# bplaut/PyTorch-VAE

Hardware: AMD Instinct MI355X
Metric: train images/sec (node) VanillaVAE 64×64 bs=64 at 1/2/4/8 GPU; ELBO match (higher is better)
Workload: dtype bf16; 1 GPU; VanillaVAE latent_dim=128 64x64 train step (fwd+ELBO+bwd+Adam); per_gpu_batch=64, global_batch=64, parallelism=dp1, graph=True, comm=none

## Files before the change

### include/vaehip.h

```cpp
#ifndef VAEHIP_H
#define VAEHIP_H

#include <stddef.h>
#include <stdint.h>

#ifdef __cplusplus
extern "C" {
#endif

#define VAE_ABI_VERSION 26

enum vae_dtype { VAE_F32 = 0, VAE_BF16 = 1 };

enum vae_status {
  VAE_OK = 0,
  VAE_E_BADARG = -1,
  VAE_E_BADSHAPE = -2,
  VAE_E_BADDTYPE = -3,
  VAE_E_UNSUPPORTED = -4
};

enum vae_xform_kind {
  VAE_X_NONE = 0,
  VAE_X_ACT = 1,
  VAE_X_BN_ACT = 2,
  VAE_X_BN_DY = 3
};

typedef struct vae_xform {
  int32_t kind;
  int32_t channels;
  float slope;
  float count;
  float eps;
  float momentum;
  const float* sum;
  const float* sumsq;
  const float* shift;
  const float* gamma;
  const float* beta;
  const float* dgamma;
  const float* dbeta;
  const void* aux;
  float* running_mean;
  float* running_var;
  int32_t reps;
  int32_t rstride;
  float* dgamma_out;
  float* dbeta_out;
  const float* table;
} vae_xform;

typedef struct vae_bn_args {
  int32_t mode;
  vae_xform xf;
  float* table;
  float* db;
} vae_bn_args;

typedef struct vae_conv_args {
  int32_t dtype;
  int32_t n, h, w, c;
  int32_t k, p, q;
  int32_t r, stride, pad;
  int32_t x_nchw_f32;
  const void* x;
  vae_xform x_xf;
  const void* wt;
  const float* bias;
  void* y;
  float* y_sum;
  float* y_sumsq;
  int32_t sum_reps;
  int32_t sum_rstride;
  const void* residual;
  vae_xform residual_xf;
  const void* dy;
  vae_xform dy_xf;
  void* dx;
  vae_xform dx_epi;
  float* dx_dgamma;
  float* dx_dbeta;
  float* dw;
  float* db;
  int32_t split_k;
  void* workspace;
  int64_t workspace_bytes;
  const struct vae_bn_args* bn_finalize;
  uint32_t* bn_counter;
  const void* wt_t;
  int32_t dw_inner;
  int32_t deterministic;
  int32_t defer_reduce;
} vae_conv_args;

typedef struct vae_linear_args {
  int32_t dtype;
  int32_t m, n, k;
  const void* x; vae_xform x_xf;
  const void* wt; const float* bias;
  void* y;
  int32_t y_f32;
  const void* dy;
  int32_t dy_f32;
  void* dx; vae_xform dx_epi; float* dx_dgamma; float* dx_dbeta;
  int32_t sum_reps, sum_rstride;
  float* dw; float* db;
  const float* mulv;
  const float* eps;
  const float* kl_coef;
  float* dmulv;
  int32_t samples;
  void* workspace;
  int64_t workspace_bytes;
  const struct vae_bn_args* bn_finalize;
  uint32_t* bn_counter;
  int32_t deterministic;
} vae_linear_args;

typedef struct vae_head_args {
  int32_t dtype;
  int32_t n, h, w, c;
  const void* x; vae_xform x_xf;
  const float* wt;
  const float* bias;
  const float* target;
  int32_t samples;
  float* recon;
  float* sse;
  const float* coef;
  void* dx; vae_xform dx_epi; float* dx_dgamma; float* dx_dbeta;
  int32_t sum_reps, sum_rstride;
  float* dw; float* db;
  const float* grad_recon;
  void* workspace;
  int64_t workspace_bytes;
  const struct vae_bn_args* bn_finalize;
  uint32_t* bn_counter;
  const struct vae_elbo_args* elbo;
  int32_t deterministic;
  int32_t defer_reduce;
} vae_head_args;



enum vae_loss_kind { VAE_LOSS_VANILLA = 0, VAE_LOSS_BETA_H = 1, VAE_LOSS_BETA_B = 2, VAE_LOSS_IWAE = 3,
                     VAE_LOSS_VQ = 4, VAE_LOSS_INFO = 5, VAE_LOSS_DIP = 6, VAE_LOSS_MIWAE = 7 };

typedef struct vae_elbo_args {
  int32_t kind;
  int32_t batch, samples, latent;
  int32_t img_elems;
  float kld_weight;
  float beta, gamma, c_max, c_stop_iter;
  const float* iter;
  const float* mulv;
  const float* sse;
  float* out;
  float* per_img;
  float* head_coef;
  float* kl_coef;
  const float* vq_sse;
  float vq_beta;
  float vq_elems;
  float recon_weight, kl_factor, mmd_coef;
  int32_t mmd_tiles;
  const double* mmd_partials;
  float* mmd_out;
} vae_elbo_args;

typedef struct vae_dip_args {
  int32_t batch, latent;
  float lambda_diag, lambda_offdiag;
  float grad_scale;
  int32_t reserved;
  const float* mulv;
  float* dmulv_dip;
  float* dmulv;
  void* workspace;
  int64_t workspace_bytes;
} vae_dip_args;

enum vae_mmd_kind { VAE_MMD_IMQ = 0, VAE_MMD_RBF = 1 };
typedef struct vae_mmd_args {
  int32_t kind;
  int32_t batch, latent;
  float latent_var;
  float grad_scale;
  int32_t prior_gen;
  const float* mulv;
  const float* eps;
  float* prior;
  float* dz;
  float* dmulv;
  void* workspace;
  int64_t workspace_bytes;
  const int32_t* prior_step;
  uint64_t prior_seed;
} vae_mmd_args;

typedef struct vae_vq_args {
  int32_t dtype;
  int32_t rows, dim, codes;
  const void* lat;
  vae_xform lat_xf;
  const float* codebook;
  int64_t* indices;
  void* q;
  float* sse;
  float beta;
  const void* dq;
  const float* loss_grad;
  void* dlat;
  float* dcodebook;
} vae_vq_args;

typedef struct vae_recon_args {
  int32_t dtype;
  int32_t n, h, w, c;
  const void* y;
  const float* target;
  float* recon;
  float* sse;
  void* dy;
  float grad_scale;
  const float* grad_recon;
  int32_t ld;
} vae_recon_args;

int vae_abi_version(void);
const char* vae_last_error(void);
const char* vae_build_digest(void);
int vae_launch_log(int32_t on);
int64_t vae_launch_log_names(char* buf, int64_t cap);

int vae_conv2d_fwd(const vae_conv_args* a, void* stream);
int vae_conv2d_bwd_data(const vae_conv_args* a, void* stream);
int vae_conv2d_bwd_filter(const vae_conv_args* a, void* stream);
int vae_convT2d_fwd(const vae_conv_args* a, void* stream);
int vae_convT2d_bwd_data(const vae_conv_args* a, void* stream);
int vae_convT2d_bwd_filter(const vae_conv_args* a, void* stream);
int vae_convT2d_bwd(const vae_conv_args* a, void* stream);
int vae_convT2d_fwd_recon(const vae_conv_args* a, const vae_recon_args* rc, void* stream);
int vae_linear_fwd(const vae_linear_args* a, void* stream);
int vae_linear_bwd_data(const vae_linear_args* a, void* stream);
int vae_linear_bwd_filter(const vae_linear_args* a, void* stream);
int vae_head_fwd(const vae_head_args* a, void* stream);
int vae_head_bwd_data(const vae_head_args* a, void* stream);
int vae_head_bwd_filter(const vae_head_args* a, void* stream);
int vae_head_bwd(const vae_head_args* a, void* stream);
int vae_bn_finalize(const vae_bn_args* a, void* stream);
int vae_reparam_fwd(int32_t dtype, int32_t rows, int32_t samples, int32_t latent,
                    const float* mulv, const float* eps, void* z, void* stream);
int vae_vq_fwd(const vae_vq_args* a, void* stream);
int vae_vq_bwd(const vae_vq_args* a, void* stream);
int vae_recon_fwd(const vae_recon_args* a, void* stream);
int vae_recon_bwd(const vae_recon_args* a, void* stream);
int vae_nchw_to_nhwc_pad(int32_t dtype, int32_t n, int32_t c, int32_t h, int32_t w, int32_t cp, const float* x,
                         void* y, void* stream);
int vae_pad_channels(int32_t dtype, int64_t rows, int32_t c, int32_t cp, const void* src, void* dst, void* stream);
int vae_unpad_accumulate(int64_t rows, int32_t cp, int32_t c, const float* src, float* dst, void* stream);
int vae_elbo_fwd(const vae_elbo_args* a, void* stream);
int vae_mmd_fwd(const vae_mmd_args* a, void* stream);
int vae_mmd_workspace_size(const vae_mmd_args* a, size_t* bytes, int32_t* tiles);
int vae_mmd_reseed(int32_t batch, int32_t latent, const float* dz, const float* scale, const float* mulv,
                   const float* eps, float* dmulv, void* stream);
int vae_dip_fwd(const vae_dip_args* a, void* stream);
int vae_dip_workspace_size(const vae_dip_args* a, size_t* bytes, int32_t* tiles);
int vae_adam_step(int64_t n, float* p, const float* g, float* m, float* v,
                  const int32_t* step, const float* lr, double beta1, double beta2, float eps,
                  float weight_decay, void* p_lowp, void* stream);
#define VAE_SUMSQ_MAX_PARTS 1024
int vae_grad_sumsq(int64_t n, const float* g, double* partials, int32_t* nparts_out, void* stream);
int vae_adam_step_clip(int64_t n, float* p, const float* g, float* m, float* v,
                       const int32_t* step, const float* lr, double beta1, double beta2, float eps,
                       float weight_decay, void* p_lowp, const double* partials, int32_t nparts,
                       const float* max_norm, float* norm_out, void* stream);
#define VAE_SLAB_MAX 32
typedef struct vae_grad_slab {
  float* dst;
  int64_t count;
  const float* slab;
  int32_t rows;
  int64_t ld;
} vae_grad_slab;
int vae_deferred_reset(void);
int32_t vae_deferred_take(vae_grad_slab* out, int32_t max, vae_elbo_args* elbo, int32_t* has_elbo);
typedef struct vae_adam_args {
  int64_t n;
  float* p; float* g; float* m; float* v;
  const int32_t* step; const float* lr;
  double beta1, beta2;
  float eps, weight_decay;
  void* p_lowp;
  int32_t nslab;
  vae_grad_slab slab[VAE_SLAB_MAX];
  int32_t has_elbo;
  vae_elbo_args elbo;
} vae_adam_args;
int vae_adam_step_ex(const vae_adam_args* a, void* stream);
int vae_cast_bf16(int64_t n, const float* src, void* dst, void* stream);
#define VAE_SWAP_MAX 16
typedef struct vae_swap_desc {
  const void* src;
  void* dst;
  int32_t a, rs, b;
  int32_t src_dtype;
} vae_swap_desc;
int vae_swap_axes(int32_t count, const vae_swap_desc* descs, void* stream);
enum vae_op { VAE_OP_FWD = 0, VAE_OP_BWD_DATA = 1, VAE_OP_BWD_FILTER = 2, VAE_OP_BWD = 3  };
int vae_conv2d_workspace_size(const vae_conv_args* a, int32_t op, size_t* bytes);
int vae_convT2d_workspace_size(const vae_conv_args* a, int32_t op, size_t* bytes);
int vae_linear_workspace_size(const vae_linear_args* a, int32_t op, size_t* bytes);
int vae_head_workspace_size(const vae_head_args* a, int32_t op, size_t* bytes);
enum vae_layer_kind { VAE_LAYER_CONV2D = 0, VAE_LAYER_CONVT2D = 1 };
int vae_conv_bwd_filter_batch(int32_t n, const int32_t* kinds, const vae_conv_args* const* items,
                              void* workspace, int64_t workspace_bytes, void* stream);
int vae_conv_bwd_filter_batch_workspace_size(int32_t n, const int32_t* kinds, const vae_conv_args* const* items,
                                             size_t* bytes);
typedef struct vae_record_args {
  int32_t batch, samples, img_elems, nterms, step;
  const float* src_terms; float* terms;
  const float* per_img; float* per;
  const float* img; const float* recon;
  float* best; int32_t* at;
  float* hi_img; float* hi_recon; float* lo_img; float* lo_recon;
} vae_record_args;
int vae_step_record(const vae_record_args* a, void* stream);
int vae_step_begin(void* zero, int64_t bytes, int32_t* step, void* stream);

#define VAE_PAD_MAX 4
typedef struct vae_pad_desc {
  int64_t rows;
  int32_t c, cp;
  const void* src;
  void* dst;
} vae_pad_desc;
typedef struct vae_step_begin_args {
  void* zero;
  int64_t bytes;
  int32_t* step;
  int32_t dtype;
  int32_t n, c, h, w, cp;
  const float* x;
  void* y;
  int32_t npad;
  vae_pad_desc pad[VAE_PAD_MAX];
  int32_t nswap;
  vae_swap_desc swap[VAE_SWAP_MAX];
  int32_t nkeep;
  struct { int64_t off, bytes; } keep[VAE_SLAB_MAX];
} vae_step_begin_args;
int vae_step_begin_ex(const vae_step_begin_args* a, void* stream);

typedef struct vae_latent_args {
  int32_t dtype;
  int32_t batch, samples, latent;
  int32_t in_features, out_features;
  const void* x;
  vae_xform x_xf;
  const void* w1;
  const float* b1;
  float* mulv;
  const float* eps;
  void* z;
  const void* w2;
  const float* b2;
  void* h;
  const void* dh;
  const float* kl_coef;
  float* dmulv;
  float* dw2; float* db2;
  void* dx;
  vae_xform dx_epi;
  float* dx_dgamma; float* dx_dbeta;
  int32_t sum_reps, sum_rstride;
  float* dw1; float* db1;
  const int32_t* eps_step;
  uint64_t eps_seed;
  int32_t eps_gen;
} vae_latent_args;
int vae_latent_fc_fwd(const vae_latent_args* a, void* stream);
int vae_latent_dec_fwd(const vae_latent_args* a, void* stream);
int vae_latent_dec_bwd(const vae_latent_args* a, void* stream);
int vae_latent_fc_bwd(const vae_latent_args* a, void* stream);

typedef struct vae_bn_apply_args {
  int32_t dtype;
  int64_t rows;
  int32_t channels;
  const void* x;
  vae_xform xf;
  float* db;
  void* out;
} vae_bn_apply_args;
int vae_bn_apply(const vae_bn_apply_args* a, void* stream);

enum vae_recon_loss_kind { VAE_RLOSS_CENTER = 0, VAE_RLOSS_MSSIM = 1 };
typedef struct vae_recon_loss_args {
  int32_t kind;
  int32_t n, c, h, w;
  const float* recon;
  const float* target;
  const float* mask;
  float window[16];
  int32_t window_size;
  int32_t levels;
  float level_weights[8];
  int32_t normalize;
  int32_t size_average;
  float* grad;
  float grad_scale;
  float* out;
  const float* sse;
  float* per_img;
  float* workspace;
  int64_t workspace_bytes;
} vae_recon_loss_args;
int vae_recon_loss(const vae_recon_loss_args* a, void* stream);
int vae_recon_loss_workspace_size(const vae_recon_loss_args* a, size_t* bytes);

typedef struct vae_logcosh_args {
  int32_t n;
  int32_t latent;
  int64_t elems;
  float alpha;
  float grad_scale;
  float kl_weight;
  int32_t reserved;
  const float* recon;
  const float* target;
  float* grad;
  const float* mulv;
  float* out;
  float* kl_coef;
  const float* sse;
  float* per_img;
  void* workspace;
  int64_t workspace_bytes;
} vae_logcosh_args;
int vae_logcosh_loss(const vae_logcosh_args* a, void* stream);
int vae_logcosh_loss_workspace_size(const vae_logcosh_args* a, size_t* bytes);

#ifdef __cplusplus
}
#endif
#endif
```

### pytorch-vae_amd/csrc/vae_cgemm.hpp

```cpp
#pragma once
#include "vae_igemm.hpp"

namespace vae {

template <int BM, int BN> struct CgWaves {
  static constexpr int WN = BN >= 2 * BM ? 4 : (BM >= 2 * BN ? 1 : 2);
  static constexpr int WM = 4 / WN;
  static constexpr int TM = BM / WM / 16, TN = BN / WN / 16;
  static_assert(TM >= 1 && TN >= 1, "wave tile below 16x16");
};

template <int XA>
__device__ __forceinline__ uint4 cg_xform(const uint32_t (&w)[4], const uint32_t (&y)[4], const Tab& t, int ch,
                                          float slope) {
  if constexpr (XA == VAE_X_NONE) {
    return uint4{w[0], w[1], w[2], w[3]};
  } else {
    uint4 o;
    uint32_t* op = reinterpret_cast<uint32_t*>(&o);
    f32x2 ab[4], bb[4], cb[4];
    if constexpr (XA != VAE_X_ACT) {
      const f32x4 a0 = tab4(t.a, ch), a1 = tab4(t.a, ch + 4);
      ab[0] = f32x2{a0[0], a0[1]}; ab[1] = f32x2{a0[2], a0[3]}; ab[2] = f32x2{a1[0], a1[1]}; ab[3] = f32x2{a1[2], a1[3]};
      {
        const f32x4 b0 = tab4(t.b, ch), b1 = tab4(t.b, ch + 4);
        bb[0] = f32x2{b0[0], b0[1]}; bb[1] = f32x2{b0[2], b0[3]}; bb[2] = f32x2{b1[0], b1[1]}; bb[3] = f32x2{b1[2], b1[3]};
      }
      if constexpr (XA == VAE_X_BN_DY) {
        const f32x4 c0 = tab4(t.c, ch), c1 = tab4(t.c, ch + 4);
        cb[0] = f32x2{c0[0], c0[1]}; cb[1] = f32x2{c0[2], c0[3]}; cb[2] = f32x2{c1[0], c1[1]}; cb[3] = f32x2{c1[2], c1[3]};
      }
    }
    const f32x2 sl = f32x2{slope, slope};
#pragma unroll
    for (int e = 0; e < 4; ++e) {
      const f32x2 v = f32x2{__uint_as_float(w[e] << 16), __uint_as_float(w[e] & 0xffff0000u)};
      f32x2 r;
      if constexpr (XA == VAE_X_ACT) {
        r = __builtin_elementwise_max(v, v * sl);
      } else if constexpr (XA == VAE_X_BN_ACT) {
        const f32x2 z = __builtin_elementwise_fma(v, ab[e], bb[e]);
        r = __builtin_elementwise_max(z, z * sl);
      } else {
        const f32x2 u = f32x2{__uint_as_float(y[e] << 16), __uint_as_float(y[e] & 0xffff0000u)};
        r = __builtin_elementwise_fma(ab[e], v, __builtin_elementwise_fma(bb[e], u, cb[e]));
      }
      bf16x2 pk;
      pk[0] = (__bf16)r[0];
      pk[1] = (__bf16)r[1];
      op[e] = *reinterpret_cast<uint32_t*>(&pk);
    }
    return o;
  }
}

constexpr int kRingLoads = 20, kRingMax = 8;
constexpr int cg_ring(int loads) {
  return kRingLoads / loads < 2 ? 2 : (kRingLoads / loads > kRingMax ? kRingMax : kRingLoads / loads);
}
template <int LOADS> constexpr int cg_stages() { return cg_ring(LOADS); }
constexpr int kRingLoadsDeep = 40, kRingMaxDeep = 16;
constexpr int cg_ring_deep(int loads) {
  return kRingLoadsDeep / loads < 2 ? 2 : (kRingLoadsDeep / loads > kRingMaxDeep ? kRingMaxDeep : kRingLoadsDeep / loads);
}
template <int LOADS> constexpr int wg_stages() {
  return 20 / LOADS < 2 ? 2 : (20 / LOADS > 8 ? 8 : 20 / LOADS);
}

template <int BM, int BN, int BK, int NBUF = 2> struct CgSmem {
  static constexpr int LDK = BK + 8;
  static constexpr int LOOP = NBUF * (BM + BN) * LDK * 2;
  static constexpr int EPI = BM * (BN + 4) * 4;
  static constexpr int BYTES = LOOP > EPI ? LOOP : EPI;
};

template <int BM, int BN, int XA> constexpr int cg_waves_per_eu() {
  return (BM >= 128 && BN >= 128) ? 2 : ((BM == 64 && BN == 32 && XA == VAE_X_BN_DY) ? 3 : 1);
}

template <int BM, int BN, int BK, int AM, int XA, int EM, int OR>
__device__ __forceinline__ void cgemm_body(const GemmParams& p, const int bid, char* smem) {
  using WG = CgWaves<BM, BN>;
  constexpr int TM = WG::TM, TN = WG::TN, WTM = TM * 16, WTN = TN * 16;
  constexpr int LDK = CgSmem<BM, BN, BK>::LDK;
  constexpr int KC = BK / 8;
  constexpr int RPP = 256 / KC;
  constexpr int APT = (BM + RPP - 1) / RPP, BPT = (BN + RPP - 1) / RPP;
  constexpr bool DY = XA == VAE_X_BN_DY;
  constexpr int NSF = OR == 3 ? cg_ring_deep(APT * (DY ? 2 : 1) + BPT) : cg_stages<APT * (DY ? 2 : 1) + BPT>();
  constexpr int NS = OR == 2 ? (NSF < 2 ? NSF : 2) : NSF;
  constexpr int NBUF = OR == 2 ? 1 : 2;
  constexpr bool ABN = XA == VAE_X_BN_ACT || XA == VAE_X_BN_DY;
  static_assert(BM % RPP == 0 || BM < RPP, "A tile rows");
  static_assert(BN % RPP == 0 || BN < RPP, "B tile rows");

  extern __shared__ float tabs[];
  __bf16* As = reinterpret_cast<__bf16*>(smem);
  __bf16* Bs = As + NBUF * BM * LDK;

#ifdef VAE_PROBE
  unsigned long long clk[4] = {0, 0, 0, 0};
  const unsigned long long wall0 = threadIdx.x == 0 ? wall_clock64() : 0;
#endif
  PROBE_MARK(0);
  const int tid = threadIdx.x, lane = tid & 63;
  const int wave = __builtin_amdgcn_readfirstlane(tid >> 6);
  const int wm = wave / WG::WN, wn = wave % WG::WN;
  const int gm = (p.M + BM - 1) / BM, gn = (p.N + BN - 1) / BN, gz = p.nphase * p.ksplit;
  int tile;
  {
    const int nb = gm * gn * gz, b = bid;
    const int q = nb >> 3, r = nb & 7, x = b & 7, loc = b >> 3;
    tile = x * q + min(x, r) + loc;
  }
  int tn, tz, tmi;
  if (p.m_fast) { tmi = tile % gm; tz = (tile / gm) % gz; tn = tile / (gm * gz); }
  else { tn = tile % gn; tz = (tile / gn) % gz; tmi = tile / (gn * gz); }
  const int m0 = tmi * BM, n0 = tn * BN;
  const int phase = (p.nphase > 1) ? (int)(tz / p.ksplit) : 0;
  const int ks = tz - phase * p.ksplit;
  const bool first_block = tile == 0;

  const PhaseInfo pq = make_phase(p, phase);
  const int Kp = AM == A_CONVT ? pq.nth * pq.ntw * p.gc : p.K;
  const int ktiles = (Kp + BK - 1) / BK;
  const int kper = (ktiles + p.ksplit - 1) / p.ksplit;
  const int kt0 = ks * kper;
  const int kt1 = min(ktiles, kt0 + kper);
  const int kend = min(Kp, kt1 * BK);

  const int kc = tid % KC, r0 = tid / KC;
  const Src<__bf16> sa = make_src<__bf16>(p.a_ptr, p.a_bytes, p.a_xf);
  const rsrc_t rb = make_rsrc(p.b_ptr, p.b_bytes);
  RowOperand<__bf16, AM, true> ar[APT];
  int bbase[BPT];
  bool bok[BPT];
#pragma unroll
  for (int i = 0; i < APT; ++i) ar[i].init(p, m0 + r0 + i * RPP, p.M, phase, p.a_ld);
#pragma unroll
  for (int i = 0; i < BPT; ++i) {
    const int n = n0 + r0 + i * RPP;
    bok[i] = n < p.N && r0 + i * RPP < BN;
    bbase[i] = n * p.b_ld;
  }
  const bool a_row_in_tile = r0 < BM;

  struct Stage {
    uint32_t a[APT][4];
    uint32_t y[DY ? APT : 1][4];
    uint32_t b[BPT][4];
    int ch;
    uint32_t okm;
  };
  auto issue = [&](int kt, Stage& st) {
    const int kk = kt * BK + 8 * kc;
    const KTap t = RowOperand<__bf16, AM, true>::tap(p, pq, p.fd_ach, p.a_xf.channels, ABN, kk, kend);
    st.ch = t.ch;
    uint32_t okm = 0u;
#pragma unroll
    for (int i = 0; i < APT; ++i) {
      bool ok = ar[i].valid && t.kin && a_row_in_tile;
      ok = ok && (uint32_t)(ar[i].hi0 + t.r) < (uint32_t)p.gh && (uint32_t)(ar[i].wi0 + t.s) < (uint32_t)p.gw;
      okm |= (uint32_t)ok << i;
      const uint32_t off = ok ? (uint32_t)(ar[i].base + t.toff) * 2u : kOOB;
      bload<16>(sa.x, off, st.a[i]);
      if constexpr (DY) bload<16>(sa.y, off, st.y[i]);
    }
    st.okm = okm;
    int boff = kk;
    if constexpr (AM == A_CONVT) {
      const int rr = pq.t0h - p.gs * t.r, ss = pq.t0w - p.gs * t.s;
      boff = t.kin ? (rr * p.gr + ss) * p.gc + t.ch : 0;
    }
#pragma unroll
    for (int i = 0; i < BPT; ++i) {
      const uint32_t off = (bok[i] && t.kin) ? (uint32_t)(bbase[i] + boff) * 2u : kOOB;
      bload<16>(rb, off, st.b[i]);
    }
  };

  const int ca = tab_stride(p.a_xf.channels), ce = tab_stride(p.epi_xf.channels);
  const Tab ta{tabs, tabs + ca, tabs + 2 * ca, nullptr, nullptr};
  float* tq = tabs + (ABN ? 3 * ca : 0);
  const Tab te{tq, tq + ce, nullptr, tq + 2 * ce, tq + 3 * ce};

  constexpr int TCH = 2;
  float tva[3][TCH], tve[4][TCH];
  const bool a_tab = ABN && p.a_xf.table != nullptr && p.a_xf.channels <= 256 * TCH;
  const bool e_tab = EM == E_BNBWD && p.epi_xf.kind == VAE_X_BN_ACT && p.epi_xf.table != nullptr &&
                     p.epi_xf.channels <= 256 * TCH;
  if (a_tab) {
    const int C = p.a_xf.channels;
#pragma unroll
    for (int j = 0; j < TCH; ++j) {
      const int ch = min(tid + 256 * j, C - 1);
#pragma unroll
      for (int q = 0; q < (DY ? 3 : 2); ++q) tva[q][j] = p.a_xf.table[q * C + ch];
    }
  }
  if (e_tab) {
    const int C = p.epi_xf.channels;
#pragma unroll
    for (int j = 0; j < TCH; ++j) {
      const int ch = min(tid + 256 * j, C - 1);
#pragma unroll
      for (int q = 0; q < 4; ++q) tve[q][j] = p.epi_xf.table[q * C + ch];
    }
  }
  TabPre<DY ? 4 : 2> pa;
  TabPre<2> pe;
  const bool a_pre = ABN && !a_tab && tab_pre_ok<XA>(p.a_xf);
  const bool e_pre = EM == E_BNBWD && !e_tab && tab_pre_ok<VAE_X_BN_ACT>(p.epi_xf);
  if (a_pre) tab_pre_load(p.a_xf, pa);
  if (e_pre) tab_pre_load(p.epi_xf, pe);
  Stage ring[NS];
#pragma unroll
  for (int u = 0; u < NS; ++u) {
    if (!OR || kt0 + u < kt1) issue(kt0 + u, ring[u]);
  }
  constexpr int EC = BN / 8, ERS = 256 / EC;
  constexpr int EPT = (BM + ERS - 1) / ERS;
  const int ec = tid % EC, er0 = tid / EC;
  const int col = n0 + ec * 8;
  const bool col_ok = col < p.N;
  uint32_t aux[EPT][4], res[EPT][4];
  int obase[EPT];
  bool rok[EPT];
  float bias[8];
  const bool has_res = p.residual != nullptr;
  constexpr bool EARLY = EPT <= 2 && cg_waves_per_eu<BM, BN, XA>() < 3;
  auto epi_loads = [&]() {
    const rsrc_t raux = epi_aux_rsrc<EM>(p);
    const rsrc_t rres = epi_res_rsrc<EM>(p);
    const bool loads = p.slab == nullptr;
#pragma unroll
    for (int i = 0; i < EPT; ++i) {
      const int rl = er0 + i * ERS, row = m0 + rl;
      rok[i] = rl < BM && row < p.M && col_ok;
      obase[i] = out_row_base(p, phase, rok[i] ? row : 0) + col;
      const uint32_t off = (rok[i] && loads) ? (uint32_t)obase[i] * 2u : kOOB;
      bload<16>(raux, off, aux[i]);
      if (EM == E_BNBWD && has_res) bload<16>(rres, off, res[i]);
      else res[i][0] = res[i][1] = res[i][2] = res[i][3] = 0u;
    }
#pragma unroll
    for (int e = 0; e < 8; ++e) bias[e] = 0.f;
    if (EM == E_STORE && p.bias && col_ok && loads) {
#pragma unroll
      for (int e = 0; e < 8; ++e) bias[e] = p.bias[col + e];
    }
  };
  if constexpr (EARLY) epi_loads();
  if (a_tab) {
    const int C = p.a_xf.channels;
#pragma unroll
    for (int j = 0; j < TCH; ++j) {
      const int ch = tid + 256 * j;
      if (ch < C) {
        ta.a[ch] = tva[0][j]; ta.b[ch] = tva[1][j];
        if (DY) ta.c[ch] = tva[2][j];
      }
    }
  } else if constexpr (ABN) {
    tab_fill_pre(p.a_xf, pa, a_pre, ta, false, first_block, reinterpret_cast<float*>(smem));
  }
  if constexpr (ABN) {
    if (tid < 8) { const int z = tab_pad(p.a_xf.channels) + tid; ta.a[z] = 0.f; ta.b[z] = 0.f; ta.c[z] = 0.f; }
  }
  if (e_tab) {
    const int C = p.epi_xf.channels;
#pragma unroll
    for (int j = 0; j < TCH; ++j) {
      const int ch = tid + 256 * j;
      if (ch < C) { te.a[ch] = tve[0][j]; te.b[ch] = tve[1][j]; te.p[ch] = tve[2][j]; te.q[ch] = tve[3][j]; }
    }
  } else if constexpr (EM == E_BNBWD) {
    tab_fill_pre(p.epi_xf, pe, e_pre, te, true, false, reinterpret_cast<float*>(smem));
  }
  __syncthreads();
  PROBE_MARK(1);

  f32x4 acc[TM][TN];
#pragma unroll
  for (int i = 0; i < TM; ++i)
#pragma unroll
    for (int j = 0; j < TN; ++j) acc[i][j] = f32x4{0.f, 0.f, 0.f, 0.f};

  auto store = [&](int buf, const Stage& st) {
    __bf16* ad = As + buf * BM * LDK + r0 * LDK + kc * 8;
#pragma unroll
    for (int i = 0; i < APT; ++i) {
      if (r0 + i * RPP < BM) {
        uint4 v;
        if constexpr (XA == VAE_X_NONE) {
          v = uint4{st.a[i][0], st.a[i][1], st.a[i][2], st.a[i][3]};
        } else {
          const int ch = ((st.okm >> i) & 1u) ? st.ch : sa.zs;
          v = cg_xform<XA>(st.a[i], st.y[DY ? i : 0], ta, ch, sa.slope);
        }
        *reinterpret_cast<uint4*>(ad + i * RPP * LDK) = v;
      }
    }
    __bf16* bd = Bs + buf * BN * LDK + r0 * LDK + kc * 8;
#pragma unroll
    for (int i = 0; i < BPT; ++i)
      if (r0 + i * RPP < BN) *reinterpret_cast<uint4*>(bd + i * RPP * LDK) = uint4{st.b[i][0], st.b[i][1], st.b[i][2], st.b[i][3]};
  };
  auto compute = [&](int buf) {
    const __bf16* a = As + buf * BM * LDK + (wm * WTM + (lane & 15)) * LDK + 8 * (lane >> 4);
    const __bf16* b = Bs + buf * BN * LDK + (wn * WTN + (lane & 15)) * LDK + 8 * (lane >> 4);
#pragma unroll
    for (int kk = 0; kk < BK / 32; ++kk) {
      bf16x8 af[TM], bfr[TN];
#pragma unroll
      for (int i = 0; i < TM; ++i) af[i] = *reinterpret_cast<const bf16x8*>(a + i * 16 * LDK + 32 * kk);
#pragma unroll
      for (int j = 0; j < TN; ++j) bfr[j] = *reinterpret_cast<const bf16x8*>(b + j * 16 * LDK + 32 * kk);
#pragma unroll
      for (int i = 0; i < TM; ++i)
#pragma unroll
        for (int j = 0; j < TN; ++j) acc[i][j] = __builtin_amdgcn_mfma_f32_16x16x32_bf16(af[i], bfr[j], acc[i][j], 0, 0, 0);
    }
  };

  if constexpr (OR != 0) {
#pragma unroll
    for (int u = 0; u < NS; ++u) {
      if (kt0 + u < kt1) {
        if (NBUF == 1 && u > 0) __syncthreads();
        store(u & (NBUF - 1), ring[u]);
        __syncthreads();
        compute(u & (NBUF - 1));
      }
    }
  } else {
    int buf = 0;
    for (int kb = kt0; kb < kt1; kb += NS) {
#pragma unroll
      for (int u = 0; u < NS; ++u) {
        const bool live = kb + u < kt1;
        if (live) store(buf, ring[u]);
        __syncthreads();
        issue(kb + u + NS, ring[u]);
        if (live) compute(buf);
        buf ^= 1;
      }
    }
  }
  PROBE_MARK(2);
#ifdef VAE_PROBE
  struct ProbeEnd {
    unsigned long long* pr; unsigned long long* clk; unsigned long long w0;
    __device__ ~ProbeEnd() { PROBE_MARK(3); probe_write(pr, clk, w0); }
  } probe_end{p.probe, clk, wall0};
#endif

  __shared__ float fpart[CgWaves<BM, BN>::WM][2][BN];
  const bool frag_sums = EM == E_STORE && p.sum != nullptr && p.slab == nullptr;
  if (frag_sums) {
#pragma unroll
    for (int j = 0; j < TN; ++j) {
      float a1 = 0.f, a2 = 0.f;
#pragma unroll
      for (int i = 0; i < TM; ++i)
#pragma unroll
        for (int e = 0; e < 4; ++e) { a1 += acc[i][j][e]; a2 = fmaf(acc[i][j][e], acc[i][j][e], a2); }
      a1 += __shfl_xor(a1, 16); a2 += __shfl_xor(a2, 16);
      a1 += __shfl_xor(a1, 32); a2 += __shfl_xor(a2, 32);
      if (lane < 16) { fpart[wm][0][wn * WTN + j * 16 + lane] = a1; fpart[wm][1][wn * WTN + j * 16 + lane] = a2; }
    }
  }
  __syncthreads();
  float* Cs = reinterpret_cast<float*>(smem);
  constexpr int LDC = BN + 4;
  {
    const int rq = wm * WTM + 4 * (lane >> 4), cq = wn * WTN + (lane & 15);
#pragma unroll
    for (int i = 0; i < TM; ++i)
#pragma unroll
      for (int j = 0; j < TN; ++j)
#pragma unroll
        for (int e = 0; e < 4; ++e) Cs[(rq + i * 16 + e) * LDC + cq + j * 16] = acc[i][j][e];
  }
  __syncthreads();
  if (p.slab) {
    float* sl = p.slab + ((long)(phase * p.ksplit + ks) * p.M) * p.N;
#pragma unroll
    for (int i = 0; i < EPT; ++i) {
      const int rl = er0 + i * ERS, row = m0 + rl;
      if (rl < BM && row < p.M && col_ok) {
        const f32x4 v0 = *reinterpret_cast<const f32x4*>(Cs + rl * LDC + ec * 8);
        const f32x4 v1 = *reinterpret_cast<const f32x4*>(Cs + rl * LDC + ec * 8 + 4);
        *reinterpret_cast<f32x4*>(sl + (long)row * p.N + col) = v0;
        *reinterpret_cast<f32x4*>(sl + (long)row * p.N + col + 4) = v1;
      }
    }
    return;
  }
  if constexpr (!EARLY) epi_loads();
  float s1[8], s2[8];
#pragma unroll
  for (int e = 0; e < 8; ++e) { s1[e] = 0.f; s2[e] = 0.f; }
  int ech = 0;
  if constexpr (EM == E_BNBWD) ech = (int)(col - p.fd_ech.div(col) * p.epi_xf.channels);
  uint4 pk[EPT];
#pragma unroll
  for (int i = 0; i < EPT; ++i) {
    const int rl = min(er0 + i * ERS, BM - 1);
    float v[8], ax[8], rs[8];
    {
      const f32x4 v0 = *reinterpret_cast<const f32x4*>(Cs + rl * LDC + ec * 8);
      const f32x4 v1 = *reinterpret_cast<const f32x4*>(Cs + rl * LDC + ec * 8 + 4);
#pragma unroll
      for (int e = 0; e < 4; ++e) { v[e] = v0[e]; v[e + 4] = v1[e]; }
    }
#pragma unroll
    for (int e = 0; e < 4; ++e) {
      ax[2 * e] = __uint_as_float(aux[i][e] << 16);
      ax[2 * e + 1] = __uint_as_float(aux[i][e] & 0xffff0000u);
      rs[2 * e] = __uint_as_float(res[i][e] << 16);
      rs[2 * e + 1] = __uint_as_float(res[i][e] & 0xffff0000u);
    }
    const float w = rok[i] ? 1.f : 0.f;
    float o[8];
    if constexpr (EM == E_STORE) {
      const bool ract = p.res_xf.kind == VAE_X_ACT;
#pragma unroll
      for (int e = 0; e < 8; ++e) {
        float y = v[e] + bias[e];
        if (has_res) y += ract ? lrelu(ax[e], p.res_xf.slope) : ax[e];
        o[e] = y;
      }
    } else {
      const int ek = p.epi_xf.kind;
#pragma unroll
      for (int e = 0; e < 8; ++e) {
        const float g0 = v[e] + rs[e];
        float g = g0;
        if (ek == VAE_X_BN_ACT) {
          const float z = fmaf(ax[e], te.a[ech + e], te.b[ech + e]);
          g = z > 0.f ? g0 : g0 * p.epi_xf.slope;
          s1[e] = fmaf(w, g, s1[e]);
          s2[e] = fmaf(w * g, fmaf(ax[e], te.p[ech + e], te.q[ech + e]), s2[e]);
        } else if (ek == VAE_X_ACT) {
          g = ax[e] > 0.f ? g0 : g0 * p.epi_xf.slope;
        }
        o[e] = g;
      }
    }
    uint32_t* pp = reinterpret_cast<uint32_t*>(&pk[i]);
#pragma unroll
    for (int e = 0; e < 4; ++e) {
      bf16x2 h;
      h[0] = (__bf16)o[2 * e];
      h[1] = (__bf16)o[2 * e + 1];
      pp[e] = *reinterpret_cast<uint32_t*>(&h);
    }
  }
  if (frag_sums) {
    for (int c = tid; c < BN; c += 256) {
      if (n0 + c < p.N) {
        float t1 = 0.f, t2 = 0.f;
#pragma unroll
        for (int w = 0; w < CgWaves<BM, BN>::WM; ++w) { t1 += fpart[w][0][c]; t2 += fpart[w][1][c]; }
        epi_flush_sums<EM>(p, bid, n0 + c, t1, t2);
      }
    }
  } else if (EM == E_BNBWD && epi_wants_sums<EM>(p)) {
    float* part = Cs;
#pragma unroll
    for (int m = EC; m < 64; m <<= 1) {
#pragma unroll
      for (int e = 0; e < 8; ++e) {
        s1[e] += __shfl_xor(s1[e], m);
        s2[e] += __shfl_xor(s2[e], m);
      }
    }
    __syncthreads();
    if (lane < EC) {
#pragma unroll
      for (int e = 0; e < 8; ++e) {
        part[(wave * 2) * BN + ec * 8 + e] = s1[e];
        part[(wave * 2 + 1) * BN + ec * 8 + e] = s2[e];
      }
    }
    __syncthreads();
    for (int c = tid; c < BN; c += 256) {
      if (n0 + c < p.N) {
        const float t1 = (part[0 * BN + c] + part[2 * BN + c]) + (part[4 * BN + c] + part[6 * BN + c]);
        const float t2 = (part[1 * BN + c] + part[3 * BN + c]) + (part[5 * BN + c] + part[7 * BN + c]);
        epi_flush_sums<EM>(p, bid, n0 + c, t1, t2);
      }
    }
  }
  __bf16* out = static_cast<__bf16*>(p.out);
#pragma unroll
  for (int i = 0; i < EPT; ++i)
    if (rok[i]) *reinterpret_cast<uint4*>(out + obase[i]) = pk[i];
}

template <int BM, int BN, int BK, int OR> constexpr int cg_nbuf() { return OR == 2 ? 1 : 2; }

template <int BM, int BN, int BK, int AM, int XA, int EM, int OR>
__global__ void __launch_bounds__(256) __attribute__((amdgpu_waves_per_eu(cg_waves_per_eu<BM, BN, XA>())))
cgemm_kernel(const GemmParams p) {
  kernarg_prefetch<sizeof(GemmParams)>();
  __shared__ __attribute__((aligned(16))) char smem[CgSmem<BM, BN, BK, cg_nbuf<BM, BN, BK, OR>()>::BYTES];
  cgemm_body<BM, BN, BK, AM, XA, EM, OR>(p, (int)blockIdx.x, smem);
}

}
```

### pytorch-vae_amd/csrc/vae_common.hpp

```cpp
#pragma once
#include <hip/hip_runtime.h>
#include <stdint.h>
#include <string.h>

#include "vaehip.h"

typedef float f32x4 __attribute__((ext_vector_type(4)));
typedef float f32x2 __attribute__((ext_vector_type(2)));
typedef __bf16 bf16x8 __attribute__((ext_vector_type(8)));
typedef __bf16 bf16x4 __attribute__((ext_vector_type(4)));
typedef __bf16 bf16x2 __attribute__((ext_vector_type(2)));

namespace vae {

void set_error(const char* fmt, ...);
int fail(int code, const char* fmt, ...);
int check_launch(const char* what);
int bn_finalize_launch(const vae_bn_args* a, hipStream_t stream);
constexpr int kRouteDeclined = 0x7fff0001;

inline int grid_for(long n, int per_block = 256, int max_blocks = 2048) {
  long b = (n + per_block - 1) / per_block;
  if (b < 1) b = 1;
  return (int)(b > max_blocks ? max_blocks : b);
}

struct OrdSum {
  const float* slab;
  long rstride;
  int groups, rpg, cols, cw;
  long hstride;
  int folds;
  long fstride;
  float* dst[2];
  long gstride;
};
int ordered_sum_launch(const OrdSum& o, hipStream_t st);

struct WsQuery {
  int on;
  long need;
};
inline WsQuery& ws_query() {
  static thread_local WsQuery q = {0, 0};
  return q;
}
inline bool querying() { return ws_query().on != 0; }
struct Deferred {
  int n;
  vae_grad_slab s[VAE_SLAB_MAX];
  int has_elbo;
  vae_elbo_args elbo;
};
inline Deferred& deferred() {
  static thread_local Deferred d = {};
  return d;
}
inline bool defer_slab(float* dst, long count, const float* slab, int rows, long ld) {
  if (querying()) return true;
  Deferred& d = deferred();
  for (int i = 0; i < d.n; ++i)
    if (d.s[i].dst == dst) {
      d.s[i] = vae_grad_slab{dst, count, slab, rows, ld};
      return true;
    }
  if (d.n >= VAE_SLAB_MAX) {
    fail(VAE_E_UNSUPPORTED, "deferred reductions: more than %d outstanding", VAE_SLAB_MAX);
    return false;
  }
  d.s[d.n++] = vae_grad_slab{dst, count, slab, rows, ld};
  return true;
}
inline void defer_elbo(const vae_elbo_args& e) {
  if (querying()) return;
  Deferred& d = deferred();
  d.has_elbo = 1;
  d.elbo = e;
}
inline bool ws_fits(long need, long have, const char* what) {
  WsQuery& q = ws_query();
  if (q.on) {
    if (need > q.need) q.need = need;
    return true;
  }
  if (need <= have) return true;
  fail(VAE_E_BADARG, "%s: workspace of %ld bytes < %ld required (see vae_*_workspace_size)", what, have, need);
  return false;
}
template <class F>
inline int with_ws_tail(long tail, F&& f) {
  WsQuery& q = ws_query();
  if (!q.on) return f();
  const long outer = q.need;
  q.need = 0;
  const int rc = f();
  const long inner = ((q.need + 255) / 256) * 256 + tail;
  q.need = outer > inner ? outer : inner;
  return rc;
}
struct LaunchLog {
  int on;
  int n;
  const void* k[64];
  int count[64];
};
inline LaunchLog& launch_log() {
  static thread_local LaunchLog l = {0, 0, {}, {}};
  return l;
}
inline void log_launch(const void* k) {
  LaunchLog& l = launch_log();
  if (!l.on) return;
  for (int i = 0; i < l.n; ++i)
    if (l.k[i] == k) { ++l.count[i]; return; }
  if (l.n < 64) { l.count[l.n] = 1; l.k[l.n++] = k; }
}
}
#define VAE_LAUNCH(K, ...)                                      \
  do {                                                          \
    if (!::vae::querying()) {                                   \
      ::vae::log_launch((const void*)(K));                      \
      hipLaunchKernelGGL(K, __VA_ARGS__);                       \
    }                                                           \
  } while (0)
namespace vae {

template <int BYTES>
__device__ __forceinline__ void kernarg_prefetch() {
  const void* k = (const void*)__builtin_amdgcn_kernarg_segment_ptr();
  unsigned d1, d2, d3, d4, d5, d6, d7;
  if constexpr (BYTES > 960) {
    unsigned e1, e2, e3, e4, e5, e6, e7, e8;
    asm volatile(
        "s_load_dword %0, %15, 64\n s_load_dword %1, %15, 128\n s_load_dword %2, %15, 192\n"
        " s_load_dword %3, %15, 256\n s_load_dword %4, %15, 320\n s_load_dword %5, %15, 384\n"
        " s_load_dword %6, %15, 448\n s_load_dword %7, %15, 512\n s_load_dword %8, %15, 576\n"
        " s_load_dword %9, %15, 640\n s_load_dword %10, %15, 704\n s_load_dword %11, %15, 768\n"
        " s_load_dword %12, %15, 832\n s_load_dword %13, %15, 896\n s_load_dword %14, %15, 960\n"
        " s_waitcnt lgkmcnt(0)"
        : "=&s"(d1), "=&s"(d2), "=&s"(d3), "=&s"(d4), "=&s"(d5), "=&s"(d6), "=&s"(d7), "=&s"(e1), "=&s"(e2), "=&s"(e3),
          "=&s"(e4), "=&s"(e5), "=&s"(e6), "=&s"(e7), "=&s"(e8)
        : "s"(k));
  } else if constexpr (BYTES > 448) {
    asm volatile(
        "s_load_dword %0, %7, 64\n s_load_dword %1, %7, 128\n s_load_dword %2, %7, 192\n"
        " s_load_dword %3, %7, 256\n s_load_dword %4, %7, 320\n s_load_dword %5, %7, 384\n"
        " s_load_dword %6, %7, 448\n s_waitcnt lgkmcnt(0)"
        : "=&s"(d1), "=&s"(d2), "=&s"(d3), "=&s"(d4), "=&s"(d5), "=&s"(d6), "=&s"(d7)
        : "s"(k));
  } else if constexpr (BYTES > 192) {
    asm volatile("s_load_dword %0, %3, 64\n s_load_dword %1, %3, 128\n s_load_dword %2, %3, 192\n"
                 " s_waitcnt lgkmcnt(0)"
                 : "=&s"(d1), "=&s"(d2), "=&s"(d3)
                 : "s"(k));
  } else if constexpr (BYTES > 64) {
    asm volatile("s_load_dword %0, %1, 64\n s_waitcnt lgkmcnt(0)" : "=&s"(d1) : "s"(k));
  }
}

__device__ __forceinline__ float ld_f(const float* p) { return *p; }
__device__ __forceinline__ float ld_f(const __bf16* p) { return (float)(*p); }
template <class T> __device__ __forceinline__ T cvt(float v);
template <> __device__ __forceinline__ float cvt<float>(float v) { return v; }
template <> __device__ __forceinline__ __bf16 cvt<__bf16>(float v) { return (__bf16)v; }

__device__ __forceinline__ void ld8(const float* p, float (&v)[8]) {
  f32x4 a = *reinterpret_cast<const f32x4*>(p);
  f32x4 b = *reinterpret_cast<const f32x4*>(p + 4);
  v[0] = a[0]; v[1] = a[1]; v[2] = a[2]; v[3] = a[3];
  v[4] = b[0]; v[5] = b[1]; v[6] = b[2]; v[7] = b[3];
}
__device__ __forceinline__ void ld8(const __bf16* p, float (&v)[8]) {
  bf16x8 a = *reinterpret_cast<const bf16x8*>(p);
#pragma unroll
  for (int j = 0; j < 8; ++j) v[j] = (float)a[j];
}
__device__ __forceinline__ void ld4(const float* p, float (&v)[4]) {
  f32x4 a = *reinterpret_cast<const f32x4*>(p);
  v[0] = a[0]; v[1] = a[1]; v[2] = a[2]; v[3] = a[3];
}
__device__ __forceinline__ void ld4(const __bf16* p, float (&v)[4]) {
  bf16x4 a = *reinterpret_cast<const bf16x4*>(p);
#pragma unroll
  for (int j = 0; j < 4; ++j) v[j] = (float)a[j];
}

__device__ __forceinline__ void st8(float* d, const float (&v)[8]) {
  *reinterpret_cast<f32x4*>(d) = f32x4{v[0], v[1], v[2], v[3]};
  *reinterpret_cast<f32x4*>(d + 4) = f32x4{v[4], v[5], v[6], v[7]};
}
__device__ __forceinline__ void st8(__bf16* d, const float (&v)[8]) {
  bf16x8 o;
#pragma unroll
  for (int j = 0; j < 8; ++j) o[j] = (__bf16)v[j];
  *reinterpret_cast<bf16x8*>(d) = o;
}
__device__ __forceinline__ void st2(float* d, float a, float b) { *reinterpret_cast<f32x2*>(d) = f32x2{a, b}; }
// ... 310 lines not shown
```

### pytorch-vae_amd/csrc/vae_convT_bwd_data.hip

```cpp
#include "vae_launch.hpp"
#include "vae_wgrad.hpp"

using namespace vae;

extern "C" int vae_convT2d_bwd_data(const vae_conv_args* a, void* stream) {
  if (int rc = check_geom(a, "convT2d_bwd_data")) return rc;
  if (!a->dy || !a->wt || !a->dx) return fail(VAE_E_BADARG, "convT2d_bwd_data: null tensor");
  if (!xf_ok(a->dy_xf, "convT2d_bwd_data.dy") || !epi_ok(a->dx_epi, "convT2d_bwd_data.epi")) return VAE_E_BADARG;
  hipStream_t st = (hipStream_t)stream;
  GemmParams p = strided_conv_params(a, true, a->wt, a->pad);
  if (int rc = bwd_epilogue(p, a->dx_epi, a->dx_dgamma, a->dx_dbeta, a->sum_reps, a->sum_rstride, nullptr, "convT2d_bwd_data"))
    return rc;
  if (int rc = check_finalize(a->bn_finalize, "convT2d_bwd_data")) return rc;
  if (a->dtype == VAE_BF16 && cg_ok(p, E_BNBWD))
    return then_finalize(cg_launch<A_CONV, E_BNBWD>(p, a->split_k, a->workspace, a->workspace_bytes, st), a->bn_finalize, st);
  return then_finalize(launch<A_CONV, B_NK, E_BNBWD, true, false>(a->dtype, false, false, p, a->split_k, a->workspace,
                                                                  a->workspace_bytes, st),
                       a->bn_finalize, st);
}
```

### pytorch-vae_amd/csrc/vae_convT_fwd.hip

```cpp
#include "vae_launch.hpp"
#include "vae_wgrad.hpp"
#include "vae_hires.hpp"

using namespace vae;

extern "C" int vae_convT2d_fwd(const vae_conv_args* a, void* stream) {
  if (int rc = check_geom(a, "convT2d_fwd")) return rc;
  if (!a->x || !a->wt || !a->y) return fail(VAE_E_BADARG, "convT2d_fwd: null tensor");
  if (!xf_ok(a->x_xf, "convT2d_fwd.x")) return VAE_E_BADARG;
  const int S = a->stride;
  if (a->p % S || a->q % S) return fail(VAE_E_BADSHAPE, "convT2d_fwd: output not a multiple of stride");
  hipStream_t st = (hipStream_t)stream;
  GemmParams p;
  if (!phase_gather_params(p, a, false)) return fail(VAE_E_UNSUPPORTED, "convT2d_fwd: stride/kernel");
  fwd_epilogue(p, a);
  if (int rc = check_finalize(a->bn_finalize, "convT2d_fwd")) return rc;
  if (a->dtype == VAE_BF16) {
    const int rc = hires_convT_fwd_launch(a, st);
    if (rc != kRouteDeclined) return rc;
    const StagedWeights w = staged_weights(a, a->wt_t);
    GemmParams q = p;
    swapped_weights(q, w.ptr);
    if (w.ptr && cg_ok(q, E_STORE)) {
      return with_staged_weights(w, a, a->c, a->k, 0, "convT2d_fwd weight copy", st, [&]() -> int {
        return then_finalize(cg_launch<A_CONVT, E_STORE>(q, a->split_k, a->workspace, w.slab_bytes, st), a->bn_finalize, st);
      });
    }
  }
  return then_finalize(launch<A_CONVT, B_KN, E_STORE, false, false>(a->dtype, false, false, p, a->split_k, a->workspace,
                                                                    a->workspace_bytes, st),
                       a->bn_finalize, st);
}
```

### pytorch-vae_amd/csrc/vae_conv_bwd_data.hip

```cpp
#include "vae_launch.hpp"
#include "vae_wgrad.hpp"
#include "vae_c3.hpp"

using namespace vae;

extern "C" int vae_conv2d_bwd_data(const vae_conv_args* a, void* stream) {
  const char* what = "conv2d_bwd_data";
  if (int rc = check_geom(a, what)) return rc;
  if (!a->dy || !a->wt || !a->dx) return fail(VAE_E_BADARG, "conv2d_bwd_data: null tensor");
  if (!xf_ok(a->dy_xf, "conv2d_bwd_data.dy") || !epi_ok(a->dx_epi, "conv2d_bwd_data.epi")) return VAE_E_BADARG;
  if (a->x_nchw_f32) return fail(VAE_E_UNSUPPORTED, "conv2d_bwd_data: no gradient for the NCHW image input");
  const int S = a->stride;
  if (a->h % S || a->w % S || a->h / S != a->p || a->w / S != a->q)
    return fail(VAE_E_BADSHAPE, "conv2d_bwd_data: needs h == p*stride (got h=%d p=%d S=%d)", a->h, a->p, S);
  hipStream_t st = (hipStream_t)stream;
  const bool tile = a->dtype == VAE_BF16 && a->wt_t && a->dy_xf.kind == VAE_X_NONE &&
                    (a->dx_epi.kind == VAE_X_NONE || a->dx_epi.kind == VAE_X_ACT) && !a->dx_dgamma && !a->bn_finalize &&
                    a->split_k <= 0;
  if (tile && pointwise(a) && p1_shape_ok((long)a->n * a->h * a->w, a->k, a->c)) {
    P1Args c;
    memset(&c, 0, sizeof(c));
    c.a = a->dy; c.b = a->wt_t; c.out = a->dx; c.residual = a->residual;
    if (a->dx_epi.kind == VAE_X_ACT) { c.aux = a->dx_epi.aux; c.aux_slope = a->dx_epi.slope; }
    c.M = (long)a->n * a->h * a->w; c.C = a->k; c.N = a->c;
    return p1_launch(c, st);
  }
  if (tile && c3_shape_ok(a->n, a->p, a->q, a->h, a->w, a->r, a->stride, a->pad, a->k, a->c)) {
    C3Args c;
    memset(&c, 0, sizeof(c));
    c.a = a->dy; c.b = a->wt_t; c.flip = 1; c.out = a->dx; c.residual = a->residual;
    if (a->dx_epi.kind == VAE_X_ACT) { c.aux = a->dx_epi.aux; c.aux_slope = a->dx_epi.slope; }
    c.n = a->n; c.C = a->k; c.N = a->c;
    return c3_launch(c, st);
  }
  auto epilogue = [&](GemmParams& p) {
    return bwd_epilogue(p, a->dx_epi, a->dx_dgamma, a->dx_dbeta, a->sum_reps, a->sum_rstride, a->residual, what);
  };
  GemmParams p;
  const bool phases = phase_gather_params(p, a, true);
  if (phases) {
    if (int rc = epilogue(p)) return rc;
  }
  if (phases && a->dtype == VAE_BF16) {
    const StagedWeights w = staged_weights(a, a->wt_t);
    GemmParams q = p;
    swapped_weights(q, w.ptr);
    if (w.ptr && cg_ok(q, E_BNBWD)) {
      if (int rc = check_finalize(a->bn_finalize, what)) return rc;
      return with_staged_weights(w, a, a->k, a->c, 0, "conv2d_bwd_data weight copy", st, [&]() -> int {
        return then_finalize(cg_launch<A_CONVT, E_BNBWD>(q, a->split_k, a->workspace, w.slab_bytes, st), a->bn_finalize, st);
      });
    }
  }
  if (S == 1 && a->dtype == VAE_BF16 && a->c % 8 == 0 && a->k % 8 == 0 && a->workspace) {
    const StagedWeights w = staged_weights(a, nullptr);
    return with_staged_weights(w, a, a->k, a->c, 1, "conv2d_bwd_data weight copy", st, [&]() -> int {
      GemmParams f = strided_conv_params(a, true, w.ptr, a->r - 1 - a->pad);
      if (int rc = epilogue(f)) return rc;
      if (int rc = check_finalize(a->bn_finalize, what)) return rc;
      return then_finalize(launch<A_CONV, B_NK, E_BNBWD, true, false>(a->dtype, false, false, f, a->split_k, a->workspace,
                                                                      w.slab_bytes, st),
                           a->bn_finalize, st);
    });
  }
  if (!phases) return fail(VAE_E_UNSUPPORTED, "conv2d_bwd_data: stride/kernel");
  if (int rc = check_finalize(a->bn_finalize, what)) return rc;
  return then_finalize(launch<A_CONVT, B_KN, E_BNBWD, true, false>(a->dtype, false, false, p, a->split_k, a->workspace,
                                                                   a->workspace_bytes, st),
                       a->bn_finalize, st);
}
```

### pytorch-vae_amd/csrc/vae_conv_fwd.hip

```cpp
#include "vae_launch.hpp"
#include "vae_wgrad.hpp"
#include "vae_c3.hpp"

using namespace vae;

extern "C" int vae_conv2d_fwd(const vae_conv_args* a, void* stream) {
  if (int rc = check_geom(a, "conv2d_fwd")) return rc;
  if (!a->x || !a->wt || !a->y) return fail(VAE_E_BADARG, "conv2d_fwd: null tensor");
  if (!xf_ok(a->x_xf, "conv2d_fwd.x")) return VAE_E_BADARG;
  hipStream_t st = (hipStream_t)stream;
  const bool tile = a->dtype == VAE_BF16 && !a->x_nchw_f32 && (a->x_xf.kind == VAE_X_NONE || a->x_xf.kind == VAE_X_ACT) &&
                    !a->y_sum && !a->y_sumsq && !a->bn_finalize && a->split_k <= 0;
  if (tile && pointwise(a) && p1_shape_ok((long)a->n * a->p * a->q, a->c, a->k) &&
      (a->residual_xf.kind == VAE_X_NONE || a->residual_xf.kind == VAE_X_ACT)) {
    P1Args c;
    memset(&c, 0, sizeof(c));
    c.a = a->x; c.a_act = a->x_xf.kind == VAE_X_ACT; c.a_slope = a->x_xf.slope;
    c.b = a->wt; c.out = a->y; c.bias = a->bias;
    c.residual = a->residual; c.res_act = a->residual && a->residual_xf.kind == VAE_X_ACT; c.res_slope = a->residual_xf.slope;
    c.M = (long)a->n * a->p * a->q; c.C = a->c; c.N = a->k;
    return p1_launch(c, st);
  }
  if (tile && c3_shape_ok(a->n, a->h, a->w, a->p, a->q, a->r, a->stride, a->pad, a->c, a->k) && !a->residual) {
    C3Args c;
    memset(&c, 0, sizeof(c));
    c.a = a->x; c.a_act = a->x_xf.kind == VAE_X_ACT; c.a_slope = a->x_xf.slope;
    c.b = a->wt; c.flip = 0; c.out = a->y; c.bias = a->bias;
    c.n = a->n; c.C = a->c; c.N = a->k;
    return c3_launch(c, st);
  }
  GemmParams p = strided_conv_params(a, false, a->wt, a->pad);
  fwd_epilogue(p, a);
  if (int rc = check_finalize(a->bn_finalize, "conv2d_fwd")) return rc;
  if (a->dtype == VAE_BF16 && cg_ok(p, E_STORE))
    return then_finalize(cg_launch<A_CONV, E_STORE>(p, a->split_k, a->workspace, a->workspace_bytes, st), a->bn_finalize, st);
  return then_finalize(launch<A_CONV, B_NK, E_STORE, false, false, true>(a->dtype, a->x_nchw_f32 != 0, false, p, a->split_k,
                                                                         a->workspace, a->workspace_bytes, st),
                       a->bn_finalize, st);
}
```

### pytorch-vae_amd/csrc/vae_igemm.hpp

```cpp
#pragma once
#include "vae_common.hpp"

namespace vae {

enum AMode { A_CONV = 0, A_CONVT = 1, A_DENSE = 2, A_KM = 3 };
enum BMode { B_NK = 0, B_KN = 1, B_GATHER = 2 };
enum EMode { E_STORE = 0, E_BNBWD = 1, E_ACC = 2, E_REPARAM = 3 };

constexpr int MAXC = 4096;
constexpr int NTHREADS = 256;

template <class T> constexpr int bk_of() { return sizeof(T) == 2 ? 64 : 32; }

struct FastDiv {
  uint32_t d, mul, shr;
  __device__ __forceinline__ uint32_t div(uint32_t n) const { return (__umulhi(n, mul) + n) >> shr; }
};

inline FastDiv make_fastdiv(uint32_t d) {
  FastDiv f;
  f.d = d < 1 ? 1 : d;
  uint32_t l = 0;
  while ((1ull << l) < f.d) ++l;
  f.shr = l;
  f.mul = (uint32_t)(((1ull << 32) * ((1ull << l) - f.d)) / f.d + 1);
  if (f.d == 1) f.mul = 0;
  return f;
}

struct GemmParams {
  int M, N, K;
  int ksplit, nphase;
  const void* a_ptr; int a_ld; vae_xform a_xf;
  const void* b_ptr; int b_ld; vae_xform b_xf;
  int ones_col;
  int b_taps;
  int g_nchw;
  int gn, gh, gw, gc, gp, gq, gr, gs, gpad, gho, gwo;
  int ntap_h[2], ntap_w[2], tap0[2];
  int tap_d[2];
  FastDiv fd_gq, fd_gp, fd_gc, fd_gr, fd_ntw[2];
  void* out; int out_ld; int out_phase;
  int out_f32;
  const float* bias; float* sum; float* sumsq;
  const void* residual; vae_xform res_xf;
  vae_xform epi_xf; float* dgamma; float* dbeta;
  float* bias_grad;
  float* dbc; int dbc_from_b;
  int sum_reps, sum_rstride;
  const float* mulv; const float* eps; const float* kl_coef; float* dmulv; int samples, latent;
  float* slab;
  uint32_t a_bytes, b_bytes;
  FastDiv fd_ach, fd_bch;
  FastDiv fd_ech;
  uint32_t out_aux_bytes;
  unsigned long long* probe;
  int m_fast;
  int det;
  float* det_slab;
  int det_rows;
};

#ifdef VAE_PROBE
#define PROBE_MARK(i) do { if (threadIdx.x == 0) clk[i] = __builtin_readcyclecounter(); } while (0)
__device__ __forceinline__ void probe_write(unsigned long long* pr, const unsigned long long* clk,
                                           unsigned long long w0) {
  if (!pr || threadIdx.x != 0) return;
  const unsigned long long slot = blockIdx.x + (unsigned long long)gridDim.x * (blockIdx.y + (unsigned long long)gridDim.y * blockIdx.z);
  if (slot >= pr[1]) return;
  unsigned long long* r = pr + 8 + slot * 8;
  r[0] = blockIdx.x | ((unsigned long long)blockIdx.y << 21) | ((unsigned long long)blockIdx.z << 42);
  r[1] = w0;
  r[2] = wall_clock64();
  r[3] = clk[0]; r[4] = clk[1]; r[5] = clk[2]; r[6] = clk[3];
  r[7] = __builtin_amdgcn_s_getreg((23 << 0) | (0 << 6) | (31 << 11));
}
#else
#define PROBE_MARK(i) do { } while (0)
#endif

struct PhaseInfo {
  int ph, pw, t0h, t0w, nth, ntw;
  int dh, dw;
  FastDiv fdw;
};

__device__ __forceinline__ PhaseInfo make_phase(const GemmParams& p, int phase) {
  PhaseInfo q;
  q.ph = phase >= p.gs ? 1 : 0;
  q.pw = phase - q.ph * p.gs;
  q.t0h = q.ph ? p.tap0[1] : p.tap0[0];
  q.t0w = q.pw ? p.tap0[1] : p.tap0[0];
  q.nth = q.ph ? p.ntap_h[1] : p.ntap_h[0];
  q.ntw = q.pw ? p.ntap_w[1] : p.ntap_w[0];
  q.fdw = q.pw ? p.fd_ntw[1] : p.fd_ntw[0];
  q.dh = q.ph ? p.tap_d[1] : p.tap_d[0];
  q.dw = q.pw ? p.tap_d[1] : p.tap_d[0];
  return q;
}

__device__ __forceinline__ void tab_zero_slot(const vae_xform& x, Tab t) {
  if (threadIdx.x < 8) {
    const int z = tab_pad(x.channels) + threadIdx.x;
    t.a[z] = 0.f; t.b[z] = 0.f;
    if (x.kind == VAE_X_BN_DY) t.c[z] = 0.f;
  }
}

__device__ __forceinline__ void tab_fill(const vae_xform& x, Tab t, bool epi, bool update_running, float* scr) {
  if (x.kind != VAE_X_BN_ACT && x.kind != VAE_X_BN_DY) return;
  tab_zero_slot(x, t);
  if (x.table) {
    const int C = x.channels;
    const bool dy = x.kind == VAE_X_BN_DY;
    const int nt = blockDim.x;
    for (int c0 = threadIdx.x; c0 < C; c0 += 4 * nt) {
      float v[4][4];
#pragma unroll
      for (int u = 0; u < 4; ++u) {
        const int ch = c0 + u * nt, cc = ch < C ? ch : C - 1;
        v[u][0] = x.table[cc];
        v[u][1] = x.table[C + cc];
        v[u][2] = (dy || epi) ? x.table[2 * C + cc] : 0.f;
        v[u][3] = (!dy && epi) ? x.table[3 * C + cc] : 0.f;
      }
#pragma unroll
      for (int u = 0; u < 4; ++u) {
        const int ch = c0 + u * nt;
        if (ch >= C) break;
        t.a[ch] = v[u][0]; t.b[ch] = v[u][1];
        if (dy) t.c[ch] = v[u][2];
        else if (epi) { t.p[ch] = v[u][2]; t.q[ch] = v[u][3]; }
      }
    }
    return;
  }
  if (blockDim.x == 256 && bn_fast_ok(x)) {
    tab_build(x, t, epi, update_running, scr);
    return;
  }
  for (int ch = threadIdx.x; ch < x.channels; ch += blockDim.x) {
    BnMom mo;
    bn_moments(x, ch, mo.mean, mo.invstd, mo.var);
    const float g = x.gamma[ch];
    if (x.kind == VAE_X_BN_ACT) {
      const BnFwd f = bn_fwd(mo, g);
      t.a[ch] = f.a;
      t.b[ch] = f.b(x.beta[ch]);
      if (epi) { t.p[ch] = f.p; t.q[ch] = f.q; }
      if (update_running && x.running_mean) {
        const float unb = bn_unbiased(mo, x);
        x.running_mean[ch] = bn_momentum(x, x.running_mean[ch], mo.mean);
        x.running_var[ch] = bn_momentum(x, x.running_var[ch], unb);
      }
    } else {
      const float inv_m = 1.0f / x.count;
      const float A = g * mo.invstd;
      const float mg = rsum(x.dbeta, x, ch) * inv_m;
      const float mgx = rsum(x.dgamma, x, ch) * inv_m;
      t.a[ch] = A;
      t.b[ch] = -A * mo.invstd * mgx;
      t.c[ch] = -A * (mg - mo.mean * mo.invstd * mgx);
    }
  }
}

__device__ __forceinline__ void tab_fill(const vae_xform& x, Tab t, bool epi, bool update_running) {
  __shared__ float scr[4 * 256];
  tab_fill(x, t, epi, update_running, scr);
}

template <int KIND>
__device__ __forceinline__ bool tab_pre_ok(const vae_xform& x) {
  return x.kind == KIND && !x.table && blockDim.x == 256 && bn_fast_ok(x);
}
template <int NS>
__device__ __forceinline__ void tab_fill_pre(const vae_xform& x, const TabPre<NS>& q, bool pre, Tab t, bool epi,
                                             bool update_running, float* scr) {
  if (!pre) { tab_fill(x, t, epi, update_running, scr); return; }
  tab_zero_slot(x, t);
  tab_pre_finish(x, q, t, epi, update_running, scr);
}

__host__ __device__ inline int tab_floats(const vae_xform& x, bool epi) {
  if (x.kind != VAE_X_BN_ACT && x.kind != VAE_X_BN_DY) return 0;
  return (epi ? 4 : 3) * tab_stride(x.channels);
}

constexpr uint32_t kOOB = 0x80000000u;
typedef __amdgpu_buffer_rsrc_t rsrc_t;

__device__ __forceinline__ rsrc_t make_rsrc(const void* ptr, uint32_t bytes) {
  return __builtin_amdgcn_make_buffer_rsrc(const_cast<void*>(ptr), (short)0, (int)bytes, 0x00020000);
}

template <int NB>
__device__ __forceinline__ void bload(rsrc_t r, uint32_t off, uint32_t* d) {
  if constexpr (NB == 16) {
    const auto v = __builtin_amdgcn_raw_buffer_load_b128(r, off, 0, 0);
    d[0] = v[0]; d[1] = v[1]; d[2] = v[2]; d[3] = v[3];
  } else if constexpr (NB == 8) {
    const auto v = __builtin_amdgcn_raw_buffer_load_b64(r, off, 0, 0);
    d[0] = v[0]; d[1] = v[1];
  } else if constexpr (NB == 4) {
    d[0] = __builtin_amdgcn_raw_buffer_load_b32(r, off, 0, 0);
  } else {
    d[0] = __builtin_amdgcn_raw_buffer_load_b16(r, off, 0, 0);
  }
}

template <class TIn>
struct Src {
  rsrc_t x, y;
// ... 997 lines not shown
```

### pytorch-vae_amd/csrc/vae_launch.hpp

```cpp
#pragma once
#include "vae_fgemm.hpp"
#include "vae_cgemm.hpp"
#include "vae_bgemm.hpp"
#include "vae_gemm_desc.hpp"
#include <stdlib.h>

#ifdef VAE_PROBE
extern "C" unsigned long long* vae_probe_buffer(void);
#endif

namespace vae {
namespace {

constexpr int kCUs = 256;
constexpr int kTargetBlocks = 512;
constexpr long kLdsBytes = 160 * 1024;

inline long cg_table_bytes(const GemmParams& p, int em) {
  const int k = p.a_xf.kind;
  return 4l * (((k == VAE_X_BN_ACT || k == VAE_X_BN_DY) ? 3 * tab_stride(p.a_xf.channels) : 0) +
               (em == E_BNBWD ? 4 * tab_stride(p.epi_xf.channels) : 0));
}
inline long cg_static_bytes(int bm, int bn) {
  const int bk = bm >= 128 ? 64 : 128;
  const long loop = 2l * (bm + bn) * (bk + 8) * 2, epi = (long)bm * (bn + 4) * 4;
  const int wn = bn >= 2 * bm ? 4 : (bm >= 2 * bn ? 1 : 2);
  return (loop > epi ? loop : epi) + (4 / wn) * 2l * bn * 4 + 256;
}

inline bool xf_ok(const vae_xform& x, const char* what) {
  if (x.kind < VAE_X_NONE || x.kind > VAE_X_BN_DY) { fail(VAE_E_BADARG, "%s: bad xform kind %d", what, x.kind); return false; }
  if (x.kind == VAE_X_BN_ACT || x.kind == VAE_X_BN_DY) {
    if (x.channels > MAXC) { fail(VAE_E_UNSUPPORTED, "%s: %d channels > %d", what, x.channels, MAXC); return false; }
    if (!x.sum || !x.sumsq || !x.gamma || !x.beta || x.count <= 0.f) {
      fail(VAE_E_BADARG, "%s: BatchNorm transform needs sum/sumsq/gamma/beta/count", what); return false;
    }
    if (x.kind == VAE_X_BN_DY && (!x.dgamma || !x.dbeta || !x.aux)) {
      fail(VAE_E_BADARG, "%s: BN_DY transform needs dgamma/dbeta/aux", what); return false;
    }
  }
  if ((x.kind == VAE_X_ACT || x.kind == VAE_X_BN_ACT) && !(x.slope >= 0.f && x.slope <= 1.f)) {
    fail(VAE_E_BADARG, "%s: LeakyReLU slope %g outside [0, 1]", what, x.slope); return false;
  }
  return true;
}

inline bool epi_ok(const vae_xform& x, const char* what) {
  if (!xf_ok(x, what)) return false;
  if ((x.kind == VAE_X_BN_ACT || x.kind == VAE_X_ACT) && !x.aux) {
    fail(VAE_E_BADARG, "%s: activation-backward epilogue needs aux (the stored pre-activation)", what);
    return false;
  }
  if (x.kind == VAE_X_BN_DY) { fail(VAE_E_BADARG, "%s: BN_DY is not an epilogue transform", what); return false; }
  return true;
}

inline int check_finalize(const vae_bn_args* f, const char* what) {
  if (!f) return VAE_OK;
  if (f->mode != 0 && f->mode != 1) return fail(VAE_E_BADARG, "%s: fused finalisation mode %d", what, f->mode);
  if (!f->table || f->xf.channels <= 0 || !f->xf.sum || !f->xf.sumsq || !f->xf.gamma || !f->xf.beta || f->xf.count <= 0.f ||
      (f->mode == 1 && (!f->xf.dgamma || !f->xf.dbeta)) || f->xf.reps > BNF_LANES * BNF_PER)
    return fail(VAE_E_BADARG, "%s: bn_finalize args", what);
  return VAE_OK;
}

inline int then_finalize(int rc, const vae_bn_args* f, hipStream_t st) {
  if (rc || !f) return rc;
  return bn_finalize_launch(f, st);
}

template <int AM>
inline long a_elems(const GemmParams& p) {
  if (AM == A_CONV || AM == A_CONVT) return (long)p.gn * p.gh * p.gw * p.gc;
  if (AM == A_DENSE) return (long)(p.M - 1) * p.a_ld + p.K;
  return (long)(p.K - 1) * p.a_ld + p.M;
}

template <int BMD>
inline long b_elems(const GemmParams& p) {
  if (BMD == B_GATHER) return (long)p.gn * p.gh * p.gw * p.gc;
  if (BMD == B_NK) return (long)(p.N - 1) * p.b_ld + p.K;
  const long rows = p.b_taps ? (long)p.gc * p.gr * p.gr : p.K;
  return (rows - 1) * p.b_ld + (p.ones_col >= 0 ? p.N - 1 : p.N);
}

inline int phase_kmax(const GemmParams& p, int am) {
  if (am != A_CONVT) return p.K;
  int kmax = 0;
  for (int ph = 0; ph < p.nphase; ++ph) {
    const int k = p.ntap_h[ph / p.gs] * p.ntap_w[ph % p.gs] * p.gc;
    kmax = k > kmax ? k : kmax;
  }
  return kmax;
}

inline long out_elems(const GemmParams& p) {
  if (p.out_phase) return (long)p.gn * p.gho * p.gwo * p.out_ld;
  return (long)p.M * p.out_ld;
}

inline int set_extents(GemmParams& p, const char* kernel, long ab, long bb, long ob, long aux, const char* out_note) {
  constexpr long lim = 1l << 31;
  if (ab <= 0 || bb <= 0 || ab >= lim || bb >= lim)
    return fail(VAE_E_UNSUPPORTED, "%s: operand of %ld / %ld bytes (buffer addressing needs < 2 GiB)", kernel, ab, bb);
  if (ob >= lim) return fail(VAE_E_UNSUPPORTED, "%s: output of %ld bytes%s", kernel, ob, out_note);
  p.a_bytes = (uint32_t)ab;
  p.b_bytes = (uint32_t)bb;
  p.out_aux_bytes = (uint32_t)aux;
#ifdef VAE_PROBE
  p.probe = vae_probe_buffer();
#endif
  return VAE_OK;
}

inline bool aligned(const void* ptr, int bytes) { return ((uintptr_t)ptr & (uintptr_t)(bytes - 1)) == 0; }

inline bool bn_kind(const vae_xform& x) { return x.kind == VAE_X_BN_ACT || x.kind == VAE_X_BN_DY; }

template <int MODE>
inline int operand_vec(const GemmParams& p, const void* ptr, const vae_xform& xf, int esize) {
  const bool vk = MODE == A_CONV || MODE == A_CONVT || MODE == A_DENSE || MODE == 100 + B_NK;
  const int grp = vk ? 8 : 4;
  const int vbytes = (grp * esize) < 16 ? grp * esize : 16;
  if (!aligned(ptr, vbytes) || (xf.kind == VAE_X_BN_DY && !aligned(xf.aux, vbytes))) return 0;
  if (bn_kind(xf) && xf.channels % grp) return 0;
  const int nrows = p.N - (p.ones_col >= 0 ? 1 : 0);
  switch (MODE) {
    case A_CONV: return !p.g_nchw && p.gc % grp == 0;
    case 100 + B_GATHER: return !p.g_nchw && p.gc % grp == 0 && nrows % grp == 0;
    case A_CONVT: return p.gc % grp == 0;
    case A_DENSE: return p.a_ld % grp == 0 && p.K % grp == 0;
    case A_KM: return p.a_ld % grp == 0 && p.M % grp == 0;
    case 100 + B_NK: return p.b_ld % grp == 0 && p.K % grp == 0;
    case 100 + B_KN: return p.b_ld % grp == 0 && nrows % grp == 0;
  }
  return 0;
}

inline void finish_divs(GemmParams& p) {
  p.fd_gq = make_fastdiv(p.gq > 0 ? p.gq : 1);
  p.fd_gp = make_fastdiv(p.gp > 0 ? p.gp : 1);
  p.fd_gc = make_fastdiv(p.gc > 0 ? p.gc : 1);
  p.fd_gr = make_fastdiv(p.gr > 0 ? p.gr : 1);
  p.fd_ntw[0] = make_fastdiv(p.ntap_w[0] > 0 ? p.ntap_w[0] : 1);
  p.fd_ntw[1] = make_fastdiv(p.ntap_w[1] > 0 ? p.ntap_w[1] : 1);
  p.fd_ach = make_fastdiv(p.a_xf.channels > 0 ? p.a_xf.channels : 1);
  p.fd_bch = make_fastdiv(p.b_xf.channels > 0 ? p.b_xf.channels : 1);
  p.fd_ech = make_fastdiv(p.epi_xf.channels > 0 ? p.epi_xf.channels : 1);
}

struct Tile { int bm, bn; };

inline long tile_blocks(long M, long N, int nphase, Tile t) {
  return ((M + t.bm - 1) / t.bm) * ((N + t.bn - 1) / t.bn) * nphase;
}

constexpr int kTileBlocks = 4 * kCUs;
inline Tile pick_tile(long M, long N, int nphase) {
  const Tile wide[] = {{64, 64}, {64, 32}, {32, 64}, {32, 32}};
  const Tile thin_n[] = {{128, 32}, {64, 32}, {32, 32}};
  const Tile thin_m[] = {{32, 128}, {32, 64}, {32, 32}};
  const Tile* c = N <= 32 ? thin_n : (M <= 32 ? thin_m : wide);
  const int nc = N <= 32 ? 3 : (M <= 32 ? 3 : 4);
  for (int i = 0; i < nc; ++i)
    if (tile_blocks(M, N, nphase, c[i]) >= kTileBlocks) return c[i];
  return c[nc - 1];
}

inline int pick_split(long blocks, int ktiles) {
  if (blocks >= kTargetBlocks || ktiles < 8) return 1;
  int s = (int)((kTargetBlocks + blocks - 1) / blocks);
  const int maxs = ktiles / 4;
  if (s > maxs) s = maxs;
  return s < 2 ? 1 : s;
}

inline int split_fits(int* split, int split_req, const GemmParams& p, const void* ws, long ws_bytes, const char* what) {
  if (*split <= 1) return VAE_OK;
  if (!ws && !querying()) {
    if (split_req > 1) return fail(VAE_E_BADARG, "%s: split_k %d needs a workspace", what, split_req);
    *split = 1;
    return VAE_OK;
  }
  return ws_fits((long)*split * p.M * p.N * p.nphase * 4, ws_bytes, what) ? VAE_OK : VAE_E_BADARG;
}

template <class T, int EM>
inline int launch_finalize(const GemmParams& p, hipStream_t st) {
  const long rows = (long)p.M * p.nphase;
  const dim3 grid((unsigned)((rows + FIN_ROWS - 1) / FIN_ROWS), (unsigned)((p.N + 63) / 64));
  const size_t lds = EM == E_BNBWD ? (size_t)tab_floats(p.epi_xf, true) * 4 : 0;
  if (p.N % 4 == 0) VAE_LAUNCH((igemm_finalize<T, EM, true>), grid, dim3(NTHREADS), lds, st, p);
  else VAE_LAUNCH((igemm_finalize<T, EM, false>), grid, dim3(NTHREADS), lds, st, p);
  return check_launch("igemm_finalize");
}

template <int EM>
inline bool det_wants_sums(const GemmParams& p) {
  return (EM == E_STORE && p.sum) || (EM == E_BNBWD && p.epi_xf.kind == VAE_X_BN_ACT);
}
inline long det_sum_rows(const GemmParams& p, int bm) {
  if (p.ksplit > 1) return ((long)p.M * p.nphase + FIN_ROWS - 1) / FIN_ROWS;
  return (long)((p.M + bm - 1) / bm) * p.nphase;
}
template <int EM>
inline long det_slab_bytes(const GemmParams& p, int bm) {
  if (!p.det) return 0;
  if (det_wants_sums<EM>(p)) return det_sum_rows(p, bm) * 2 * p.N * 4;
  if (EM == E_REPARAM) return (long)p.M * 2 * p.latent * 4;
  return 0;
}
template <int EM>
inline int det_reduce(const GemmParams& p, hipStream_t st) {
  if (!p.det_slab) return VAE_OK;
  OrdSum o;
  memset(&o, 0, sizeof(o));
  o.slab = p.det_slab;
  if (EM == E_REPARAM) {
    o.rstride = 2L * p.latent; o.groups = p.M / p.samples; o.rpg = p.samples;
    o.cols = 2 * p.latent; o.cw = p.latent; o.hstride = p.latent; o.folds = 1;
    o.dst[0] = p.dmulv; o.dst[1] = p.dmulv + p.latent; o.gstride = 2L * p.latent;
  } else {
    const int ch = EM == E_STORE ? p.N : p.epi_xf.channels;
    o.rstride = 2L * p.N; o.groups = 1; o.rpg = (int)(p.det_rows);
    o.cols = 2 * ch; o.cw = ch; o.hstride = p.N; o.folds = p.N / ch; o.fstride = ch;
    o.dst[0] = EM == E_STORE ? p.sum : p.dbeta;
    o.dst[1] = EM == E_STORE ? p.sumsq : p.dgamma;
  }
  return ordered_sum_launch(o, st);
}

inline thread_local bool lds_error = false;
template <class K>
inline bool lds_fits(K kernel, size_t dyn) {
  if (dyn <= 64 * 1024 || querying()) return true;
  hipFuncAttributes at;
  if (hipFuncGetAttributes(&at, reinterpret_cast<const void*>(kernel)) != hipSuccess) return true;
  if ((long)(at.sharedSizeBytes + dyn) <= kLdsBytes) return true;
  lds_error = true;
  return false;
}

#define VAE_TILE_CASE(BM_, BN_) \
  if (t.bm == BM_ && t.bn == BN_) { \
    if (lds_fits(igemm_kernel<T, TA, TB, BM_, BN_, AM, BMD, EM, VA, VB, DYA, DYB>, lds)) \
      VAE_LAUNCH((igemm_kernel<T, TA, TB, BM_, BN_, AM, BMD, EM, VA, VB, DYA, DYB>), grid, block, lds, st, p); \
    return; \
  }

template <class T, class TA, class TB, int AM, int BMD, int EM, bool VA, bool VB, bool DYA, bool DYB>
inline void launch_shape(const GemmParams& p, Tile t, hipStream_t st) {
  const dim3 block(NTHREADS);
  const dim3 grid((p.M + t.bm - 1) / t.bm, (p.N + t.bn - 1) / t.bn, p.nphase * p.ksplit);
  const size_t lds = (size_t)table_floats(p, EM == E_BNBWD) * 4;
  VAE_TILE_CASE(64, 64)
  VAE_TILE_CASE(128, 32)
  VAE_TILE_CASE(32, 128)
  VAE_TILE_CASE(64, 32)
  VAE_TILE_CASE(32, 64)
  VAE_TILE_CASE(32, 32)
}
#undef VAE_TILE_CASE

template <class T, class TA, class TB, int AM, int BMD, int EM, bool DYA, bool DYB>
inline int launch_tiled(GemmParams p, Tile t, hipStream_t st) {
  const bool tensor_out = EM != E_ACC && EM != E_REPARAM;
  const long oe = tensor_out ? out_elems(p) : 0;
  if (int rc = set_extents(p, "igemm", a_elems<AM>(p) * (long)sizeof(TA), b_elems<BMD>(p) * (long)sizeof(TB),
                           oe * (long)(p.out_f32 ? 4 : sizeof(T)), oe * (long)sizeof(T), " (needs < 2 GiB)"))
    return rc;
  if ((!DYA && p.a_xf.kind == VAE_X_BN_DY) || (!DYB && p.b_xf.kind == VAE_X_BN_DY))
    return fail(VAE_E_UNSUPPORTED, "igemm: BN_DY transform on an operand this op does not support");
  const bool va = operand_vec<AM>(p, p.a_ptr, p.a_xf, (int)sizeof(TA));
  const bool vb = operand_vec<100 + BMD>(p, p.b_ptr, p.b_xf, (int)sizeof(TB));
  if (va && vb) launch_shape<T, TA, TB, AM, BMD, EM, true, true, DYA, DYB>(p, t, st);
  else if (va) launch_shape<T, TA, TB, AM, BMD, EM, true, false, DYA, DYB>(p, t, st);
  else if (vb) launch_shape<T, TA, TB, AM, BMD, EM, false, true, DYA, DYB>(p, t, st);
  else launch_shape<T, TA, TB, AM, BMD, EM, false, false, DYA, DYB>(p, t, st);
  if (lds_error) {
    lds_error = false;
    return fail(VAE_E_UNSUPPORTED, "igemm: per-channel tables of %d / %d channels exceed the LDS", p.a_xf.channels,
                p.epi_xf.channels);
  }
  int rc = check_launch("igemm");
  if (rc) return rc;
  if (p.slab && (rc = launch_finalize<T, EM>(p, st))) return rc;
  return det_reduce<EM>(p, st);
}

template <int AM, int BMD, int EM>
inline bool fgemm_ok(const GemmParams& p) {
  if constexpr (BMD != B_NK || AM == A_KM || EM == E_ACC) return false;
  if constexpr (AM == A_CONV || AM == A_CONVT) return false;
  if (p.g_nchw || p.ones_col >= 0) return false;
  if (p.K % 32 || p.a_ld % 8 || p.b_ld % 8) return false;
  if (!aligned(p.a_ptr, 16) || !aligned(p.b_ptr, 16)) return false;
  if (p.a_xf.kind == VAE_X_BN_DY && !aligned(p.a_xf.aux, 16)) return false;
  if (bn_kind(p.a_xf) && p.a_xf.channels % 8) return false;
  return true;
}

template <class T, class TA, int AM, int EM, bool DYA>
inline int launch_fgemm(GemmParams p, void* ws, long ws_bytes, hipStream_t st) {
  constexpr int BM = 32, BN = 32;
  if (int rc = set_extents(p, "fgemm", a_elems<AM>(p) * (long)sizeof(TA), b_elems<B_NK>(p) * (long)sizeof(T), 0,
                           EM != E_REPARAM ? out_elems(p) * (long)sizeof(T) : 0, ""))
    return rc;
  const int steps = (phase_kmax(p, AM) + 31) / 32;
  const long tiles = (long)((p.M + BM - 1) / BM) * ((p.N + BN - 1) / BN) * p.nphase;
  int split = 1;
  if (tiles < 2 * kCUs) {
    split = (int)((2 * kCUs + tiles - 1) / tiles);
    if (split > steps / 4) split = steps / 4;
    if (split < 2) split = 1;
  }
  if (int rc = split_fits(&split, 0, p, ws, ws_bytes, "fgemm split-K")) return rc;
  p.ksplit = split;
  p.slab = split > 1 ? static_cast<float*>(ws) : nullptr;
  const dim3 grid((p.M + BM - 1) / BM, (p.N + BN - 1) / BN, p.nphase * p.ksplit);
  const size_t lds = (size_t)(tab_floats(p.a_xf, false) + (EM == E_BNBWD ? tab_floats(p.epi_xf, true) : 0)) * 4;
  VAE_LAUNCH((fgemm_kernel<T, TA, BM, BN, AM, EM, DYA>), grid, dim3(256), lds, st, p);
  int rc = check_launch("fgemm");
  if (rc) return rc;
  if (p.slab) return launch_finalize<T, EM>(p, st);
  return VAE_OK;
}

template <int AM, int BMD, int EM, bool DYA, bool DYB, bool A_F32 = false, bool B_F32 = false>
inline int launch(int dtype, bool a_f32, bool b_f32, GemmParams p, int split_req, void* ws, long ws_bytes,
                  hipStream_t st) {
  if (p.M <= 0 || p.N <= 0) return VAE_OK;
  finish_divs(p);
  if constexpr (BMD == B_NK && AM != A_KM && EM != E_ACC) {
    if (!a_f32 && !b_f32 && split_req <= 0 && !p.det && fgemm_ok<AM, BMD, EM>(p)) {
      if (dtype == VAE_F32) return launch_fgemm<float, float, AM, EM, DYA>(p, ws, ws_bytes, st);
      if (dtype == VAE_BF16) return launch_fgemm<__bf16, __bf16, AM, EM, DYA>(p, ws, ws_bytes, st);
    }
// ... 28 lines not shown
  }
  if (dtype == VAE_F32) return launch_tiled<float, float, float, AM, BMD, EM, DYA, DYB>(p, t, st);
  if (dtype != VAE_BF16) return fail(VAE_E_BADDTYPE, "dtype %d", dtype);
  if constexpr (A_F32) {
    if (a_f32) return launch_tiled<__bf16, float, __bf16, AM, BMD, EM, DYA, DYB>(p, t, st);
  }
  if constexpr (B_F32) {
    if (b_f32) return launch_tiled<__bf16, __bf16, float, AM, BMD, EM, DYA, DYB>(p, t, st);
  }
  if (a_f32 || b_f32) return fail(VAE_E_UNSUPPORTED, "fp32 operand not instantiated for this op");
  return launch_tiled<__bf16, __bf16, __bf16, AM, BMD, EM, DYA, DYB>(p, t, st);
}

template <class T, int V>
__global__ void __launch_bounds__(256) column_sum_flat(const T* x, long nvec, int C, float* out) {
  extern __shared__ float red[];
  const int groups = C / V;
  for (int c = threadIdx.x; c < C; c += blockDim.x) red[c] = 0.f;
  __syncthreads();
  const int c0 = (int)(threadIdx.x % groups) * V;
  float acc[V];
#pragma unroll
  for (int j = 0; j < V; ++j) acc[j] = 0.f;
  const long stride = (long)gridDim.x * blockDim.x;
  long i = (long)blockIdx.x * blockDim.x + threadIdx.x;
  for (; i + 7 * stride < nvec; i += 8 * stride) {
    if constexpr (V == 8) {
      float v[8][8];
#pragma unroll
      for (int u = 0; u < 8; ++u) ld8(x + (i + u * stride) * 8, v[u]);
#pragma unroll
      for (int u = 0; u < 8; ++u)
#pragma unroll
        for (int j = 0; j < 8; ++j) acc[j] += v[u][j];
    } else {
      float v[8];
#pragma unroll
      for (int u = 0; u < 8; ++u) v[u] = ld_f(x + i + u * stride);
      acc[0] += ((v[0] + v[1]) + (v[2] + v[3])) + ((v[4] + v[5]) + (v[6] + v[7]));
    }
  }
  for (; i < nvec; i += stride) {
    if constexpr (V == 8) {
      float v[8];
      ld8(x + i * 8, v);
#pragma unroll
      for (int j = 0; j < 8; ++j) acc[j] += v[j];
    } else {
      acc[0] += ld_f(x + i);
    }
  }
#pragma unroll
  for (int j = 0; j < V; ++j) atomicAdd(red + c0 + j, acc[j]);
  __syncthreads();
  for (int c = threadIdx.x; c < C; c += blockDim.x) atomicAdd(out + c, red[c]);
}

template <class T>
__global__ void column_sum(const T* x, long rows, int C, float* out) {
  const int c = blockIdx.y * 64 + (threadIdx.x & 63);
  if (c >= C) return;
  float s = 0.f;
  for (long r = blockIdx.x * 4 + (threadIdx.x >> 6); r < rows; r += (long)gridDim.x * 4) s += ld_f(x + r * C + c);
  atomicAdd(out + c, s);
}

__global__ void __launch_bounds__(256) flip_weights_kernel(const __bf16* w, __bf16* wf, int K, int RR, int C, int flip) {
  __shared__ float t[32][33];
  const int tap = blockIdx.z, k0 = blockIdx.y * 32, c0 = blockIdx.x * 32;
  const int tx = threadIdx.x & 31, ty = threadIdx.x >> 5;
  for (int j = ty; j < 32; j += 8) {
    const int k = k0 + j, c = c0 + tx;
    t[j][tx] = (k < K && c < C) ? (float)w[((long)k * RR + tap) * C + c] : 0.f;
  }
  __syncthreads();
  const int tap2 = flip ? RR - 1 - tap : tap;
  for (int j = ty; j < 32; j += 8) {
    const int c = c0 + j, k = k0 + tx;
    if (c < C && k < K) wf[((long)c * RR + tap2) * K + k] = (__bf16)t[tx][j];
  }
}

inline int flip_weights_launch(const __bf16* w, __bf16* wf, int K, int R, int C, hipStream_t st, int flip) {
  const dim3 grid((C + 31) / 32, (K + 31) / 32, R * R);
  VAE_LAUNCH(flip_weights_kernel, grid, dim3(256), 0, st, w, wf, K, R * R, C, flip);
  return check_launch("flip_weights");
}

struct StagedWeights {
  const void* ptr;
  long slab_bytes;
  long tail;
};
inline StagedWeights staged_weights(const vae_conv_args* a, const void* given) {
  StagedWeights s = {given, a->workspace_bytes, 0};
  if (!given && a->workspace) {
    s.tail = (long)a->k * a->r * a->r * a->c * 2;
    s.slab_bytes = ((a->workspace_bytes - s.tail) / 256) * 256;
    if (s.slab_bytes < 0) s.slab_bytes = 0;
    s.ptr = static_cast<char*>(a->workspace) + s.slab_bytes;
  }
  return s;
}
template <class F>
inline int with_staged_weights(const StagedWeights& s, const vae_conv_args* a, int K, int C, int flip, const char* what,
                               hipStream_t st, F&& go) {
  return with_ws_tail(s.tail, [&]() -> int {
    if (s.tail) {
      if (!ws_fits(s.tail, a->workspace_bytes, what)) return VAE_E_BADARG;
      if (int rc = flip_weights_launch(static_cast<const __bf16*>(a->wt), static_cast<__bf16*>(const_cast<void*>(s.ptr)),
                                       K, a->r, C, st, flip)) return rc;
    }
    return go();
  });
}

inline bool cg_ok(const GemmParams& p, int em) {
  if (p.g_nchw || p.ones_col >= 0 || p.gc % 8 || p.N % 8 || p.out_ld % 8 || p.b_ld % 8) return false;
  if (!aligned(p.a_ptr, 16) || !aligned(p.b_ptr, 16) || !aligned(p.out, 16)) return false;
  const int k = p.a_xf.kind;
  if (em == E_STORE && k == VAE_X_BN_DY) return false;
  if (em == E_BNBWD && k == VAE_X_BN_ACT) return false;
  if ((k == VAE_X_BN_ACT || k == VAE_X_BN_DY) && (p.a_xf.channels != p.gc || p.a_xf.channels > MAXC)) return false;
  if (k == VAE_X_BN_DY && !aligned(p.a_xf.aux, 16)) return false;
  if (p.residual && !aligned(p.residual, 16)) return false;
  if (cg_table_bytes(p, em) + cg_static_bytes(32, 32) > kLdsBytes) return false;
  if (em == E_BNBWD && p.epi_xf.kind != VAE_X_NONE) {
    if (!aligned(p.epi_xf.aux, 16) || (p.epi_xf.kind == VAE_X_BN_ACT && p.epi_xf.channels % 8)) return false;
  }
  return true;
}

struct CgTile { int bm, bn; };

constexpr int kCgMinWg = 2, kCgSplitWg = 1;

inline CgTile cg_pick(long M, long N, int nphase, long table_bytes = 0, bool xform = false) {
  const CgTile c[] = {{128, 128}, {128, 32}, {64, 64}, {64, 32}, {32, 64}, {32, 32}};
  for (const CgTile& t : c) {
    if (table_bytes + cg_static_bytes(t.bm, t.bn) > kLdsBytes) continue;
    if (t.bm > 32 && M < t.bm) continue;
    if (t.bn > 32 && N < t.bn) continue;
    if (t.bm == 128 && t.bn == 32 && tile_blocks(M, N, nphase, Tile{64, 32}) < (xform ? 4 : 8) * kCUs) continue;
    if (tile_blocks(M, N, nphase, Tile{t.bm, t.bn}) >= (long)kCgMinWg * kCUs) return t;
  }
  return CgTile{32, 32};
}

template <int BM, int BN> constexpr int cg_bk() { return BM >= 128 ? 64 : 128; }

template <int AM, int XA, int EM, int OR>
inline void cg_launch_tile(const GemmParams& p, CgTile t, hipStream_t st) {
  const size_t lds = (size_t)cg_table_bytes(p, EM);
#define VAE_CG_CASE(BM_, BN_) \
  if (t.bm == BM_ && t.bn == BN_) { \
    const unsigned nb = (unsigned)(((p.M + BM_ - 1) / BM_) * ((p.N + BN_ - 1) / BN_) * p.nphase * p.ksplit); \
    VAE_LAUNCH((cgemm_kernel<BM_, BN_, cg_bk<BM_, BN_>(), AM, XA, EM, OR>), dim3(nb), dim3(256), lds, st, p); \
    return; \
  }
  VAE_CG_CASE(128, 128)
  VAE_CG_CASE(128, 32)
  VAE_CG_CASE(64, 64)
  VAE_CG_CASE(64, 32)
  VAE_CG_CASE(32, 64)
  VAE_CG_CASE(32, 32)
#undef VAE_CG_CASE
}

template <int AM, int EM>
inline int cg_launch(GemmParams p, int split_req, void* ws, long ws_bytes, hipStream_t st) {
  if (p.M <= 0 || p.N <= 0) return VAE_OK;
  finish_divs(p);
  const long ob = out_elems(p) * 2;
  if (int rc = set_extents(p, "cgemm", a_elems<AM>(p) * 2, (long)p.N * p.b_ld * 2, ob, ob, "")) return rc;
  if (split_req <= 0 && bgemm_ok(p, AM, EM)) {
    const int rc = bgemm_launch(p, AM, EM, ws, ws_bytes, st);
    if (rc != kRouteDeclined) return rc;
  }
  const CgTile t = cg_pick(p.M, p.N, p.nphase, cg_table_bytes(p, EM),
                           p.a_xf.kind == VAE_X_BN_ACT || p.a_xf.kind == VAE_X_BN_DY);
  const int bk = t.bm >= 128 ? 64 : 128;
  p.m_fast = (long)p.b_bytes > (long)p.a_bytes ? 1 : 0;
  const int ktiles = (phase_kmax(p, AM) + bk - 1) / bk;
  const long blocks = tile_blocks(p.M, p.N, p.nphase, Tile{t.bm, t.bn});
  int split = split_req > 0 ? split_req : 1;
  if (split_req <= 0 && blocks < (long)kCgSplitWg * kCUs && ktiles >= 4) {
    split = (int)((2 * (long)kCgSplitWg * kCUs + blocks - 1) / blocks);
    if (split > ktiles / 2) split = ktiles / 2;
  }
  if (int rc = split_fits(&split, split_req, p, ws, ws_bytes, "cgemm split-K")) return rc;
  p.ksplit = split < 1 ? 1 : split;
  p.slab = p.ksplit > 1 ? static_cast<float*>(ws) : nullptr;
  const int kps = (ktiles + p.ksplit - 1) / p.ksplit;
  const bool dy = p.a_xf.kind == VAE_X_BN_DY;
  const int KCt = bk / 8, RPPt = 256 / KCt;
  const int loads = ((t.bm + RPPt - 1) / RPPt) * (dy ? 2 : 1) + (t.bn + RPPt - 1) / RPPt;
  const int ns = cg_ring(loads);
  const bool one = kps <= ns;
  const bool deep = EM == E_STORE && !one && kps <= cg_ring_deep(loads) && blocks * p.ksplit <= 2l * kCUs;
#define VAE_CG_XA(XA_) (deep ? cg_launch_tile<AM, XA_, EM, (EM == E_STORE ? 3 : 0)>(p, t, st) \
                        : !one ? cg_launch_tile<AM, XA_, EM, 0>(p, t, st) \
                              : kps <= 2 ? cg_launch_tile<AM, XA_, EM, 2>(p, t, st) : cg_launch_tile<AM, XA_, EM, 1>(p, t, st))
  switch (p.a_xf.kind) {
    case VAE_X_NONE: VAE_CG_XA(VAE_X_NONE); break;
    case VAE_X_ACT: VAE_CG_XA(VAE_X_ACT); break;
    case VAE_X_BN_ACT:
      if constexpr (EM == E_STORE) VAE_CG_XA(VAE_X_BN_ACT);
      break;
    case VAE_X_BN_DY:
      if constexpr (EM == E_BNBWD) VAE_CG_XA(VAE_X_BN_DY);
      break;
  }
#undef VAE_CG_XA
  int rc = check_launch("cgemm");
  if (rc) return rc;
  if (p.slab) return launch_finalize<__bf16, EM>(p, st);
  return VAE_OK;
}

inline int column_sum_launch(int dtype, const void* dy, long rows, int C, float* db, hipStream_t st) {
  const int V = (C % 8 == 0 && ((uintptr_t)dy % 16) == 0) ? 8 : 1;
  const int groups = C / V;
  if (groups <= 256 && rows > 0) {
    const int bd = (256 / groups) * groups;
    const long nvec = rows * (long)(C / V);
    long blocks = (nvec + (long)bd * 8 - 1) / ((long)bd * 8);
    if (blocks > 256) blocks = 256;
    if (blocks < 1) blocks = 1;
    const size_t lds = (size_t)C * sizeof(float);
    if (dtype == VAE_F32) {
      if (V == 8) VAE_LAUNCH((column_sum_flat<float, 8>), dim3((unsigned)blocks), dim3(bd), lds, st, (const float*)dy, nvec, C, db);
      else VAE_LAUNCH((column_sum_flat<float, 1>), dim3((unsigned)blocks), dim3(bd), lds, st, (const float*)dy, nvec, C, db);
    } else {
      if (V == 8) VAE_LAUNCH((column_sum_flat<__bf16, 8>), dim3((unsigned)blocks), dim3(bd), lds, st, (const __bf16*)dy, nvec, C, db);
      else VAE_LAUNCH((column_sum_flat<__bf16, 1>), dim3((unsigned)blocks), dim3(bd), lds, st, (const __bf16*)dy, nvec, C, db);
    }
    return check_launch("column_sum");
  }
  const dim3 grid(64, (C + 63) / 64);
  if (dtype == VAE_F32) VAE_LAUNCH(column_sum<float>, grid, dim3(256), 0, st, (const float*)dy, rows, C, db);
  else VAE_LAUNCH(column_sum<__bf16>, grid, dim3(256), 0, st, (const __bf16*)dy, rows, C, db);
  return check_launch("column_sum");
}

inline int then_bias_grad(int rc, const vae_conv_args* a, bool done, hipStream_t st) {
  if (rc || !a->db || done) return rc;
  return column_sum_launch(a->dtype, a->dy, (long)a->n * a->p * a->q, a->k, a->db, st);
}

}
}
```

### pytorch-vae_amd/csrc/vae_runtime.hip

```cpp
#include <cxxabi.h>
#include <stdarg.h>
#include <stdio.h>
#include <stdlib.h>

#include "vae_common.hpp"

namespace vae {

static thread_local char g_err[512] = "";

void set_error(const char* fmt, ...) {
  va_list ap;
  va_start(ap, fmt);
  vsnprintf(g_err, sizeof(g_err), fmt, ap);
  va_end(ap);
}

int fail(int code, const char* fmt, ...) {
  va_list ap;
  va_start(ap, fmt);
  vsnprintf(g_err, sizeof(g_err), fmt, ap);
  va_end(ap);
  return code;
}

int check_launch(const char* what) {
  if (querying()) return VAE_OK;
  const hipError_t e = hipGetLastError();
  if (e != hipSuccess) return fail((int)e, "%s: %s", what, hipGetErrorString(e));
  return VAE_OK;
}

namespace {

__global__ void __launch_bounds__(256) ordered_sum_kernel(const OrdSum o) {
  __shared__ float part[8][33];
  const int cl = threadIdx.x & 31, rl = threadIdx.x >> 5;
  const long e = (long)blockIdx.x * 32 + cl;
  const bool ok = e < (long)o.groups * o.cols;
  const int g = ok ? (int)(e / o.cols) : 0;
  const int c = ok ? (int)(e - (long)g * o.cols) : 0;
  const int half = c / o.cw, cc = c - half * o.cw;
  const float* base = o.slab + (long)g * o.rpg * o.rstride + (long)half * o.hstride + cc;
  float s = 0.f;
  if (ok) {
    int r = rl;
    for (; r + 24 < o.rpg; r += 32) {
      float v[4];
#pragma unroll
      for (int u = 0; u < 4; ++u) {
        float t = 0.f;
        for (int f = 0; f < o.folds; ++f) t += base[(long)(r + 8 * u) * o.rstride + (long)f * o.fstride];
        v[u] = t;
      }
#pragma unroll
      for (int u = 0; u < 4; ++u) s += v[u];
    }
    for (; r < o.rpg; r += 8) {
      float t = 0.f;
      for (int f = 0; f < o.folds; ++f) t += base[(long)r * o.rstride + (long)f * o.fstride];
      s += t;
    }
  }
  part[rl][cl] = s;
  __syncthreads();
  if (rl == 0 && ok) {
    float t = 0.f;
#pragma unroll
    for (int l = 0; l < 8; ++l) t += part[l][cl];
    float* d = o.dst[half] + (long)g * o.gstride + cc;
    *d += t;
  }
}

}

int ordered_sum_launch(const OrdSum& o, hipStream_t st) {
  const long outs = (long)o.groups * o.cols;
  if (outs <= 0 || o.rpg <= 0) return VAE_OK;
  if (!o.slab || !o.dst[0] || (o.cols > o.cw && !o.dst[1]))
    return fail(VAE_E_BADARG, "ordered_sum: null slab or destination");
  VAE_LAUNCH(ordered_sum_kernel, dim3((unsigned)((outs + 31) / 32)), dim3(256), 0, st, o);
  return check_launch("ordered_sum");
}
}

using namespace vae;

extern "C" int vae_abi_version(void) { return VAE_ABI_VERSION; }

extern "C" int vae_launch_log(int32_t on) {
  LaunchLog& l = launch_log();
  if (on) l.n = 0;
  l.on = on ? 1 : 0;
  return VAE_OK;
}

extern "C" int64_t vae_launch_log_names(char* buf, int64_t cap) {
  const LaunchLog& l = launch_log();
  int64_t need = 0;
  for (int i = 0; i < l.n; ++i) {
    const char* m = hipKernelNameRefByPtr(l.k[i], nullptr);
    if (!m) m = "?";
    int st = 0;
    char* d = abi::__cxa_demangle(m, nullptr, nullptr, &st);
    const int w = snprintf(buf && need < cap ? buf + need : nullptr, buf && need < cap ? (size_t)(cap - need) : 0,
                           "%s\t%s\t%d\n", m, (st == 0 && d) ? d : m, l.count[i]);
    free(d);
    need += w > 0 ? w : 0;
  }
  if (buf && cap > 0 && need >= cap) buf[cap - 1] = '\0';
  return need + 1;
}
extern "C" const char* vae_last_error(void) { return g_err; }

#ifdef VAE_PROBE
static unsigned long long* g_probe = nullptr;
extern "C" void vae_probe_set(void* buf) { g_probe = static_cast<unsigned long long*>(buf); }
extern "C" unsigned long long* vae_probe_buffer(void) { return g_probe; }
#endif

extern "C" int vae_deferred_reset(void) {
  deferred().n = 0;
  deferred().has_elbo = 0;
  return VAE_OK;
}

extern "C" int32_t vae_deferred_take(vae_grad_slab* out, int32_t max, vae_elbo_args* elbo, int32_t* has_elbo) {
  Deferred& d = deferred();
  const int n = d.n;
  for (int i = 0; i < n && i < max && out; ++i) out[i] = d.s[i];
  if (has_elbo) *has_elbo = d.has_elbo;
  if (elbo && d.has_elbo) *elbo = d.elbo;
  d.n = 0;
  d.has_elbo = 0;
  return n;
}

namespace {
template <class A, class F>
int ws_size(const A* a, size_t* bytes, F&& call) {
  if (!a || !bytes) return fail(VAE_E_BADARG, "workspace_size: null argument");
  A c = *a;
  c.workspace = reinterpret_cast<void*>(uintptr_t(1) << 40);
  c.workspace_bytes = int64_t(1) << 50;
  WsQuery& q = ws_query();
  q.on = 1;
  q.need = 0;
  const int rc = call(&c);
  *bytes = rc ? 0 : (size_t)q.need;
  q.on = 0;
  q.need = 0;
  return rc;
}
}

extern "C" int vae_conv2d_workspace_size(const vae_conv_args* a, int32_t op, size_t* bytes) {
  switch (op) {
    case VAE_OP_FWD: return ws_size(a, bytes, [](const vae_conv_args* c) { return vae_conv2d_fwd(c, nullptr); });
    case VAE_OP_BWD_DATA: return ws_size(a, bytes, [](const vae_conv_args* c) { return vae_conv2d_bwd_data(c, nullptr); });
    case VAE_OP_BWD_FILTER: return ws_size(a, bytes, [](const vae_conv_args* c) { return vae_conv2d_bwd_filter(c, nullptr); });
  }
  return fail(VAE_E_BADARG, "conv2d_workspace_size: op %d", op);
}

extern "C" int vae_convT2d_workspace_size(const vae_conv_args* a, int32_t op, size_t* bytes) {
  switch (op) {
    case VAE_OP_FWD: return ws_size(a, bytes, [](const vae_conv_args* c) { return vae_convT2d_fwd(c, nullptr); });
    case VAE_OP_BWD_DATA: return ws_size(a, bytes, [](const vae_conv_args* c) { return vae_convT2d_bwd_data(c, nullptr); });
    case VAE_OP_BWD_FILTER: return ws_size(a, bytes, [](const vae_conv_args* c) { return vae_convT2d_bwd_filter(c, nullptr); });
    case VAE_OP_BWD: return ws_size(a, bytes, [](const vae_conv_args* c) { return vae_convT2d_bwd(c, nullptr); });
  }
  return fail(VAE_E_BADARG, "convT2d_workspace_size: op %d", op);
}

extern "C" int vae_linear_workspace_size(const vae_linear_args* a, int32_t op, size_t* bytes) {
  switch (op) {
    case VAE_OP_FWD: return ws_size(a, bytes, [](const vae_linear_args* c) { return vae_linear_fwd(c, nullptr); });
    case VAE_OP_BWD_DATA: return ws_size(a, bytes, [](const vae_linear_args* c) { return vae_linear_bwd_data(c, nullptr); });
    case VAE_OP_BWD_FILTER: return ws_size(a, bytes, [](const vae_linear_args* c) { return vae_linear_bwd_filter(c, nullptr); });
  }
  return fail(VAE_E_BADARG, "linear_workspace_size: op %d", op);
}

extern "C" int vae_head_workspace_size(const vae_head_args* a, int32_t op, size_t* bytes) {
  switch (op) {
    case VAE_OP_FWD: return ws_size(a, bytes, [](const vae_head_args* c) { return vae_head_fwd(c, nullptr); });
    case VAE_OP_BWD_DATA: return ws_size(a, bytes, [](const vae_head_args* c) { return vae_head_bwd_data(c, nullptr); });
    case VAE_OP_BWD_FILTER: return ws_size(a, bytes, [](const vae_head_args* c) { return vae_head_bwd_filter(c, nullptr); });
    case VAE_OP_BWD: return ws_size(a, bytes, [](const vae_head_args* c) { return vae_head_bwd(c, nullptr); });
  }
  return fail(VAE_E_BADARG, "head_workspace_size: op %d", op);
}
```

### pytorch-vae_amd/vae_amd/_lib.py

```python
from __future__ import annotations

import ctypes
import os
from ctypes import POINTER, c_float, c_int32, c_int64, c_void_p

import torch

LIB_NAME = "libvaehip.so"
LIB_PATH = os.path.join(os.path.dirname(os.path.abspath(__file__)), LIB_NAME)
if os.environ.get("VAE_HIP_LIB"):
    LIB_PATH = LIB_PATH.replace("libvaehip.so", "libvaehip_%s.so" % os.environ["VAE_HIP_LIB"])
ABI_VERSION = 26

F32, BF16 = 0, 1
X_NONE, X_ACT, X_BN_ACT, X_BN_DY = 0, 1, 2, 3
LOSS_VANILLA, LOSS_BETA_H, LOSS_BETA_B, LOSS_IWAE, LOSS_VQ, LOSS_INFO, LOSS_DIP = 0, 1, 2, 3, 4, 5, 6
LOSS_MIWAE = 7
MMD_IMQ, MMD_RBF = 0, 1


class VaeHipError(RuntimeError):
    pass


class Xform(ctypes.Structure):
    _fields_ = [("kind", c_int32), ("channels", c_int32), ("slope", c_float), ("count", c_float),
                ("eps", c_float), ("momentum", c_float),
                ("sum", c_void_p), ("sumsq", c_void_p), ("shift", c_void_p), ("gamma", c_void_p),
                ("beta", c_void_p), ("dgamma", c_void_p), ("dbeta", c_void_p), ("aux", c_void_p),
                ("running_mean", c_void_p), ("running_var", c_void_p),
                ("reps", c_int32), ("rstride", c_int32), ("dgamma_out", c_void_p), ("dbeta_out", c_void_p),
                ("table", c_void_p)]


class BnArgs(ctypes.Structure):
    _fields_ = [("mode", c_int32), ("xf", Xform), ("table", c_void_p), ("db", c_void_p)]


class ConvArgs(ctypes.Structure):
    _fields_ = [("dtype", c_int32), ("n", c_int32), ("h", c_int32), ("w", c_int32), ("c", c_int32),
                ("k", c_int32), ("p", c_int32), ("q", c_int32), ("r", c_int32), ("stride", c_int32),
                ("pad", c_int32), ("x_nchw_f32", c_int32),
                ("x", c_void_p), ("x_xf", Xform), ("wt", c_void_p), ("bias", c_void_p), ("y", c_void_p),
                ("y_sum", c_void_p), ("y_sumsq", c_void_p), ("sum_reps", c_int32), ("sum_rstride", c_int32),
                ("residual", c_void_p), ("residual_xf", Xform),
                ("dy", c_void_p), ("dy_xf", Xform), ("dx", c_void_p), ("dx_epi", Xform),
                ("dx_dgamma", c_void_p), ("dx_dbeta", c_void_p), ("dw", c_void_p), ("db", c_void_p),
                ("split_k", c_int32), ("workspace", c_void_p), ("workspace_bytes", c_int64),
                ("bn_finalize", POINTER(BnArgs)), ("bn_counter", c_void_p), ("wt_t", c_void_p),
                ("dw_inner", c_int32), ("deterministic", c_int32), ("defer_reduce", c_int32)]


class LinearArgs(ctypes.Structure):
    _fields_ = [("dtype", c_int32), ("m", c_int32), ("n", c_int32), ("k", c_int32),
                ("x", c_void_p), ("x_xf", Xform), ("wt", c_void_p), ("bias", c_void_p), ("y", c_void_p),
                ("y_f32", c_int32), ("dy", c_void_p), ("dy_f32", c_int32), ("dx", c_void_p), ("dx_epi", Xform),
                ("dx_dgamma", c_void_p),
                ("dx_dbeta", c_void_p), ("sum_reps", c_int32), ("sum_rstride", c_int32),
                ("dw", c_void_p), ("db", c_void_p),
                ("mulv", c_void_p), ("eps", c_void_p), ("kl_coef", c_void_p), ("dmulv", c_void_p),
                ("samples", c_int32), ("workspace", c_void_p), ("workspace_bytes", c_int64),
                ("bn_finalize", POINTER(BnArgs)), ("bn_counter", c_void_p), ("deterministic", c_int32)]


class HeadArgs(ctypes.Structure):
    _fields_ = [("dtype", c_int32), ("n", c_int32), ("h", c_int32), ("w", c_int32), ("c", c_int32),
                ("x", c_void_p), ("x_xf", Xform), ("wt", c_void_p), ("bias", c_void_p),
                ("target", c_void_p), ("samples", c_int32), ("recon", c_void_p), ("sse", c_void_p),
                ("coef", c_void_p), ("dx", c_void_p), ("dx_epi", Xform), ("dx_dgamma", c_void_p),
                ("dx_dbeta", c_void_p), ("sum_reps", c_int32), ("sum_rstride", c_int32),
                ("dw", c_void_p), ("db", c_void_p), ("grad_recon", c_void_p),
                ("workspace", c_void_p), ("workspace_bytes", c_int64),
                ("bn_finalize", POINTER(BnArgs)), ("bn_counter", c_void_p), ("elbo", c_void_p),
                ("deterministic", c_int32), ("defer_reduce", c_int32)]


class ElboArgs(ctypes.Structure):
    _fields_ = [("kind", c_int32), ("batch", c_int32), ("samples", c_int32), ("latent", c_int32),
                ("img_elems", c_int32), ("kld_weight", c_float), ("beta", c_float), ("gamma", c_float),
                ("c_max", c_float), ("c_stop_iter", c_float), ("iter", c_void_p), ("mulv", c_void_p),
                ("sse", c_void_p), ("out", c_void_p), ("per_img", c_void_p), ("head_coef", c_void_p),
                ("kl_coef", c_void_p), ("vq_sse", c_void_p), ("vq_beta", c_float), ("vq_elems", c_float),
                ("recon_weight", c_float), ("kl_factor", c_float), ("mmd_coef", c_float), ("mmd_tiles", c_int32),
                ("mmd_partials", c_void_p), ("mmd_out", c_void_p)]


class MmdArgs(ctypes.Structure):
    _fields_ = [("kind", c_int32), ("batch", c_int32), ("latent", c_int32), ("latent_var", c_float),
                ("grad_scale", c_float), ("prior_gen", c_int32), ("mulv", c_void_p), ("eps", c_void_p),
                ("prior", c_void_p), ("dz", c_void_p), ("dmulv", c_void_p), ("workspace", c_void_p),
                ("workspace_bytes", c_int64), ("prior_step", c_void_p), ("prior_seed", ctypes.c_uint64)]


class DipArgs(ctypes.Structure):
    _fields_ = [("batch", c_int32), ("latent", c_int32), ("lambda_diag", c_float), ("lambda_offdiag", c_float),
                ("grad_scale", c_float), ("reserved", c_int32), ("mulv", c_void_p), ("dmulv_dip", c_void_p),
                ("dmulv", c_void_p), ("workspace", c_void_p), ("workspace_bytes", c_int64)]


SLAB_MAX = 32
SUMSQ_MAX_PARTS = 1024


class GradSlab(ctypes.Structure):
    _fields_ = [("dst", c_void_p), ("count", c_int64), ("slab", c_void_p), ("rows", c_int32), ("ld", c_int64)]


class AdamArgs(ctypes.Structure):
    _fields_ = [("n", c_int64), ("p", c_void_p), ("g", c_void_p), ("m", c_void_p), ("v", c_void_p),
                ("step", c_void_p), ("lr", c_void_p), ("beta1", ctypes.c_double), ("beta2", ctypes.c_double),
                ("eps", c_float), ("weight_decay", c_float), ("p_lowp", c_void_p), ("nslab", c_int32),
                ("slab", GradSlab * SLAB_MAX), ("has_elbo", c_int32), ("elbo", ElboArgs)]


class VqArgs(ctypes.Structure):
    _fields_ = [("dtype", c_int32), ("rows", c_int32), ("dim", c_int32), ("codes", c_int32),
                ("lat", c_void_p), ("lat_xf", Xform), ("codebook", c_void_p), ("indices", c_void_p),
                ("q", c_void_p), ("sse", c_void_p), ("beta", c_float), ("dq", c_void_p), ("loss_grad", c_void_p),
                ("dlat", c_void_p), ("dcodebook", c_void_p)]


class ReconArgs(ctypes.Structure):
    _fields_ = [("dtype", c_int32), ("n", c_int32), ("h", c_int32), ("w", c_int32), ("c", c_int32),
                ("y", c_void_p), ("target", c_void_p), ("recon", c_void_p), ("sse", c_void_p), ("dy", c_void_p),
                ("grad_scale", c_float), ("grad_recon", c_void_p), ("ld", c_int32)]


class BnApplyArgs(ctypes.Structure):
    _fields_ = [("dtype", c_int32), ("rows", c_int64), ("channels", c_int32), ("x", c_void_p), ("xf", Xform),
                ("db", c_void_p), ("out", c_void_p)]


class ReconLossArgs(ctypes.Structure):
    _fields_ = [("kind", c_int32), ("n", c_int32), ("c", c_int32), ("h", c_int32), ("w", c_int32),
                ("recon", c_void_p), ("target", c_void_p), ("mask", c_void_p), ("window", c_float * 16),
                ("window_size", c_int32), ("levels", c_int32), ("level_weights", c_float * 8),
                ("normalize", c_int32), ("size_average", c_int32), ("grad", c_void_p), ("grad_scale", c_float),
                ("out", c_void_p), ("sse", c_void_p), ("per_img", c_void_p), ("workspace", c_void_p),
                ("workspace_bytes", c_int64)]


RLOSS_CENTER, RLOSS_MSSIM = 0, 1


class LogCoshArgs(ctypes.Structure):
    _fields_ = [("n", c_int32), ("latent", c_int32), ("elems", c_int64), ("alpha", c_float),
                ("grad_scale", c_float), ("kl_weight", c_float), ("reserved", c_int32),
                ("recon", c_void_p), ("target", c_void_p), ("grad", c_void_p), ("mulv", c_void_p),
                ("out", c_void_p), ("kl_coef", c_void_p), ("sse", c_void_p), ("per_img", c_void_p),
                ("workspace", c_void_p), ("workspace_bytes", c_int64)]


class RecordArgs(ctypes.Structure):
    _fields_ = [("batch", c_int32), ("samples", c_int32), ("img_elems", c_int32), ("nterms", c_int32),
                ("step", c_int32), ("src_terms", c_void_p), ("terms", c_void_p), ("per_img", c_void_p),
                ("per", c_void_p), ("img", c_void_p), ("recon", c_void_p), ("best", c_void_p), ("at", c_void_p),
                ("hi_img", c_void_p), ("hi_recon", c_void_p), ("lo_img", c_void_p), ("lo_recon", c_void_p)]


class SwapDesc(ctypes.Structure):
    _fields_ = [("src", c_void_p), ("dst", c_void_p), ("a", c_int32), ("rs", c_int32), ("b", c_int32),
                ("src_dtype", c_int32)]


SWAP_MAX = 16
PAD_MAX = 4


class PadDesc(ctypes.Structure):
    _fields_ = [("rows", c_int64), ("c", c_int32), ("cp", c_int32), ("src", c_void_p), ("dst", c_void_p)]


class KeepRange(ctypes.Structure):
    _fields_ = [("off", c_int64), ("bytes", c_int64)]


class StepBeginArgs(ctypes.Structure):
    _fields_ = [("zero", c_void_p), ("bytes", c_int64), ("step", c_void_p), ("dtype", c_int32),
                ("n", c_int32), ("c", c_int32), ("h", c_int32), ("w", c_int32), ("cp", c_int32),
                ("x", c_void_p), ("y", c_void_p), ("npad", c_int32), ("pad", PadDesc * PAD_MAX),
                ("nswap", c_int32), ("swap", SwapDesc * SWAP_MAX), ("nkeep", c_int32),
                ("keep", KeepRange * 32)]


class LatentArgs(ctypes.Structure):
    _fields_ = [("dtype", c_int32), ("batch", c_int32), ("samples", c_int32), ("latent", c_int32),
                ("in_features", c_int32), ("out_features", c_int32),
                ("x", c_void_p), ("x_xf", Xform), ("w1", c_void_p), ("b1", c_void_p), ("mulv", c_void_p),
                ("eps", c_void_p), ("z", c_void_p), ("w2", c_void_p), ("b2", c_void_p), ("h", c_void_p),
                ("dh", c_void_p), ("kl_coef", c_void_p), ("dmulv", c_void_p), ("dw2", c_void_p), ("db2", c_void_p),
                ("dx", c_void_p), ("dx_epi", Xform), ("dx_dgamma", c_void_p), ("dx_dbeta", c_void_p),
                ("sum_reps", c_int32), ("sum_rstride", c_int32), ("dw1", c_void_p), ("db1", c_void_p),
                ("eps_step", c_void_p), ("eps_seed", ctypes.c_uint64), ("eps_gen", c_int32)]

_SIGS = {
    "vae_abi_version": [],
    "vae_last_error": [],
    "vae_build_digest": [],
    "vae_launch_log": [c_int32],
    "vae_launch_log_names": [ctypes.c_char_p, c_int64],
    "vae_conv2d_fwd": [POINTER(ConvArgs), c_void_p],
    "vae_conv2d_bwd_data": [POINTER(ConvArgs), c_void_p],
    "vae_conv2d_bwd_filter": [POINTER(ConvArgs), c_void_p],
    "vae_convT2d_fwd": [POINTER(ConvArgs), c_void_p],
    "vae_convT2d_bwd_data": [POINTER(ConvArgs), c_void_p],
    "vae_convT2d_bwd_filter": [POINTER(ConvArgs), c_void_p],
    "vae_convT2d_bwd": [POINTER(ConvArgs), c_void_p],
    "vae_convT2d_fwd_recon": [POINTER(ConvArgs), POINTER(ReconArgs), c_void_p],
    "vae_linear_fwd": [POINTER(LinearArgs), c_void_p],
    "vae_linear_bwd_data": [POINTER(LinearArgs), c_void_p],
    "vae_linear_bwd_filter": [POINTER(LinearArgs), c_void_p],
    "vae_head_fwd": [POINTER(HeadArgs), c_void_p],
    "vae_head_bwd_data": [POINTER(HeadArgs), c_void_p],
    "vae_head_bwd_filter": [POINTER(HeadArgs), c_void_p],
    "vae_head_bwd": [POINTER(HeadArgs), c_void_p],
    "vae_bn_finalize": [POINTER(BnArgs), c_void_p],
    "vae_reparam_fwd": [c_int32, c_int32, c_int32, c_int32, c_void_p, c_void_p, c_void_p, c_void_p],
    "vae_elbo_fwd": [POINTER(ElboArgs), c_void_p],
    "vae_mmd_fwd": [POINTER(MmdArgs), c_void_p],
    "vae_mmd_workspace_size": [POINTER(MmdArgs), POINTER(ctypes.c_size_t), POINTER(c_int32)],
    "vae_mmd_reseed": [c_int32, c_int32, c_void_p, c_void_p, c_void_p, c_void_p, c_void_p, c_void_p],
    "vae_dip_fwd": [POINTER(DipArgs), c_void_p],
    "vae_dip_workspace_size": [POINTER(DipArgs), POINTER(ctypes.c_size_t), POINTER(c_int32)],
    "vae_vq_fwd": [POINTER(VqArgs), c_void_p],
    "vae_vq_bwd": [POINTER(VqArgs), c_void_p],
    "vae_recon_fwd": [POINTER(ReconArgs), c_void_p],
    "vae_recon_bwd": [POINTER(ReconArgs), c_void_p],
    "vae_adam_step": [c_int64, c_void_p, c_void_p, c_void_p, c_void_p, c_void_p, c_void_p, ctypes.c_double,
                      ctypes.c_double, c_float, c_float, c_void_p, c_void_p],
    "vae_grad_sumsq": [c_int64, c_void_p, c_void_p, POINTER(c_int32), c_void_p],
    "vae_adam_step_clip": [c_int64, c_void_p, c_void_p, c_void_p, c_void_p, c_void_p, c_void_p, ctypes.c_double,
                           ctypes.c_double, c_float, c_float, c_void_p, c_void_p, c_int32, c_void_p, c_void_p,
                           c_void_p],
    "vae_cast_bf16": [c_int64, c_void_p, c_void_p, c_void_p],
    "vae_deferred_reset": [],
    "vae_deferred_take": [POINTER(GradSlab), c_int32, POINTER(ElboArgs), POINTER(c_int32)],
    "vae_adam_step_ex": [POINTER(AdamArgs), c_void_p],
    "vae_step_begin": [c_void_p, c_int64, c_void_p, c_void_p],
    "vae_step_record": [POINTER(RecordArgs), c_void_p],
    "vae_swap_axes": [c_int32, c_void_p, c_void_p],
    "vae_nchw_to_nhwc_pad": [c_int32, c_int32, c_int32, c_int32, c_int32, c_int32, c_void_p, c_void_p, c_void_p],
    "vae_pad_channels": [c_int32, c_int64, c_int32, c_int32, c_void_p, c_void_p, c_void_p],
    "vae_unpad_accumulate": [c_int64, c_int32, c_int32, c_void_p, c_void_p, c_void_p],
    "vae_conv2d_workspace_size": [POINTER(ConvArgs), c_int32, POINTER(ctypes.c_size_t)],
    "vae_convT2d_workspace_size": [POINTER(ConvArgs), c_int32, POINTER(ctypes.c_size_t)],
    "vae_linear_workspace_size": [POINTER(LinearArgs), c_int32, POINTER(ctypes.c_size_t)],
    "vae_head_workspace_size": [POINTER(HeadArgs), c_int32, POINTER(ctypes.c_size_t)],
    "vae_conv_bwd_filter_batch": [c_int32, c_void_p, c_void_p, c_void_p, c_int64, c_void_p],
    "vae_conv_bwd_filter_batch_workspace_size": [c_int32, c_void_p, c_void_p, POINTER(ctypes.c_size_t)],
    "vae_step_begin_ex": [POINTER(StepBeginArgs), c_void_p],
    "vae_latent_fc_fwd": [POINTER(LatentArgs), c_void_p],
    "vae_latent_dec_fwd": [POINTER(LatentArgs), c_void_p],
    "vae_latent_dec_bwd": [POINTER(LatentArgs), c_void_p],
    "vae_latent_fc_bwd": [POINTER(LatentArgs), c_void_p],
    "vae_recon_loss": [POINTER(ReconLossArgs), c_void_p],
    "vae_bn_apply": [POINTER(BnApplyArgs), c_void_p],
    "vae_recon_loss_workspace_size": [POINTER(ReconLossArgs), POINTER(ctypes.c_size_t)],
    "vae_logcosh_loss": [POINTER(LogCoshArgs), c_void_p],
    "vae_logcosh_loss_workspace_size": [POINTER(LogCoshArgs), POINTER(ctypes.c_size_t)],
}
EXPORTED = tuple(_SIGS)

_lib = None


def load(path: str = LIB_PATH):
    global _lib
    if _lib is not None:
        return _lib
    if not os.path.exists(path):
        raise VaeHipError(f"{path} not found — build it with `make -C pytorch-vae_amd/csrc` "
                          f"(or __graft_entry__.build()); there is no fallback path")
    lib = ctypes.CDLL(path)
    for name, argtypes in _SIGS.items():
        fn = getattr(lib, name)
        fn.argtypes = argtypes
        fn.restype = (ctypes.c_char_p if name in ("vae_last_error", "vae_build_digest") else
                      c_int64 if name == "vae_launch_log_names" else c_int32)
    if lib.vae_abi_version() != ABI_VERSION:
        raise VaeHipError(f"libvaehip ABI {lib.vae_abi_version()} != expected {ABI_VERSION}")
    _lib = lib
    return lib


def call(name: str, *args):
    lib = load()
    rc = getattr(lib, name)(*args)
    if rc != 0:
        msg = lib.vae_last_error().decode(errors="replace")
        raise VaeHipError(f"{name} failed (rc={rc}): {msg}")


OP_FWD, OP_BWD_DATA, OP_BWD_FILTER, OP_BWD = 0, 1, 2, 3
LAYER_CONV2D, LAYER_CONVT2D = 0, 1

WS_QUERY = {
    "vae_conv2d_fwd": ("vae_conv2d_workspace_size", OP_FWD),
    "vae_conv2d_bwd_data": ("vae_conv2d_workspace_size", OP_BWD_DATA),
    "vae_conv2d_bwd_filter": ("vae_conv2d_workspace_size", OP_BWD_FILTER),
    "vae_convT2d_fwd": ("vae_convT2d_workspace_size", OP_FWD),
    "vae_convT2d_bwd_data": ("vae_convT2d_workspace_size", OP_BWD_DATA),
    "vae_convT2d_bwd_filter": ("vae_convT2d_workspace_size", OP_BWD_FILTER),
    "vae_convT2d_bwd": ("vae_convT2d_workspace_size", OP_BWD),
    "vae_linear_fwd": ("vae_linear_workspace_size", OP_FWD),
    "vae_linear_bwd_data": ("vae_linear_workspace_size", OP_BWD_DATA),
    "vae_linear_bwd_filter": ("vae_linear_workspace_size", OP_BWD_FILTER),
    "vae_head_fwd": ("vae_head_workspace_size", OP_FWD),
    "vae_head_bwd_data": ("vae_head_workspace_size", OP_BWD_DATA),
    "vae_head_bwd_filter": ("vae_head_workspace_size", OP_BWD_FILTER),
    "vae_head_bwd": ("vae_head_workspace_size", OP_BWD),
}


def deferred_take():
    lib = load()
    out = (GradSlab * SLAB_MAX)()
    el = ElboArgs()
    has = c_int32(0)
    n = lib.vae_deferred_take(out, SLAB_MAX, ctypes.byref(el), ctypes.byref(has))
    if n > SLAB_MAX:
        raise VaeHipError(f"{n} deferred reductions > {SLAB_MAX}")
    return [GradSlab.from_buffer_copy(out[i]) for i in range(n)], (el if has.value else None)


def workspace_size(fn: str, arg) -> int:
    q, op = WS_QUERY[fn]
    out = ctypes.c_size_t(0)
    call(q, ctypes.byref(arg), op, ctypes.byref(out))
    return int(out.value)


def ptr(t) -> int | None:
    if t is None:
        return None
    return t.data_ptr()


def stream_ptr() -> int:
    return torch.cuda.current_stream().cuda_stream


def dtype_code(dt: torch.dtype) -> int:
    if dt == torch.float32:
        return F32
    if dt == torch.bfloat16:
        return BF16
    raise VaeHipError(f"unsupported dtype {dt}")


class FilterBatch:

    FNS = {"vae_conv2d_bwd_filter": LAYER_CONV2D, "vae_convT2d_bwd_filter": LAYER_CONVT2D}

    def __init__(self, calls):
        self.calls = list(calls)
        n = len(self.calls)
        self.kinds = (c_int32 * n)(*[self.FNS[fn] for fn, _ in self.calls])
        self.items = (c_void_p * n)(*[ctypes.addressof(ref._obj) for _, ref in self.calls])
        self.workspace, self.workspace_bytes = None, 0
        self.side = False
        self.after = []

    @property
    def args(self):
        return [ref._obj for _, ref in self.calls]

    def workspace_size(self) -> int:
        out = ctypes.c_size_t(0)
        call("vae_conv_bwd_filter_batch_workspace_size", len(self.calls), self.kinds, self.items, ctypes.byref(out))
        return int(out.value)

    def __call__(self, stream):
        call("vae_conv_bwd_filter_batch", len(self.calls), self.kinds, self.items, self.workspace,
             self.workspace_bytes, stream)
        for fn, args in self.after:
            call(fn, *args, stream)


def recon_loss_args(kind: int, n: int, c: int, h: int, w: int, *, mask=None, window=None, levels: int = 5,
                    level_weights=(0.0448, 0.2856, 0.3001, 0.2363, 0.1333), normalize: bool = True) -> "ReconLossArgs":
    a = ReconLossArgs(kind=kind, n=n, c=c, h=h, w=w, size_average=1, grad_scale=1.0)
    if kind == RLOSS_CENTER:
        a.mask = mask.data_ptr()
    else:
        win = [float(v) for v in window]
        a.window_size = len(win)
        for i, v in enumerate(win):
            a.window[i] = v
        a.levels = levels
        for i, v in enumerate(level_weights):
            a.level_weights[i] = float(v)
        a.normalize = int(normalize)
    return a


def logcosh_args(n: int, elems: int, alpha: float, *, kl_weight: float = 0.0, latent: int = 0,
                 grad_scale: float = 1.0) -> "LogCoshArgs":
    return LogCoshArgs(n=n, elems=elems, alpha=alpha, grad_scale=grad_scale, kl_weight=kl_weight, latent=latent)


def mmd_workspace(a: "MmdArgs"):
    out, tiles = ctypes.c_size_t(0), c_int32(0)
    call("vae_mmd_workspace_size", ctypes.byref(a), ctypes.byref(out), ctypes.byref(tiles))
    return int(out.value), int(tiles.value)


def dip_workspace(a: "DipArgs"):
    out, tiles = ctypes.c_size_t(0), c_int32(0)
    call("vae_dip_workspace_size", ctypes.byref(a), ctypes.byref(out), ctypes.byref(tiles))
    return int(out.value), int(tiles.value)


def recon_loss_workspace(a: "ReconLossArgs") -> int:
    out = ctypes.c_size_t(0)
    call("vae_recon_loss_workspace_size", ctypes.byref(a), ctypes.byref(out))
    return int(out.value)


def logcosh_workspace(a: "LogCoshArgs") -> int:
    out = ctypes.c_size_t(0)
    call("vae_logcosh_loss_workspace_size", ctypes.byref(a), ctypes.byref(out))
    return int(out.value)
```

### pytorch-vae_amd/vae_amd/calls.py

```python
from __future__ import annotations

import ctypes
from typing import List

import torch

from . import _lib as L

BATCH_FN = "vae_conv_bwd_filter_batch"
DEFERRED_FNS = frozenset(("vae_conv2d_bwd_filter", "vae_convT2d_bwd_filter", "vae_unpad_accumulate"))
SIDE_FNS = frozenset(("vae_conv2d_bwd_filter", "vae_convT2d_bwd_filter", "vae_linear_bwd_filter",
                      "vae_unpad_accumulate"))
_BYREF = type(ctypes.byref(ctypes.c_int32()))


def structs(ref) -> List[ctypes.Structure]:
    if isinstance(ref, L.FilterBatch):
        return ref.args
    if isinstance(ref, _BYREF):
        return [ref._obj]
    if isinstance(ref, tuple):
        return [r._obj for r in ref if isinstance(r, _BYREF)]
    return []


def on_side(plan, fn, ref) -> bool:
    if fn == BATCH_FN:
        return ref.side
    return plan.side_all and fn in SIDE_FNS


def batch_filter_calls(calls, ends, splits=(), enabled: bool = True):
    if not enabled:
        return list(calls), list(ends)
    out, new_ends, lo = [], [], 0

    def emit(deferred, side):
        wg = [(fn, ref) for fn, ref in deferred if fn != "vae_unpad_accumulate"]
        if len(wg) > 1 or (side and wg):
            b = L.FilterBatch(wg)
            b.side = side
            out.append((BATCH_FN, b))
            unpads = [(fn, ref) for fn, ref in deferred if fn == "vae_unpad_accumulate"]
            if side:
                b.after = unpads
            else:
                out.extend(unpads)
        else:
            out.extend(deferred)

    for end in ends:
        deferred = []
        for i in range(lo, end):
            if i in splits and deferred:
                emit(deferred, True)
                deferred = []
            fn, ref = calls[i]
            if fn in DEFERRED_FNS:
                deferred.append((fn, ref))
            else:
                out.append((fn, ref))
        emit(deferred, False)
        new_ends.append(len(out))
        lo = end
    return out, new_ends


def size_workspaces(plan, call_lists):
    dev = plan.net.device
    need = {"main": 0, "side": 0}
    sized = []
    for calls in call_lists:
        for fn, ref in calls:
            if fn == BATCH_FN:
                arg = ref
                b = ref.workspace_size()
            elif fn not in L.WS_QUERY:
                continue
            else:
                arg = ref._obj
                b = L.workspace_size(fn, arg)
            deferred = any(getattr(a, "defer_reduce", 0) for a in structs(ref))
            chain = "side" if plan.side is not None and on_side(plan, fn, ref) else "main"
            if deferred and b > 0:
                chain = f"deferred{len(need)}"
                need[chain] = 0
            need[chain] = max(need[chain], b)
            sized.append((arg, b, chain))
    bufs = {c: torch.empty(max(1, (n + 3) // 4), dtype=torch.float32, device=dev) for c, n in need.items()}
    for arg, b, chain in sized:
        if b > 0:
            arg.workspace = bufs[chain].data_ptr()
            arg.workspace_bytes = bufs[chain].numel() * 4
        else:
            arg.workspace, arg.workspace_bytes = None, 0
    plan.workspace, plan.workspace_side, plan.workspace_need = bufs["main"], bufs["side"], need
    plan.workspace_deferred = [v for k, v in bufs.items() if k.startswith("deferred")]


def run_calls(plan, calls, stream):
    if plan.net.swaps_stale:
        plan.net.refresh_swaps(stream)
    side = plan.side
    main = torch.cuda.current_stream() if side is not None else None
    if main is not None and main.cuda_stream != stream:
        side = None
    forked = False
    for fn, arg in calls:
        if side is not None and on_side(plan, fn, arg):
            side.wait_stream(main)
            call_one(fn, arg, side.cuda_stream)
            forked = True
        else:
            call_one(fn, arg, stream)
    if forked:
        main.wait_stream(side)


def call_one(fn, arg, stream):
    if fn == BATCH_FN:
        arg(stream)
    elif isinstance(arg, tuple):
        L.call(fn, *arg, stream)
    else:
        L.call(fn, arg, stream)
```

### pytorch-vae_amd/vae_amd/net.py

```python
from __future__ import annotations

import ctypes
from typing import Dict, List, Optional

import torch

from . import _lib as L
from .calls import BATCH_FN, batch_filter_calls, call_one, run_calls, size_workspaces, structs
from .layout import reference_key_order, vanilla_layout
from .plan import NetBase, PlanBase, ZeroRegion, _pad4, make_swaps
from .closers import CLOSERS, ReconLoss
from .terms import MMD_KINDS, TERMS

SLOPE = 0.01
MAT_MIN_FLOPS = 4e9
BN_EPS = 1e-5
BN_MOMENTUM = 0.1


class VAENet(NetBase):

    swaps_in_step_begin = True

    def __init__(self, in_channels: int = 3, latent_dim: int = 128, hidden_dims: Optional[List[int]] = None,
                 img_size: int = 64, dtype: torch.dtype = torch.float32, device=None,
                 generator: Optional[torch.Generator] = None):
        self.in_channels = in_channels
        self.latent_dim = latent_dim
        self.hidden_dims = list(hidden_dims or [32, 64, 128, 256, 512])
        self.img_size = img_size
        if img_size % (2 ** len(self.hidden_dims)) or img_size // (2 ** len(self.hidden_dims)) != 2:
            raise ValueError("the reference's bottleneck is a [C,2,2] map (fc_mu = hidden_dims[-1]*4, "
                             "models/vanilla_vae.py:36): need img_size == 2 * 2**len(hidden_dims)")
        if in_channels != 3:
            raise ValueError("the head reconstructs 3 channels (vanilla_vae.py:73); in_channels must be 3")
        super().__init__(vanilla_layout(in_channels, latent_dim, self.hidden_dims),
                         reference_key_order(in_channels, latent_dim, self.hidden_dims), dtype, device, generator)
        if self.lowp is not None:
            names = ([f"encoder.{i}.0.weight" for i in range(1, len(self.hidden_dims))] +
                     [f"decoder.{i}.0.weight" for i in range(len(self.hidden_dims) - 1)] + ["final_layer.0.weight"])
            descs, self.lowp_t = make_swaps(self.layout, self.params, names, self.device, self.wt_t, self.lowp)
            self.swap_descs = [descs]
        self.sync_lowp()

    def run_stats(self, prefix: str):
        b = self.layout.bn_by_prefix[prefix]
        return self.running.data_ptr() + 4 * b.offset, self.running.data_ptr() + 4 * (b.offset + b.channels)


class StepPlan(PlanBase):

    def __init__(self, net: VAENet, batch: int, *, loss: str = "vanilla", kld_weight: float = 1e-8,
                 samples: int = 1, beta: float = 4.0, gamma: float = 1000.0, max_capacity: float = 25.0,
                 capacity_max_iter: float = 1e5, fused_loss: bool = True, training: bool = True,
                 concurrent: bool = False, fuse_bn: bool = False, bn_in_consumer: bool = True,
                 wg_overlap: bool = False, recon_loss: Optional[dict] = None,
                 deterministic: Optional[bool] = None, latent_kernels: bool = True, head_kernels: bool = True,
                 pad_rgb: bool = True, materialise: bool = True, mat_min_flops: float = MAT_MIN_FLOPS,
                 batch_wgrads: bool = True, alpha: float = -0.5, reg_weight: float = 100.0,
                 kernel_type: str = "imq", latent_var: float = 2.0, lambda_diag: float = 10.0,
                 lambda_offdiag: float = 5.0, estimates: Optional[int] = None):
        if loss in CLOSERS:
            CLOSERS[loss].check(alpha=alpha, samples=samples, recon_loss=recon_loss)
        super().__init__(net)
        self.materialise, self.mat_min_flops = bool(materialise), float(mat_min_flops)
        self.batch_wgrads_on = bool(batch_wgrads)
        self.deterministic = (net.dtype == torch.float32) if deterministic is None else bool(deterministic)
        closing = (ReconLoss if recon_loss is not None else CLOSERS.get(loss)) if training and fused_loss else None
        self.seed_recon = (not fused_loss) or closing is not None
        self.B = batch
        self.training = training
        self.fused_loss = fused_loss
        self.bn_in_consumer = bn_in_consumer and training
        if estimates is not None and loss != "miwae":
            raise ValueError(f"estimates is MIWAE's argument, not loss {loss!r}'s")
        self.M = 1
        if loss == "miwae":
            self.M = 1 if estimates is None else int(estimates)
            if self.M < 1 or int(samples) < 1:
                raise ValueError(f"StepPlan(loss='miwae') needs samples >= 1 and estimates >= 1, "
                                 f"got {samples} and {estimates}")
            if not 1 <= batch <= 1024:
                raise ValueError(f"StepPlan(loss='miwae') takes 1..1024 images a batch (vae_elbo_fwd), got {batch}")
        self.S = samples if loss == "iwae" else (self.M * int(samples) if loss == "miwae" else 1)
        self.loss, self.loss_kind = loss, self.LOSS_KINDS[loss]
        self.kld_weight, self.beta, self.gamma = kld_weight, beta, gamma
        if kernel_type not in MMD_KINDS:
            raise ValueError('Undefined kernel type.')
        if loss in TERMS and fused_loss and not training:
            raise ValueError(f"StepPlan(loss='{loss}', training=False) has no fused loss: pass fused_loss=False")
        self.max_capacity, self.capacity_max_iter = max_capacity, capacity_max_iter
        dev, T = net.device, net.dtype
        D, h, img = net.latent_dim, net.hidden_dims, net.img_size
        B, BS = self.B, self.B * self.S
        C5, r0 = net.hidden_dims[-1], net.hidden_dims[::-1][0]
        self.latent_fused = (T == torch.bfloat16 and training and fused_loss and net.latent_dim in (64, 128)
                             and C5 % 128 == 0 and (4 * r0) % 128 == 0 and net.img_size == 64
                             and latent_kernels)
        head_mfma = T == torch.bfloat16 and img == 64 and h[0] in (64, 128) and head_kernels
        self.wide_head = h[0] > 32 and self.S == 1 and not head_mfma

        f32 = dict(dtype=torch.float32, device=dev)
        self.x = torch.zeros(B, 3, img, img, **f32)
        self.pad_rgb = T == torch.bfloat16 and pad_rgb
        if self.pad_rgb:
            self.x8 = torch.zeros(B, img, img, 8, dtype=T, device=dev)
            self.w8 = torch.zeros(h[0] * 9 * 8, dtype=T, device=dev)
        self.eps = torch.zeros(BS, D, **f32)
        self.enc = [torch.empty(B, img >> (i + 1), img >> (i + 1), c, dtype=T, device=dev) for i, c in enumerate(h)]
        self.mulv = torch.empty(B, 2 * D, **f32)
        self.z = torch.empty(BS, D, dtype=T, device=dev)
        r = h[::-1]
        self.h0 = torch.empty(BS, 2, 2, r[0], dtype=T, device=dev)
        self.dec = [torch.empty(BS, 4 << i, 4 << i, c, dtype=T, device=dev) for i, c in enumerate(r[1:])]
        self.fin = torch.empty(BS, img, img, r[-1], dtype=T, device=dev)
        if self.wide_head:
            self.y8 = torch.zeros(BS, img, img, 8, dtype=T, device=dev)
            self.g8 = torch.zeros(BS, img, img, 8, dtype=T, device=dev)
            self.w8h = torch.zeros(8 * 9 * r[-1], dtype=T, device=dev)
            self.b8h = torch.zeros(8, dtype=torch.float32, device=dev)
        self.recon = torch.empty(BS, 3, img, img, **f32)
        self.grad_recon = torch.zeros(BS, 3, img, img, **f32) if self.seed_recon else None
        self.out = torch.zeros(4, **f32)
        self.per_img, self.head_coef, self.kl_coef = (torch.zeros(BS, **f32) for _ in range(3))
        self.num_iter = torch.zeros(1, **f32)
        self.g_enc = [torch.empty_like(t) for t in self.enc]
        self.g_h0 = torch.empty_like(self.h0)
        self.g_dec = [torch.empty_like(t) for t in self.dec]
        self.g_fin = torch.empty_like(self.fin)
        bn_shape = {b.prefix: (2, bn_reps(b.channels), b.channels) for b in net.layout.bns}
        zr = ZeroRegion()
        zr.add("grads", net.layout.total)
        zr.add("metrics", 4)
        for p, (_, reps, c) in bn_shape.items():
            zr.add("bnfwd." + p, 2 * reps * c, pad=False)
            zr.add("bnbwd." + p, 2 * reps * c, pad=False)
        zr.add("sse", BS)
        zr.add("dmulv", B * 2 * D)
        zr.add("counters", 2 * len(bn_shape))
        if self.latent_fused:
            zr.add("mulv", B * 2 * D)
        if self.wide_head:
            zr.add("dw8h", 8 * 9 * r[-1])
            zr.add("db8h", 8)
        z = zr.alloc(dev)
        self.zero, self.grads, self.metrics, self.sse, self.dmulv = (z[k] for k in ("zero", "grads", "metrics", "sse", "dmulv"))
        self.bnfwd = {p: z["bnfwd." + p].view(s) for p, s in bn_shape.items()}
        self.bnbwd = {p: z["bnbwd." + p].view(s) for p, s in bn_shape.items()}
        self.counters = z["counters"].view(torch.int32)
        if self.latent_fused:
            self.mulv = z["mulv"].view(B, 2 * D)
        self.dw8h, self.db8h = z.get("dw8h"), z.get("db8h")
        self.bntab: Dict[str, torch.Tensor] = {
            b.prefix: torch.zeros(7 * b.channels, **f32) for b in net.layout.bns}
        self.step = torch.zeros(1, dtype=torch.int32, device=dev)
        self.side = torch.cuda.Stream(device=dev) if (concurrent and training) else None
        self.wg_overlap = wg_overlap and training and not concurrent
        self._mat_a: Dict[str, torch.Tensor] = {}
        self._mat_dz: Dict[str, torch.Tensor] = {}
        self.side_all = self.side is not None
        if self.wg_overlap:
            self.side = torch.cuda.Stream(device=dev)
        self.term = None
        if loss in TERMS and training:
            self.term = TERMS[loss](self, alpha=alpha, reg_weight=reg_weight, kernel_type=kernel_type,
                                    latent_var=latent_var, lambda_diag=lambda_diag, lambda_offdiag=lambda_offdiag)
        self.closer = None
        if closing is not None:
            self.closer = closing.for_plan(self, recon_loss=recon_loss, alpha=alpha, beta=beta)
        self._build()
        if fuse_bn and training:
            self._fuse_finalize(self.fwd_calls)
            self._fuse_finalize(self.bwd_calls)
        self._bwd_raw = list(self.bwd_calls)
        self.batch_wgrads([len(self._bwd_raw)])

    def defer_reductions(self) -> bool:
        if self.deferred or self.net.dtype != torch.bfloat16 or not self.training:
            return self.deferred
        args = [a for fn, ref in self.bwd_calls if fn in (BATCH_FN, "vae_convT2d_bwd", "vae_head_bwd")
                for a in structs(ref)]
        for a in args:
            a.defer_reduce = 1
        if args:
            self.deferred = True
            self.size_workspaces()
        return self.deferred

    def batch_wgrads(self, ends):
        splits = []
        if self.wg_overlap and len(ends) == 1:
            raw = self.bwd_calls_raw
            first_lin = next((i for i, (fn, _) in enumerate(raw)
                              if fn in ("vae_latent_dec_bwd", "vae_linear_bwd_data")), None)
            if first_lin is not None:
                splits = [first_lin]
        if self.deterministic:
            for fn, ref in self.fwd_calls + self.bwd_calls_raw:
                for a in structs(ref):
                    if hasattr(a, "deterministic"):
                        a.deterministic = 1
        self.bwd_calls, new_ends = batch_filter_calls(self.bwd_calls_raw, ends, splits,
                                                      enabled=self.batch_wgrads_on)
        self.size_workspaces()
        return new_ends

    def _bn_prod_bias(self, prefix: str) -> str:
        return prefix[:-2] + ".0.bias"

    def bn_xf(self, prefix: str, kind: int, count: int, aux=None, running: bool = False,
              table: Optional[bool] = None) -> L.Xform:
        if table is None:
            table = not self.bn_in_consumer or self.wide_bn(prefix)
        net = self.net
        C = net.layout.bn_by_prefix[prefix].channels
        s = self.bnfwd[prefix]
        xf = L.Xform(kind=kind, channels=C, slope=SLOPE, count=float(count), eps=BN_EPS, momentum=BN_MOMENTUM)
        xf.sum, xf.sumsq, xf.reps, xf.rstride = s[0].data_ptr(), s[1].data_ptr(), s.shape[1], C
        xf.shift, xf.gamma, xf.beta = net.p(self._bn_prod_bias(prefix)), net.p(prefix + ".weight"), net.p(prefix + ".bias")
        if kind == L.X_BN_DY:
            xf.dgamma, xf.dbeta = self.bnbwd[prefix][0].data_ptr(), self.bnbwd[prefix][1].data_ptr()
        if table:
            xf.table = self.bntab[prefix].data_ptr() + (4 * 4 * C if kind == L.X_BN_DY else 0)
        if aux is not None:
            xf.aux = aux.data_ptr()
        if running:
            xf.running_mean, xf.running_var = net.run_stats(prefix)
        return xf

    def _publish(self, arg, xf, prefix: str):
        xf.dgamma_out, xf.dbeta_out = self.g(prefix + ".weight"), self.g(prefix + ".bias")
        arg.db = self.g(self._bn_prod_bias(prefix))

    def wide_bn(self, prefix: str) -> bool:
        return self.bn_in_consumer and self.net.layout.bn_by_prefix[prefix].channels > 512

    def fwd_sums(self, arg, prefix: str):
        s = self.bnfwd[prefix]
        arg.y_sum, arg.y_sumsq = s[0].data_ptr(), s[1].data_ptr()
        arg.sum_reps, arg.sum_rstride = s.shape[1], s.shape[2]

    def bwd_sums(self, arg, prefix: str):
        s = self.bnbwd[prefix]
        arg.dx_dgamma, arg.dx_dbeta = s[0].data_ptr(), s[1].data_ptr()
        arg.sum_reps, arg.sum_rstride = s.shape[1], s.shape[2]

    def bwd_extras(self, arg, prefix: str):
        if self.bn_in_consumer and not self.wide_bn(prefix):
            self._publish(arg, arg.dy_xf, prefix)

    def bn_finalize(self, lst, prefix: str, mode: int, count: int):
        if self.bn_in_consumer and mode in (0, 1) and not self.wide_bn(prefix):
            return
        C = self.net.layout.bn_by_prefix[prefix].channels
        a = L.BnArgs(mode=mode)
        a.xf = self.bn_xf(prefix, L.X_BN_DY if mode == 1 else L.X_BN_ACT, count, running=(mode != 1), table=False)
        a.table = self.bntab[prefix].data_ptr() + (4 * 4 * C if mode == 1 else 0)
        if mode == 1:
            self._publish(a, a.xf, prefix)
        self._add(lst, "vae_bn_finalize", a)

    def big_layer(self, flops: float, cin: int, cout: int) -> bool:
        return (self.net.dtype == torch.bfloat16 and self.training and self.materialise
                and flops >= self.mat_min_flops and min(cin, cout) >= 128)

    def mat_act(self, F, prefix: str, t: torch.Tensor):
        out = self._mat_a[prefix] = torch.empty_like(t)
        a = L.BnApplyArgs(dtype=self.net.dcode, rows=t.numel() // t.shape[-1], channels=t.shape[-1])
        a.x, a.out = t.data_ptr(), out.data_ptr()
        a.xf = self.bn_xf(prefix, L.X_BN_ACT, _cnt(t), running=True)
        self._add(F, "vae_bn_apply", a)

    def mat_dz(self, Bw, prefix: str, g: torch.Tensor, y: torch.Tensor):
        out = self._mat_dz[prefix] = torch.empty_like(g)
        a = L.BnApplyArgs(dtype=self.net.dcode, rows=g.numel() // g.shape[-1], channels=g.shape[-1])
        a.x, a.out = g.data_ptr(), out.data_ptr()
        a.xf = self.bn_xf(prefix, L.X_BN_DY, _cnt(y), aux=y)
        if self.bn_in_consumer and not self.wide_bn(prefix):
            self._publish(a, a.xf, prefix)
        self._add(Bw, "vae_bn_apply", a)
        return out

    def _read(self, a, prefix: str, t: torch.Tensor, running: bool = False):
        if prefix in self._mat_a:
            a.x = self._mat_a[prefix].data_ptr()
        else:
            a.x, a.x_xf = t.data_ptr(), self.bn_xf(prefix, L.X_BN_ACT, _cnt(t), running=running)

    def _bwd_dy(self, Bw, prefix: str, g: torch.Tensor, y: torch.Tensor, big: bool):
        self.bn_finalize(Bw, prefix, 1, _cnt(y))
        if big:
            return self.mat_dz(Bw, prefix, g, y).data_ptr(), L.Xform(kind=L.X_NONE, channels=y.shape[-1]), True
        return g.data_ptr(), self.bn_xf(prefix, L.X_BN_DY, _cnt(y), aux=y), False

    def _fuse_finalize(self, calls):
        out = []
        nctr = 0
        for fn, ref in calls:
            bn = structs(ref)[0] if fn == "vae_bn_finalize" else None
            if bn is not None and bn.mode in (0, 1):
                field, key = ("y_sum", bn.xf.sum) if bn.mode == 0 else ("dx_dgamma", bn.xf.dgamma)
                prod = next((a for _, pref in reversed(out) for a in structs(pref)
# ... 399 lines not shown
```

### pytorch-vae_amd/vae_amd/plan.py

```python
from __future__ import annotations

import ctypes
from typing import Dict, List

import torch

from . import _lib as L
from .calls import run_calls, size_workspaces
from .layout import Layout, default_init


def _pad4(n: int) -> int:
    return (n + 3) // 4 * 4


class NetBase:

    swaps_in_step_begin = False

    def __init__(self, layout: Layout, ref_order, dtype: torch.dtype, device, generator):
        self.layout, self.ref_order, self.dtype = layout, ref_order, dtype
        self.device = torch.device(device) if device is not None else torch.device("cuda", torch.cuda.current_device())
        cpu_p = torch.zeros(layout.total)
        cpu_r = torch.zeros(max(1, layout.bn_total))
        default_init(layout, cpu_p, cpu_r[:layout.bn_total], generator)
        self.params = cpu_p.to(self.device)
        self.running = cpu_r.to(self.device)
        self.lowp = (torch.zeros(layout.total, dtype=torch.bfloat16, device=self.device)
                     if dtype == torch.bfloat16 else None)
        self.num_batches_tracked = 0
        self.wt_t: Dict[str, int] = {}
        self.swap_descs: List = []
        self.swaps_stale = False

    @property
    def dcode(self) -> int:
        return L.dtype_code(self.dtype)

    def refresh_swaps(self, stream=None):
        self.swaps_stale = False
        for d in self.swap_descs:
            L.call("vae_swap_axes", len(d), ctypes.byref(d), stream if stream is not None else L.stream_ptr())

    def sync_lowp(self):
        if self.lowp is not None:
            L.call("vae_cast_bf16", self.params.numel(), self.params.data_ptr(), self.lowp.data_ptr(), L.stream_ptr())
            self.refresh_swaps()

    def load_reference_state_dict(self, sd: Dict[str, torch.Tensor]):
        self.layout.load_reference(self.params, self.running, {k: v.to(self.device) for k, v in sd.items()})
        bns = self.layout.bns
        nbt = sd.get(bns[0].prefix + ".num_batches_tracked") if bns else None
        self.num_batches_tracked = int(nbt) if nbt is not None else 0
        self.sync_lowp()

    def reference_state_dict(self) -> Dict[str, torch.Tensor]:
        return self.layout.export_reference(self.params, self.running, self.num_batches_tracked, self.ref_order)

    def p(self, name: str) -> int:
        s = self.layout.by_name[name]
        return self.params.data_ptr() + 4 * s.offset

    def w(self, name: str) -> int:
        s = self.layout.by_name[name]
        if self.lowp is not None:
            return self.lowp.data_ptr() + 2 * s.offset
        return self.params.data_ptr() + 4 * s.offset


def make_swaps(layout: Layout, params: torch.Tensor, names, device, out: Dict[str, int], lowp=None):
    specs = [layout.by_name[n] for n in names if n in layout.by_name]
    if len(specs) > L.SWAP_MAX:
        raise ValueError(f"{len(specs)} swapped weights > {L.SWAP_MAX} per vae_swap_axes launch")
    sizes = [(s.numel + 63) // 64 * 64 for s in specs]
    buf = torch.zeros(max(1, sum(sizes)), dtype=torch.bfloat16, device=device)
    descs = (L.SwapDesc * len(specs))()
    o = 0
    for i, (spec, n) in enumerate(zip(specs, sizes)):
        a, r, r2, b = spec.native_shape
        d = descs[i]
        if lowp is not None:
            d.src, d.src_dtype = lowp.data_ptr() + 2 * spec.offset, L.BF16
        else:
            d.src, d.src_dtype = params.data_ptr() + 4 * spec.offset, L.F32
        d.dst = buf.data_ptr() + 2 * o
        d.a, d.rs, d.b = a, r * r2, b
        out[spec.name] = d.dst
        o += n
    return descs, buf


class ZeroRegion:

    def __init__(self):
        self.pieces = []
        self.numel = 0

    def add(self, name: str, numel: int, pad: bool = True):
        self.pieces.append((name, self.numel, numel))
        self.numel += _pad4(numel) if pad else numel

    def alloc(self, device) -> Dict[str, torch.Tensor]:
        zero = torch.zeros(self.numel, dtype=torch.float32, device=device)
        return {"zero": zero, **{name: zero[o:o + n] for name, o, n in self.pieces}}


class PlanBase:

    side = None
    side_all = True
    wg_overlap = False
    elbo_in_head = False
    closer = None
    term = None
    prior = None
    extra_term = None
    backward_done = False
    deferred = False
    loss_names = ("loss", "Reconstruction_Loss", "KLD")
    _loss_pending = False
    _bwd_raw = None

    def __init__(self, net):
        self.net = net
        self._keep = []
        self.fwd_calls: List = []
        self.bwd_calls: List = []

    @property
    def bwd_calls_raw(self):
        return self.bwd_calls if self._bwd_raw is None else self._bwd_raw

    def batch_wgrads(self, ends):
        return ends

    def defer_reductions(self) -> bool:
        return False

    def use_device_eps(self, step: torch.Tensor, seed: int = 1265) -> bool:
        return False

    def use_device_prior(self, step: torch.Tensor, seed: int = 1265) -> bool:
        return False

    def draw_noise(self, eps: bool = True, prior: bool = True):
        """Fill the step's random inputs on the host side (a plan without any has nothing to do)."""

    def g(self, name: str) -> int:
        s = self.net.layout.by_name[name]
        return self.grads.data_ptr() + 4 * s.offset

    def _add(self, lst, fn, arg):
        self._keep.append(arg)
        lst.append((fn, ctypes.byref(arg)))

    def size_workspaces(self):
        size_workspaces(self, [self.fwd_calls, self.bwd_calls])

    def _run(self, calls, stream):
        run_calls(self, calls, stream)

    def begin(self, stream=None):
        stream = stream if stream is not None else L.stream_ptr()
        L.call("vae_step_begin", self.zero.data_ptr(), self.zero.numel() * 4, self.step.data_ptr(), stream)

    def forward(self, stream=None):
        self._run(self.fwd_calls, stream if stream is not None else L.stream_ptr())
        self._loss_pending = self.elbo_in_head

    def backward(self, stream=None):
        if self.deferred:
            raise RuntimeError(DEFERRED_MSG)
        self._run(self.bwd_calls, stream if stream is not None else L.stream_ptr())
        self._loss_pending = False

    def loss_dict(self) -> Dict[str, float]:
        return dict(zip(self.loss_names, self.out.tolist()))


DEFERRED_MSG = ("this plan's backward is deferred to the optimizer launch of a TrainStep (defer_reductions): "
                "run on its own it leaves unreduced partial gradients.  Build a new plan for plan.backward(), "
                "for a step with a gradient exchange or for TrainStep(defer_reductions=False)")
```

### pytorch-vae_amd/vae_amd/vq.py

```python
from __future__ import annotations

import ctypes
from typing import Dict, List, Optional

import torch

from . import _lib as L
from .calls import structs
from .layout import vq_layout, vq_param_spec
from .net import MAT_MIN_FLOPS, SLOPE
from .plan import NetBase, PlanBase, ZeroRegion, make_swaps

NRES = 6


class VQNet(NetBase):

    def __init__(self, in_channels: int = 3, embedding_dim: int = 64, num_embeddings: int = 512,
                 hidden_dims: Optional[List[int]] = None, img_size: int = 64, dtype: torch.dtype = torch.float32,
                 device=None, generator: Optional[torch.Generator] = None):
        if in_channels != 3:
            raise ValueError("the output layer reconstructs 3 channels (vq_vae.py:156); in_channels must be 3")
        self.in_channels = in_channels
        self.embedding_dim = embedding_dim
        self.num_embeddings = num_embeddings
        self.hidden_dims = list(hidden_dims or [128, 256])
        self.img_size = img_size
        if img_size % (2 ** len(self.hidden_dims)):
            raise ValueError("img_size must be divisible by 2**len(hidden_dims)")
        spec = vq_param_spec(in_channels, embedding_dim, num_embeddings, self.hidden_dims)
        super().__init__(vq_layout(in_channels, embedding_dim, num_embeddings, self.hidden_dims),
                         [n for n, _, _ in spec], dtype, device, generator)
        self.lowp_t: List[torch.Tensor] = []
        self.sync_lowp()

    def ensure_swaps(self, names):
        if self.lowp is None:
            return
        new = sorted(set(names) - set(self.wt_t))
        if not new:
            return
        for i in range(0, len(new), L.SWAP_MAX):
            d, b = make_swaps(self.layout, self.params, new[i:i + L.SWAP_MAX], self.device, self.wt_t)
            self.swap_descs.append(d)
            self.lowp_t.append(b)
        self.refresh_swaps()

    def name_of_lowp(self, ptr: int) -> Optional[str]:
        if self.lowp is None:
            return None
        off = (ptr - self.lowp.data_ptr()) // 2
        for s in self.layout.params:
            if s.offset == off:
                return s.name
        return None


def _act(slope: float = SLOPE, aux: Optional[torch.Tensor] = None) -> L.Xform:
    xf = L.Xform(kind=L.X_ACT, channels=1, slope=slope)
    if aux is not None:
        xf.aux = aux.data_ptr()
    return xf


class VQStepPlan(PlanBase):

    loss_kind = L.LOSS_VQ
    loss_names = ("loss", "Reconstruction_Loss", "VQ_Loss")

    def __init__(self, net: VQNet, batch: int, *, beta: float = 0.25, fused_loss: bool = True, concurrent: bool = False,
                 materialise: bool = True, mat_min_flops: float = MAT_MIN_FLOPS):
        super().__init__(net)
        self.B, self.beta, self.fused_loss = batch, beta, fused_loss
        self.materialise, self.mat_min_flops = bool(materialise), float(mat_min_flops)
        dev, T = net.device, net.dtype
        h, E, img = net.hidden_dims, net.embedding_dim, net.img_size
        B = batch
        f32 = dict(dtype=torch.float32, device=dev)
        act = dict(dtype=T, device=dev)
        self.x = torch.zeros(B, 3, img, img, **f32)
        sp = img
        self.enc = []
        for c in h:
            sp //= 2
            self.enc.append(torch.empty(B, sp, sp, c, **act))
        self.s, C = sp, h[-1]
        m = (B, sp, sp, C)
        self.e_in = torch.empty(*m, **act)
        self.e_t = [torch.empty(*m, **act) for _ in range(NRES)]
        self.e_h = [torch.empty(*m, **act) for _ in range(NRES)]
        self.latpre = torch.empty(B, sp, sp, E, **act)
        self.q = torch.empty(B, sp, sp, E, **act)
        self.indices = torch.zeros(B * sp * sp, dtype=torch.int64, device=dev)
        self.d_in = torch.empty(*m, **act)
        self.d_t = [torch.empty(*m, **act) for _ in range(NRES)]
        self.d_h = [torch.empty(*m, **act) for _ in range(NRES)]
        r = h[::-1]
        self.up = []
        s2 = sp
        for i in range(len(r) - 1):
            s2 *= 2
            self.up.append(torch.empty(B, s2, s2, r[i + 1], **act))
        self.pad_rgb = T == torch.bfloat16
        self.cy = 8 if self.pad_rgb else 3
        if self.pad_rgb:
            self.x8 = torch.zeros(B, img, img, 8, **act)
            self.w8e = torch.zeros(h[0] * 16 * 8, **act)
            self.w8d = torch.zeros(r[-1] * 16 * 8, **act)
            self.b8d = torch.zeros(8, **f32)
        self.y = torch.empty(B, img, img, self.cy, **act)
        self.recon = torch.empty(B, 3, img, img, **f32)
        self.grad_recon = None if fused_loss else torch.zeros(B, 3, img, img, **f32)
        self.vq_grad = torch.ones(1, **f32)
        self.out = torch.zeros(4, **f32)
        self.per_img = torch.zeros(B, **f32)
        self.num_iter = torch.zeros(1, **f32)
        self.g_y = torch.empty_like(self.y)
        self.g_up = [torch.empty_like(t) for t in self.up]
        self.g_h = {st: [torch.empty(*m, **act) for _ in range(NRES + 1)] for st in ("encoder", "decoder")}
        self.g_t = {st: [torch.empty(*m, **act) for _ in range(NRES)] for st in ("encoder", "decoder")}
        self.g_q = torch.empty_like(self.q)
        self.g_lat = torch.empty_like(self.latpre)
        self.g_enc = [torch.empty_like(t) for t in self.enc]
        zr = ZeroRegion()
        zr.add("grads", net.layout.total)
        zr.add("metrics", 4)
        zr.add("sse", B)
        zr.add("vq_sse", 1)
        z = zr.alloc(dev)
        self.zero, self.grads, self.metrics, self.sse, self.vq_sse = (z[k] for k in ("zero", "grads", "metrics", "sse", "vq_sse"))
        self.step = torch.zeros(1, dtype=torch.int32, device=dev)
        self._mat: Dict[int, torch.Tensor] = {}
        self.side = torch.cuda.Stream(device=dev) if concurrent else None
        self._build()
        self._attach_swaps()
        self.size_workspaces()

    def _attach_swaps(self):
        net = self.net
        if net.lowp is None:
            return
        use = []
        for fn, ref in self.fwd_calls + self.bwd_calls:
            if fn in ("vae_conv2d_bwd_data", "vae_convT2d_fwd"):
                for a in structs(ref):
                    name = net.name_of_lowp(a.wt or 0)
                    if name is not None:
                        use.append((a, name))
        net.ensure_swaps([n for _, n in use])
        for arg, name in use:
            arg.wt_t = net.wt_t[name]

    def _conv(self, t_in, cin, cout, r, stride, pad, transposed=False):
        n, hh, ww = t_in.shape[0], t_in.shape[1], t_in.shape[2]
        if transposed:
            p = q = hh * stride
        else:
            p = q = (hh + 2 * pad - r) // stride + 1
        return L.ConvArgs(dtype=self.net.dcode, n=n, h=hh, w=ww, c=cin, k=cout, p=p, q=q, r=r, stride=stride, pad=pad)

    def _res_stack(self, pre: str, first_idx: int, x0: torch.Tensor, ts, hs):
        F, net = self.fwd_calls, self.net
        C = x0.shape[3]
        for j in range(NRES):
            idx = first_idx + j
            hin, hin_xf = (x0, _act()) if j == 0 else (hs[j - 1], L.Xform())
            a = self._conv(hin, C, C, 3, 1, 1)
            a.x, a.x_xf = hin.data_ptr(), hin_xf
            a.wt = net.w(f"{pre}.{idx}.resblock.0.weight")
            a.y = ts[j].data_ptr()
            self._add(F, "vae_conv2d_fwd", a)
            b = self._conv(ts[j], C, C, 1, 1, 0)
            b.x, b.x_xf = ts[j].data_ptr(), _act(0.0)
            b.wt = net.w(f"{pre}.{idx}.resblock.2.weight")
            b.residual, b.residual_xf = hin.data_ptr(), (_act() if j == 0 else L.Xform())
            b.y = hs[j].data_ptr()
            self._add(F, "vae_conv2d_fwd", b)

    def _res_stack_bwd(self, pre: str, first_idx: int, x0: torch.Tensor, ts, hs) -> torch.Tensor:
        Bw, net = self.bwd_calls, self.net
        C = x0.shape[3]
        gh, gt_ = self.g_h[pre], self.g_t[pre]
        for j in reversed(range(NRES)):
            idx = first_idx + j
            dh, dnext, gt = gh[j + 1], gh[j], gt_[j]
            hin, hin_xf = (x0, _act()) if j == 0 else (hs[j - 1], L.Xform())
            a = self._conv(ts[j], C, C, 1, 1, 0)
            a.dy, a.wt = dh.data_ptr(), net.w(f"{pre}.{idx}.resblock.2.weight")
            a.dx, a.dx_epi = gt.data_ptr(), _act(0.0, ts[j])
            self._add(Bw, "vae_conv2d_bwd_data", a)
            f = self._conv(ts[j], C, C, 1, 1, 0)
            f.x, f.x_xf = ts[j].data_ptr(), _act(0.0)
            f.dy, f.dw = dh.data_ptr(), self.g(f"{pre}.{idx}.resblock.2.weight")
            self._add(Bw, "vae_conv2d_bwd_filter", f)
            a = self._conv(hin, C, C, 3, 1, 1)
            a.dy, a.wt = gt.data_ptr(), net.w(f"{pre}.{idx}.resblock.0.weight")
            a.dx, a.residual = dnext.data_ptr(), dh.data_ptr()
            if j == 0:
                a.dx_epi = _act(SLOPE, x0)
            self._add(Bw, "vae_conv2d_bwd_data", a)
            f = self._conv(hin, C, C, 3, 1, 1)
            f.x, f.x_xf = hin.data_ptr(), hin_xf
            f.dy, f.dw = gt.data_ptr(), self.g(f"{pre}.{idx}.resblock.0.weight")
            self._add(Bw, "vae_conv2d_bwd_filter", f)
        return gh[0]

    def _mat_lrelu(self, F, t: torch.Tensor) -> torch.Tensor:
        key = t.data_ptr()
        out = self._mat.get(key)
        if out is None:
            out = self._mat[key] = torch.empty_like(t)
            a = L.BnApplyArgs(dtype=self.net.dcode, rows=t.numel() // t.shape[-1], channels=t.shape[-1])
            a.x, a.out, a.xf = t.data_ptr(), out.data_ptr(), _act()
            self._add(F, "vae_bn_apply", a)
        return out

    def _mat_ok(self, flops: float) -> bool:
        return self.net.dtype == torch.bfloat16 and self.materialise and flops >= self.mat_min_flops

    def _build(self):
        net = self.net
        h, E, K = net.hidden_dims, net.embedding_dim, net.num_embeddings
        nh = len(h)
        B, img = self.B, net.img_size
        C = h[-1]
        F = self.fwd_calls
        T = net.dcode
        r = h[::-1]
        iup = 1 + NRES + 1
        wout = f"decoder.{iup + len(r) - 1}.0"

        def strided(i, cin):
            return L.ConvArgs(dtype=T, n=B, h=img >> i, w=img >> i, c=cin, k=h[i], p=img >> (i + 1), q=img >> (i + 1),
                              r=4, stride=2, pad=1)
        if self.pad_rgb:
            F.append(("vae_nchw_to_nhwc_pad", (T, B, 3, img, img, 8, self.x.data_ptr(), self.x8.data_ptr())))
            F.append(("vae_pad_channels", (T, h[0] * 16, 3, 8, net.w("encoder.0.0.weight"), self.w8e.data_ptr())))
            F.append(("vae_pad_channels", (T, r[-1] * 16, 3, 8, net.w(wout + ".weight"), self.w8d.data_ptr())))
            F.append(("vae_pad_channels", (L.F32, 1, 3, 8, net.p(wout + ".bias"), self.b8d.data_ptr())))
        for i in range(nh):
            src = self.x if i == 0 else self.enc[i - 1]
            cin = 3 if i == 0 else h[i - 1]
            a = strided(i, cin)
            if i == 0:
                if self.pad_rgb:
                    a.c, a.x = 8, self.x8.data_ptr()
                else:
                    a.x_nchw_f32, a.x = 1, self.x.data_ptr()
            elif self._mat_ok(2.0 * B * a.p * a.q * h[i] * 16 * cin):
                a.x = self._mat_lrelu(F, src).data_ptr()
            else:
                a.x, a.x_xf = src.data_ptr(), _act()
            a.wt, a.bias = net.w(f"encoder.{i}.0.weight"), net.p(f"encoder.{i}.0.bias")
            if i == 0 and self.pad_rgb:
                a.wt = self.w8e.data_ptr()
            a.y = self.enc[i].data_ptr()
            self._add(F, "vae_conv2d_fwd", a)
        a = self._conv(self.enc[-1], C, C, 3, 1, 1)
        a.x, a.x_xf = self.enc[-1].data_ptr(), _act()
        a.wt, a.bias = net.w(f"encoder.{nh}.0.weight"), net.p(f"encoder.{nh}.0.bias")
        a.y = self.e_in.data_ptr()
        self._add(F, "vae_conv2d_fwd", a)
        self._res_stack("encoder", nh + 1, self.e_in, self.e_t, self.e_h)
        ilat = nh + 1 + NRES + 1
        a = self._conv(self.e_h[-1], C, E, 1, 1, 0)
        a.x, a.x_xf = self.e_h[-1].data_ptr(), _act()
        a.wt, a.bias = net.w(f"encoder.{ilat}.0.weight"), net.p(f"encoder.{ilat}.0.bias")
        a.y = self.latpre.data_ptr()
        self._add(F, "vae_conv2d_fwd", a)
        self.n_encode = len(F)
        v = L.VqArgs(dtype=net.dcode, rows=B * self.s * self.s, dim=E, codes=K, beta=self.beta)
        v.lat, v.lat_xf = self.latpre.data_ptr(), _act()
        v.codebook = net.p("vq_layer.embedding.weight")
        v.indices, v.q, v.sse = self.indices.data_ptr(), self.q.data_ptr(), self.vq_sse.data_ptr()
        v.dq, v.dlat = self.g_q.data_ptr(), self.g_lat.data_ptr()
        v.loss_grad = None if self.fused_loss else self.vq_grad.data_ptr()
        v.dcodebook = self.g("vq_layer.embedding.weight")
        self._add(F, "vae_vq_fwd", v)
        self.n_decode0 = len(F)
        a = self._conv(self.q, E, C, 3, 1, 1)
        a.x = self.q.data_ptr()
        a.wt, a.bias = net.w("decoder.0.0.weight"), net.p("decoder.0.0.bias")
# ... 112 lines not shown
```

Before: 142,600 images/s.

## Fuse split-K reduction into the GEMM launch via per-tile tickets

For 32x32 cgemm tiles with split-K, each split writes its partial slab, then takes an atomic ticket per output tile. The last arriving workgroup sums all partial slabs and runs the epilogue, including BN sums, inside the same launch. This removes the separate finalize kernel launch for conv forward and backward-data layers. Ticket counters live in the zeroed region or workspace and reset themselves after use. The cost is atomics plus a serialized reduction by one workgroup per tile, and reliance on correct memory ordering.

```diff
diff --git a/include/vaehip.h b/include/vaehip.h
--- a/include/vaehip.h
+++ b/include/vaehip.h
@@ -57,6 +57,8 @@
   float* table;
   float* db;
 } vae_bn_args;
+
+enum vae_split_reduce { VAE_SPLIT_DEFAULT = 0, VAE_SPLIT_IN_LAUNCH = 1, VAE_SPLIT_TWO_LAUNCH = 2 };
 
 typedef struct vae_conv_args {
   int32_t dtype;
@@ -92,6 +94,9 @@
   int32_t dw_inner;
   int32_t deterministic;
   int32_t defer_reduce;
+  int32_t split_reduce;
+  uint32_t* split_tickets;
+  int64_t split_tickets_bytes;
 } vae_conv_args;
 
 typedef struct vae_linear_args {
@@ -313,6 +318,8 @@
 int vae_convT2d_workspace_size(const vae_conv_args* a, int32_t op, size_t* bytes);
 int vae_linear_workspace_size(const vae_linear_args* a, int32_t op, size_t* bytes);
 int vae_head_workspace_size(const vae_head_args* a, int32_t op, size_t* bytes);
+int vae_conv2d_split_tickets_size(const vae_conv_args* a, int32_t op, size_t* bytes);
+int vae_convT2d_split_tickets_size(const vae_conv_args* a, int32_t op, size_t* bytes);
 enum vae_layer_kind { VAE_LAYER_CONV2D = 0, VAE_LAYER_CONVT2D = 1 };
 int vae_conv_bwd_filter_batch(int32_t n, const int32_t* kinds, const vae_conv_args* const* items,
                               void* workspace, int64_t workspace_bytes, void* stream);
diff --git a/pytorch-vae_amd/csrc/vae_cgemm.hpp b/pytorch-vae_amd/csrc/vae_cgemm.hpp
--- a/pytorch-vae_amd/csrc/vae_cgemm.hpp
+++ b/pytorch-vae_amd/csrc/vae_cgemm.hpp
@@ -78,8 +78,9 @@
   return (BM >= 128 && BN >= 128) ? 2 : ((BM == 64 && BN == 32 && XA == VAE_X_BN_DY) ? 3 : 1);
 }
 
-template <int BM, int BN, int BK, int AM, int XA, int EM, int OR>
+template <int BM, int BN, int BK, int AM, int XA, int EM, int OR, bool FUSE = false>
 __device__ __forceinline__ void cgemm_body(const GemmParams& p, const int bid, char* smem) {
+  static_assert(!FUSE || (BM == 32 && BN == 32), "the in-launch reducer is written for the 32 x 32 tile");
   using WG = CgWaves<BM, BN>;
   constexpr int TM = WG::TM, TN = WG::TN, WTM = TM * 16, WTN = TN * 16;
   constexpr int LDK = CgSmem<BM, BN, BK>::LDK;
@@ -229,15 +230,16 @@
   float bias[8];
   const bool has_res = p.residual != nullptr;
   constexpr bool EARLY = EPT <= 2 && cg_waves_per_eu<BM, BN, XA>() < 3;
-  auto epi_loads = [&]() {
+  auto epi_loads = [&](const bool loads, const bool addr = true) {
     const rsrc_t raux = epi_aux_rsrc<EM>(p);
     const rsrc_t rres = epi_res_rsrc<EM>(p);
-    const bool loads = p.slab == nullptr;
 #pragma unroll
     for (int i = 0; i < EPT; ++i) {
-      const int rl = er0 + i * ERS, row = m0 + rl;
-      rok[i] = rl < BM && row < p.M && col_ok;
-      obase[i] = out_row_base(p, phase, rok[i] ? row : 0) + col;
+      if (addr) {
+        const int rl = er0 + i * ERS, row = m0 + rl;
+        rok[i] = rl < BM && row < p.M && col_ok;
+        obase[i] = out_row_base(p, phase, rok[i] ? row : 0) + col;
+      }
       const uint32_t off = (rok[i] && loads) ? (uint32_t)obase[i] * 2u : kOOB;
       bload<16>(raux, off, aux[i]);
       if (EM == E_BNBWD && has_res) bload<16>(rres, off, res[i]);
@@ -250,7 +252,7 @@
       for (int e = 0; e < 8; ++e) bias[e] = p.bias[col + e];
     }
   };
-  if constexpr (EARLY) epi_loads();
+  if constexpr (EARLY) epi_loads(p.slab == nullptr);
   if (a_tab) {
     const int C = p.a_xf.channels;
 #pragma unroll
@@ -383,24 +385,81 @@
         for (int e = 0; e < 4; ++e) Cs[(rq + i * 16 + e) * LDC + cq + j * 16] = acc[i][j][e];
   }
   __syncthreads();
+  bool reduced = false;
   if (p.slab) {
     float* sl = p.slab + ((long)(phase * p.ksplit + ks) * p.M) * p.N;
+    const rsrc_t rsl = make_rsrc(p.slab, (uint32_t)((long)p.M * p.nphase * p.ksplit * p.N * 4));
+    typedef decltype(__builtin_amdgcn_raw_buffer_load_b128(rsl, 0, 0, 0)) u32x4;
 #pragma unroll
     for (int i = 0; i < EPT; ++i) {
       const int rl = er0 + i * ERS, row = m0 + rl;
       if (rl < BM && row < p.M && col_ok) {
         const f32x4 v0 = *reinterpret_cast<const f32x4*>(Cs + rl * LDC + ec * 8);
         const f32x4 v1 = *reinterpret_cast<const f32x4*>(Cs + rl * LDC + ec * 8 + 4);
-        *reinterpret_cast<f32x4*>(sl + (long)row * p.N + col) = v0;
-        *reinterpret_cast<f32x4*>(sl + (long)row * p.N + col + 4) = v1;
-      }
-    }
-    return;
-  }
-  if constexpr (!EARLY) epi_loads();
+        if constexpr (FUSE) {
+          const uint32_t off = (uint32_t)((((long)phase * p.ksplit + ks) * p.M + row) * p.N + col) * 4u;
+          __builtin_amdgcn_raw_buffer_store_b128(__builtin_bit_cast(u32x4, v0), rsl, off, 0, 16);
+          __builtin_amdgcn_raw_buffer_store_b128(__builtin_bit_cast(u32x4, v1), rsl, off + 16u, 0, 16);
+        } else {
+          *reinterpret_cast<f32x4*>(sl + (long)row * p.N + col) = v0;
+          *reinterpret_cast<f32x4*>(sl + (long)row * p.N + col + 4) = v1;
+        }
+      }
+    }
+    if constexpr (!FUSE) {
+      return;
+    } else {
+      asm volatile("s_waitcnt vmcnt(0)" ::: "memory");
+      __syncthreads();
+      uint32_t* const draw_s = reinterpret_cast<uint32_t*>(smem);
+      const uint32_t last = (uint32_t)p.ksplit - 1u;
+      if (tid == 0) {
+        const long tix = ((long)phase * ((p.M + BM - 1) / BM) + m0 / BM) * ((p.N + BN - 1) / BN) + n0 / BN;
+        typedef __attribute__((address_space(1))) uint32_t gu32;
+        gu32* const ticket = (gu32*)(p.tickets + tix);
+        const uint32_t d = __hip_atomic_fetch_add(ticket, 1u, __ATOMIC_RELAXED, __HIP_MEMORY_SCOPE_AGENT);
+        if (d == last) __hip_atomic_store(ticket, 0u, __ATOMIC_RELAXED, __HIP_MEMORY_SCOPE_AGENT);
+        *draw_s = d;
+      }
+      __syncthreads();
+      const uint32_t draw = (uint32_t)__builtin_amdgcn_readfirstlane((int)*draw_s);
+      if (draw != last) return;
+      __syncthreads();
+      __builtin_amdgcn_fence(__ATOMIC_ACQUIRE, "wavefront");
+      static_assert(EARLY, "the fused tile issues its epilogue loads early");
+      epi_loads(true, false);
+      {
+        static_assert(BM * BN == 256 * 4, "one 16-byte group per thread");
+        const int rr = tid / (BN / 4), rc = (tid % (BN / 4)) * 4;
+        const bool ok = m0 + rr < p.M && n0 + rc < p.N;
+        const uint32_t soff = (uint32_t)((((long)phase * p.ksplit) * p.M + m0 + rr) * p.N + n0 + rc) * 4u;
+        const uint32_t sstride = (uint32_t)((long)p.M * p.N * 4);
+        f32x4 v = f32x4{0.f, 0.f, 0.f, 0.f};
+        for (int s0 = 0; s0 < p.ksplit; s0 += 4) {
+          uint32_t t[4][4];
+#pragma unroll
+          for (int u = 0; u < 4; ++u)
+          {
+            const u32x4 q = __builtin_amdgcn_raw_buffer_load_b128(
+                rsl, (ok && s0 + u < p.ksplit) ? soff + (uint32_t)(s0 + u) * sstride : kOOB, 0, 16);
+            t[u][0] = q[0]; t[u][1] = q[1]; t[u][2] = q[2]; t[u][3] = q[3];
+          }
+#pragma unroll
+          for (int u = 0; u < 4; ++u)
+#pragma unroll
+            for (int e = 0; e < 4; ++e) v[e] += __uint_as_float(t[u][e]);
+        }
+        *reinterpret_cast<f32x4*>(Cs + rr * LDC + rc) = v;
+      }
+      __syncthreads();
+      reduced = true;
+    }
+  }
+  if constexpr (!EARLY) epi_loads(true);
   float s1[8], s2[8];
 #pragma unroll
   for (int e = 0; e < 8; ++e) { s1[e] = 0.f; s2[e] = 0.f; }
+  const bool tile_sums = FUSE && EM == E_STORE && reduced && p.sum != nullptr;
   int ech = 0;
   if constexpr (EM == E_BNBWD) ech = (int)(col - p.fd_ech.div(col) * p.epi_xf.channels);
   uint4 pk[EPT];
@@ -466,6 +525,14 @@
         epi_flush_sums<EM>(p, bid, n0 + c, t1, t2);
       }
     }
+  } else if (tile_sums) {
+    for (int c = tid; c < BN; c += 256) {
+      if (n0 + c < p.N) {
+        float t1 = 0.f, t2 = 0.f;
+        for (int r = 0; r < BM; ++r) { const float x = Cs[r * LDC + c]; t1 += x; t2 = fmaf(x, x, t2); }
+        epi_flush_sums<EM>(p, bid, n0 + c, t1, t2);
+      }
+    }
   } else if (EM == E_BNBWD && epi_wants_sums<EM>(p)) {
     float* part = Cs;
 #pragma unroll
@@ -509,4 +576,12 @@
   cgemm_body<BM, BN, BK, AM, XA, EM, OR>(p, (int)blockIdx.x, smem);
 }
 
-}
+template <int AM, int XA, int EM, int OR>
+__global__ void __launch_bounds__(256) __attribute__((amdgpu_waves_per_eu(cg_waves_per_eu<32, 32, XA>())))
+cgemm_kernel_fused(const GemmParams p) {
+  kernarg_prefetch<sizeof(GemmParams)>();
+  __shared__ __attribute__((aligned(16))) char smem[CgSmem<32, 32, 128, cg_nbuf<32, 32, 128, OR>()>::BYTES];
+  cgemm_body<32, 32, 128, AM, XA, EM, OR, true>(p, (int)blockIdx.x, smem);
+}
+
+}
diff --git a/pytorch-vae_amd/csrc/vae_common.hpp b/pytorch-vae_amd/csrc/vae_common.hpp
--- a/pytorch-vae_amd/csrc/vae_common.hpp
+++ b/pytorch-vae_amd/csrc/vae_common.hpp
@@ -40,9 +40,10 @@
 struct WsQuery {
   int on;
   long need;
+  long tickets;
 };
 inline WsQuery& ws_query() {
-  static thread_local WsQuery q = {0, 0};
+  static thread_local WsQuery q = {0, 0, 0};
   return q;
 }
 inline bool querying() { return ws_query().on != 0; }
diff --git a/pytorch-vae_amd/csrc/vae_convT_bwd_data.hip b/pytorch-vae_amd/csrc/vae_convT_bwd_data.hip
--- a/pytorch-vae_amd/csrc/vae_convT_bwd_data.hip
+++ b/pytorch-vae_amd/csrc/vae_convT_bwd_data.hip
@@ -13,7 +13,7 @@
     return rc;
   if (int rc = check_finalize(a->bn_finalize, "convT2d_bwd_data")) return rc;
   if (a->dtype == VAE_BF16 && cg_ok(p, E_BNBWD))
-    return then_finalize(cg_launch<A_CONV, E_BNBWD>(p, a->split_k, a->workspace, a->workspace_bytes, st), a->bn_finalize, st);
+    return then_finalize(cg_launch<A_CONV, E_BNBWD>(p, a->split_k, a->workspace, a->workspace_bytes, split_mode(a), st), a->bn_finalize, st);
   return then_finalize(launch<A_CONV, B_NK, E_BNBWD, true, false>(a->dtype, false, false, p, a->split_k, a->workspace,
                                                                   a->workspace_bytes, st),
                        a->bn_finalize, st);
diff --git a/pytorch-vae_amd/csrc/vae_convT_fwd.hip b/pytorch-vae_amd/csrc/vae_convT_fwd.hip
--- a/pytorch-vae_amd/csrc/vae_convT_fwd.hip
+++ b/pytorch-vae_amd/csrc/vae_convT_fwd.hip
@@ -23,7 +23,7 @@
     swapped_weights(q, w.ptr);
     if (w.ptr && cg_ok(q, E_STORE)) {
       return with_staged_weights(w, a, a->c, a->k, 0, "convT2d_fwd weight copy", st, [&]() -> int {
-        return then_finalize(cg_launch<A_CONVT, E_STORE>(q, a->split_k, a->workspace, w.slab_bytes, st), a->bn_finalize, st);
+        return then_finalize(cg_launch<A_CONVT, E_STORE>(q, a->split_k, a->workspace, w.slab_bytes, split_mode(a), st), a->bn_finalize, st);
       });
     }
   }
diff --git a/pytorch-vae_amd/csrc/vae_conv_bwd_data.hip b/pytorch-vae_amd/csrc/vae_conv_bwd_data.hip
--- a/pytorch-vae_amd/csrc/vae_conv_bwd_data.hip
+++ b/pytorch-vae_amd/csrc/vae_conv_bwd_data.hip
@@ -48,7 +48,7 @@
     if (w.ptr && cg_ok(q, E_BNBWD)) {
       if (int rc = check_finalize(a->bn_finalize, what)) return rc;
       return with_staged_weights(w, a, a->k, a->c, 0, "conv2d_bwd_data weight copy", st, [&]() -> int {
-        return then_finalize(cg_launch<A_CONVT, E_BNBWD>(q, a->split_k, a->workspace, w.slab_bytes, st), a->bn_finalize, st);
+        return then_finalize(cg_launch<A_CONVT, E_BNBWD>(q, a->split_k, a->workspace, w.slab_bytes, split_mode(a), st), a->bn_finalize, st);
       });
     }
   }
diff --git a/pytorch-vae_amd/csrc/vae_conv_fwd.hip b/pytorch-vae_amd/csrc/vae_conv_fwd.hip
--- a/pytorch-vae_amd/csrc/vae_conv_fwd.hip
+++ b/pytorch-vae_amd/csrc/vae_conv_fwd.hip
@@ -33,7 +33,7 @@
   fwd_epilogue(p, a);
   if (int rc = check_finalize(a->bn_finalize, "conv2d_fwd")) return rc;
   if (a->dtype == VAE_BF16 && cg_ok(p, E_STORE))
-    return then_finalize(cg_launch<A_CONV, E_STORE>(p, a->split_k, a->workspace, a->workspace_bytes, st), a->bn_finalize, st);
+    return then_finalize(cg_launch<A_CONV, E_STORE>(p, a->split_k, a->workspace, a->workspace_bytes, split_mode(a), st), a->bn_finalize, st);
   return then_finalize(launch<A_CONV, B_NK, E_STORE, false, false, true>(a->dtype, a->x_nchw_f32 != 0, false, p, a->split_k,
                                                                          a->workspace, a->workspace_bytes, st),
                        a->bn_finalize, st);
diff --git a/pytorch-vae_amd/csrc/vae_igemm.hpp b/pytorch-vae_amd/csrc/vae_igemm.hpp
--- a/pytorch-vae_amd/csrc/vae_igemm.hpp
+++ b/pytorch-vae_amd/csrc/vae_igemm.hpp
@@ -59,6 +59,7 @@
   int det;
   float* det_slab;
   int det_rows;
+  uint32_t* tickets;
 };
 
 #ifdef VAE_PROBE
diff --git a/pytorch-vae_amd/csrc/vae_launch.hpp b/pytorch-vae_amd/csrc/vae_launch.hpp
--- a/pytorch-vae_amd/csrc/vae_launch.hpp
+++ b/pytorch-vae_amd/csrc/vae_launch.hpp
@@ -175,14 +175,32 @@
   return s < 2 ? 1 : s;
 }
 
-inline int split_fits(int* split, int split_req, const GemmParams& p, const void* ws, long ws_bytes, const char* what) {
+inline long split_ticket_offset(int split, const GemmParams& p) {
+  return (((long)split * p.M * p.N * p.nphase * 4 + 255) / 256) * 256;
+}
+inline long split_ticket_bytes(long words) { return ((words * 4 + 15) / 16) * 16; }
+inline int split_fits(int* split, int split_req, const GemmParams& p, const void* ws, long ws_bytes, const char* what,
+                      long ticket_words = 0) {
   if (*split <= 1) return VAE_OK;
   if (!ws && !querying()) {
     if (split_req > 1) return fail(VAE_E_BADARG, "%s: split_k %d needs a workspace", what, split_req);
     *split = 1;
     return VAE_OK;
   }
-  return ws_fits((long)*split * p.M * p.N * p.nphase * 4, ws_bytes, what) ? VAE_OK : VAE_E_BADARG;
+  const long need = ticket_words > 0 ? split_ticket_offset(*split, p) + split_ticket_bytes(ticket_words)
+                                     : (long)*split * p.M * p.N * p.nphase * 4;
+  return ws_fits(need, ws_bytes, what) ? VAE_OK : VAE_E_BADARG;
+}
+
+constexpr bool kCgSplitInLaunch = true;
+struct SplitMode {
+  uint32_t* words;
+  long bytes;
+  bool two_launch;
+};
+inline SplitMode split_mode(const vae_conv_args* a) {
+  const bool in_launch = a->split_reduce == VAE_SPLIT_IN_LAUNCH || (a->split_reduce == VAE_SPLIT_DEFAULT && kCgSplitInLaunch);
+  return SplitMode{a->split_tickets, (long)a->split_tickets_bytes, !in_launch};
 }
 
 template <class T, int EM>
@@ -517,6 +535,12 @@
 template <int AM, int XA, int EM, int OR>
 inline void cg_launch_tile(const GemmParams& p, CgTile t, hipStream_t st) {
   const size_t lds = (size_t)cg_table_bytes(p, EM);
+  if (p.tickets) {
+    static_assert(cg_bk<32, 32>() == 128, "cgemm_kernel_fused's K-step");
+    const unsigned nb = (unsigned)(((p.M + 31) / 32) * ((p.N + 31) / 32) * p.nphase * p.ksplit);
+    VAE_LAUNCH((cgemm_kernel_fused<AM, XA, EM, OR>), dim3(nb), dim3(256), lds, st, p);
+    return;
+  }
 #define VAE_CG_CASE(BM_, BN_) \
   if (t.bm == BM_ && t.bn == BN_) { \
     const unsigned nb = (unsigned)(((p.M + BM_ - 1) / BM_) * ((p.N + BN_ - 1) / BN_) * p.nphase * p.ksplit); \
@@ -533,7 +557,7 @@
 }
 
 template <int AM, int EM>
-inline int cg_launch(GemmParams p, int split_req, void* ws, long ws_bytes, hipStream_t st) {
+inline int cg_launch(GemmParams p, int split_req, void* ws, long ws_bytes, const SplitMode& sm, hipStream_t st) {
   if (p.M <= 0 || p.N <= 0) return VAE_OK;
   finish_divs(p);
   const long ob = out_elems(p) * 2;
@@ -553,9 +577,27 @@
     split = (int)((2 * (long)kCgSplitWg * kCUs + blocks - 1) / blocks);
     if (split > ktiles / 2) split = ktiles / 2;
   }
-  if (int rc = split_fits(&split, split_req, p, ws, ws_bytes, "cgemm split-K")) return rc;
+  const bool fuse = !sm.two_launch && t.bm == 32 && t.bn == 32 &&
+                    (long)split * p.M * p.N * p.nphase * 4 < (1l << 31);
+  const bool own_words = fuse && sm.words == nullptr;
+  if (int rc = split_fits(&split, split_req, p, ws, ws_bytes, "cgemm split-K", own_words ? blocks : 0)) return rc;
   p.ksplit = split < 1 ? 1 : split;
   p.slab = p.ksplit > 1 ? static_cast<float*>(ws) : nullptr;
+  if (p.slab && fuse) {
+    const long tbytes = split_ticket_bytes(blocks);
+    if (querying()) {
+      if (tbytes > ws_query().tickets) ws_query().tickets = tbytes;
+    } else if (own_words) {
+      p.tickets = reinterpret_cast<uint32_t*>(static_cast<char*>(ws) + split_ticket_offset(p.ksplit, p));
+      const hipError_t e = hipMemsetAsync(p.tickets, 0, (size_t)tbytes, st);
+      if (e != hipSuccess) return fail((int)e, "cgemm split-K tickets: %s", hipGetErrorString(e));
+    } else {
+      if (sm.bytes < tbytes)
+        return fail(VAE_E_BADARG, "cgemm split-K: split_tickets of %ld bytes < %ld required (see vae_*_split_tickets_size)",
+                    sm.bytes, tbytes);
+      p.tickets = sm.words;
+    }
+  }
   const int kps = (ktiles + p.ksplit - 1) / p.ksplit;
   const bool dy = p.a_xf.kind == VAE_X_BN_DY;
   const int KCt = bk / 8, RPPt = 256 / KCt;
@@ -579,7 +621,7 @@
 #undef VAE_CG_XA
   int rc = check_launch("cgemm");
   if (rc) return rc;
-  if (p.slab) return launch_finalize<__bf16, EM>(p, st);
+  if (p.slab && !p.tickets) return launch_finalize<__bf16, EM>(p, st);
   return VAE_OK;
 }
 
diff --git a/pytorch-vae_amd/csrc/vae_runtime.hip b/pytorch-vae_amd/csrc/vae_runtime.hip
--- a/pytorch-vae_amd/csrc/vae_runtime.hip
+++ b/pytorch-vae_amd/csrc/vae_runtime.hip
@@ -139,7 +139,7 @@
 
 namespace {
 template <class A, class F>
-int ws_size(const A* a, size_t* bytes, F&& call) {
+int ws_size(const A* a, size_t* bytes, F&& call, bool tickets = false) {
   if (!a || !bytes) return fail(VAE_E_BADARG, "workspace_size: null argument");
   A c = *a;
   c.workspace = reinterpret_cast<void*>(uintptr_t(1) << 40);
@@ -147,12 +147,30 @@
   WsQuery& q = ws_query();
   q.on = 1;
   q.need = 0;
+  q.tickets = 0;
   const int rc = call(&c);
-  *bytes = rc ? 0 : (size_t)q.need;
+  *bytes = rc ? 0 : (size_t)(tickets ? q.tickets : q.need);
   q.on = 0;
   q.need = 0;
+  q.tickets = 0;
   return rc;
 }
+}
+
+extern "C" int vae_conv2d_split_tickets_size(const vae_conv_args* a, int32_t op, size_t* bytes) {
+  switch (op) {
+    case VAE_OP_FWD: return ws_size(a, bytes, [](const vae_conv_args* c) { return vae_conv2d_fwd(c, nullptr); }, true);
+    case VAE_OP_BWD_DATA: return ws_size(a, bytes, [](const vae_conv_args* c) { return vae_conv2d_bwd_data(c, nullptr); }, true);
+  }
+  return fail(VAE_E_BADARG, "conv2d_split_tickets_size: op %d", op);
+}
+
+extern "C" int vae_convT2d_split_tickets_size(const vae_conv_args* a, int32_t op, size_t* bytes) {
+  switch (op) {
+    case VAE_OP_FWD: return ws_size(a, bytes, [](const vae_conv_args* c) { return vae_convT2d_fwd(c, nullptr); }, true);
+    case VAE_OP_BWD_DATA: return ws_size(a, bytes, [](const vae_conv_args* c) { return vae_convT2d_bwd_data(c, nullptr); }, true);
+  }
+  return fail(VAE_E_BADARG, "convT2d_split_tickets_size: op %d", op);
 }
 
 extern "C" int vae_conv2d_workspace_size(const vae_conv_args* a, int32_t op, size_t* bytes) {
diff --git a/pytorch-vae_amd/vae_amd/_lib.py b/pytorch-vae_amd/vae_amd/_lib.py
--- a/pytorch-vae_amd/vae_amd/_lib.py
+++ b/pytorch-vae_amd/vae_amd/_lib.py
@@ -13,6 +13,7 @@
 ABI_VERSION = 26
 
 F32, BF16 = 0, 1
+SPLIT_DEFAULT, SPLIT_IN_LAUNCH, SPLIT_TWO_LAUNCH = 0, 1, 2
 X_NONE, X_ACT, X_BN_ACT, X_BN_DY = 0, 1, 2, 3
 LOSS_VANILLA, LOSS_BETA_H, LOSS_BETA_B, LOSS_IWAE, LOSS_VQ, LOSS_INFO, LOSS_DIP = 0, 1, 2, 3, 4, 5, 6
 LOSS_MIWAE = 7
@@ -48,7 +49,8 @@
                 ("dx_dgamma", c_void_p), ("dx_dbeta", c_void_p), ("dw", c_void_p), ("db", c_void_p),
                 ("split_k", c_int32), ("workspace", c_void_p), ("workspace_bytes", c_int64),
                 ("bn_finalize", POINTER(BnArgs)), ("bn_counter", c_void_p), ("wt_t", c_void_p),
-                ("dw_inner", c_int32), ("deterministic", c_int32), ("defer_reduce", c_int32)]
+                ("dw_inner", c_int32), ("deterministic", c_int32), ("defer_reduce", c_int32),
+                ("split_reduce", c_int32), ("split_tickets", c_void_p), ("split_tickets_bytes", c_int64)]
 
 
 class LinearArgs(ctypes.Structure):
@@ -246,7 +248,9 @@
     "vae_convT2d_workspace_size": [POINTER(ConvArgs), c_int32, POINTER(ctypes.c_size_t)],
     "vae_linear_workspace_size": [POINTER(LinearArgs), c_int32, POINTER(ctypes.c_size_t)],
     "vae_head_workspace_size": [POINTER(HeadArgs), c_int32, POINTER(ctypes.c_size_t)],
-    "vae_conv_bwd_filter_batch": [c_int32, c_void_p, c_void_p, c_void_p, c_int64, c_void_p],
+    "vae_conv2d_split_tickets_size": [POINTER(ConvArgs), c_int32, POINTER(ctypes.c_size_t)],
+    "vae_convT2d_split_tickets_size": [POINTER(ConvArgs), c_int32, POINTER(ctypes.c_size_t)],
+    "vae_conv_bwd_filter_batch":[c_int32, c_void_p, c_void_p, c_void_p, c_int64, c_void_p],
     "vae_conv_bwd_filter_batch_workspace_size": [c_int32, c_void_p, c_void_p, POINTER(ctypes.c_size_t)],
     "vae_step_begin_ex": [POINTER(StepBeginArgs), c_void_p],
     "vae_latent_fc_fwd": [POINTER(LatentArgs), c_void_p],
@@ -330,6 +334,21 @@
     return int(out.value)
 
 
+TICKET_QUERY = {
+    "vae_conv2d_fwd": ("vae_conv2d_split_tickets_size", OP_FWD),
+    "vae_conv2d_bwd_data": ("vae_conv2d_split_tickets_size", OP_BWD_DATA),
+    "vae_convT2d_fwd": ("vae_convT2d_split_tickets_size", OP_FWD),
+    "vae_convT2d_bwd_data": ("vae_convT2d_split_tickets_size", OP_BWD_DATA),
+}
+
+
+def split_tickets_size(fn: str, arg) -> int:
+    q, op = TICKET_QUERY[fn]
+    out = ctypes.c_size_t(0)
+    call(q, ctypes.byref(arg), op, ctypes.byref(out))
+    return int(out.value)
+
+
 def ptr(t) -> int | None:
     if t is None:
         return None
diff --git a/pytorch-vae_amd/vae_amd/calls.py b/pytorch-vae_amd/vae_amd/calls.py
--- a/pytorch-vae_amd/vae_amd/calls.py
+++ b/pytorch-vae_amd/vae_amd/calls.py
@@ -66,8 +66,26 @@
     return out, new_ends
 
 
+def assign_split_tickets(plan, call_lists):
+    pool = plan.tickets
+    used = 0
+    for calls in call_lists:
+        for fn, ref in calls:
+            if fn not in L.TICKET_QUERY:
+                continue
+            arg = ref._obj
+            arg.split_reduce = L.SPLIT_IN_LAUNCH if plan.split_in_launch else L.SPLIT_TWO_LAUNCH
+            arg.split_tickets, arg.split_tickets_bytes = None, 0
+            b = L.split_tickets_size(fn, arg)
+            if pool is not None and 0 < b <= pool.numel() * 4 - used:
+                arg.split_tickets, arg.split_tickets_bytes = pool.data_ptr() + used, b
+                used += b
+    plan.tickets_used = used
+
+
 def size_workspaces(plan, call_lists):
     dev = plan.net.device
+    assign_split_tickets(plan, call_lists)
     need = {"main": 0, "side": 0}
     sized = []
     for calls in call_lists:
diff --git a/pytorch-vae_amd/vae_amd/net.py b/pytorch-vae_amd/vae_amd/net.py
--- a/pytorch-vae_amd/vae_amd/net.py
+++ b/pytorch-vae_amd/vae_amd/net.py
@@ -8,7 +8,7 @@
 from . import _lib as L
 from .calls import BATCH_FN, batch_filter_calls, call_one, run_calls, size_workspaces, structs
 from .layout import reference_key_order, vanilla_layout
-from .plan import NetBase, PlanBase, ZeroRegion, _pad4, make_swaps
+from .plan import TICKET_POOL_WORDS, NetBase, PlanBase, ZeroRegion, _pad4, make_swaps
 from .closers import CLOSERS, ReconLoss
 from .terms import MMD_KINDS, TERMS
 
@@ -59,11 +59,13 @@
                  pad_rgb: bool = True, materialise: bool = True, mat_min_flops: float = MAT_MIN_FLOPS,
                  batch_wgrads: bool = True, alpha: float = -0.5, reg_weight: float = 100.0,
                  kernel_type: str = "imq", latent_var: float = 2.0, lambda_diag: float = 10.0,
-                 lambda_offdiag: float = 5.0, estimates: Optional[int] = None):
+                 lambda_offdiag: float = 5.0, estimates: Optional[int] = None, split_in_launch: Optional[bool] = None):
         if loss in CLOSERS:
             CLOSERS[loss].check(alpha=alpha, samples=samples, recon_loss=recon_loss)
         super().__init__(net)
         self.materialise, self.mat_min_flops = bool(materialise), float(mat_min_flops)
+        if split_in_launch is not None:
+            self.split_in_launch = bool(split_in_launch)
         self.batch_wgrads_on = bool(batch_wgrads)
         self.deterministic = (net.dtype == torch.float32) if deterministic is None else bool(deterministic)
         closing = (ReconLoss if recon_loss is not None else CLOSERS.get(loss)) if training and fused_loss else None
@@ -143,11 +145,13 @@
         if self.wide_head:
             zr.add("dw8h", 8 * 9 * r[-1])
             zr.add("db8h", 8)
+        zr.add("tickets", TICKET_POOL_WORDS)
         z = zr.alloc(dev)
         self.zero, self.grads, self.metrics, self.sse, self.dmulv = (z[k] for k in ("zero", "grads", "metrics", "sse", "dmulv"))
         self.bnfwd = {p: z["bnfwd." + p].view(s) for p, s in bn_shape.items()}
         self.bnbwd = {p: z["bnbwd." + p].view(s) for p, s in bn_shape.items()}
         self.counters = z["counters"].view(torch.int32)
+        self.tickets = z["tickets"].view(torch.int32)
         if self.latent_fused:
             self.mulv = z["mulv"].view(B, 2 * D)
         self.dw8h, self.db8h = z.get("dw8h"), z.get("db8h")
diff --git a/pytorch-vae_amd/vae_amd/plan.py b/pytorch-vae_amd/vae_amd/plan.py
--- a/pytorch-vae_amd/vae_amd/plan.py
+++ b/pytorch-vae_amd/vae_amd/plan.py
@@ -90,6 +90,9 @@
     return descs, buf
 
 
+TICKET_POOL_WORDS = 8192
+
+
 class ZeroRegion:
 
     def __init__(self):
@@ -120,6 +123,8 @@
     loss_names = ("loss", "Reconstruction_Loss", "KLD")
     _loss_pending = False
     _bwd_raw = None
+    tickets = None
+    split_in_launch = True
 
     def __init__(self, net):
         self.net = net
diff --git a/pytorch-vae_amd/vae_amd/vq.py b/pytorch-vae_amd/vae_amd/vq.py
--- a/pytorch-vae_amd/vae_amd/vq.py
+++ b/pytorch-vae_amd/vae_amd/vq.py
@@ -9,7 +9,7 @@
 from .calls import structs
 from .layout import vq_layout, vq_param_spec
 from .net import MAT_MIN_FLOPS, SLOPE
-from .plan import NetBase, PlanBase, ZeroRegion, make_swaps
+from .plan import TICKET_POOL_WORDS, NetBase, PlanBase, ZeroRegion, make_swaps
 
 NRES = 6
 
@@ -127,7 +127,9 @@
         zr.add("metrics", 4)
         zr.add("sse", B)
         zr.add("vq_sse", 1)
+        zr.add("tickets", TICKET_POOL_WORDS)
         z = zr.alloc(dev)
+        self.tickets = z["tickets"].view(torch.int32)
         self.zero, self.grads, self.metrics, self.sse, self.vq_sse = (z[k] for k in ("zero", "grads", "metrics", "sse", "vq_sse"))
         self.step = torch.zeros(1, dtype=torch.int32, device=dev)
         self._mat: Dict[int, torch.Tensor] = {}
```

Result: no change. 143,500 images/s, median of 6 (+0.6%).
